# feiyeha/EGM-Unet

Hardware: AMD Instinct MI355X
Metric: train images/sec at 3x512x512 bs=8/GPU (higher is better)
Workload: dtype bf16; 1 GPU; EGM-UNet GRFBUNet(3,2,base_c=32) fwd+5-term-loss+bwd+SGD, 8x3x512x512 per GPU (BASELINE.json configs[1]); global_batch=8, parallelism=dp1, launch=hipGraph replay, world_size=1

## Files before the change

egm_unet_amd/csrc/blocks.hip:

```cpp
#include "common.h"
#include "derived_pack.h"

namespace {

__device__ __forceinline__ float sigm(float v) { return 1.f / (1.f + expf(-v)); }

#define PIX_LOOP(total_expr)                                                                           \
    const int ncv = C >> 3;                                                                            \
    const long long total = (total_expr);                                                              \
    for (long long i = blockIdx.x * 256LL + threadIdx.x; i < total; i += (long long)gridDim.x * 256)
#define PIX_LOOP_XCD(total_expr)                                                                       \
    const int ncv = C >> 3;                                                                            \
    const long long total = (total_expr);                                                              \
    for (long long i = xcd_contiguous_item(blockIdx.x, gridDim.x) * 256LL + threadIdx.x; i < total; i += (long long)gridDim.x * 256)

template <typename T>
__global__ void highpass3_kernel(const T* __restrict__ x, int ldx, T* __restrict__ out, int ldo, int N, int H, int W, int C) {
    PIX_LOOP_XCD((long long)N * H * W * ncv) {
        long long p; int cv; egm_divmod(i, ncv, p, cv);
        int xx, yy; egm_pix_yx(p, H, W, yy, xx);
        float s[8], c[8], v[8];
        zero8(s);
        load8(x + p * ldx + cv * 8, c);
#pragma unroll
        for (int r = -1; r <= 1; ++r)
#pragma unroll
            for (int q = -1; q <= 1; ++q) {
                if (yy + r < 0 || yy + r >= H || xx + q < 0 || xx + q >= W) continue;
                load8(x + (p + (long long)r * W + q) * ldx + cv * 8, v);
#pragma unroll
                for (int j = 0; j < 8; ++j) s[j] += v[j];
            }
#pragma unroll
        for (int j = 0; j < 8; ++j) c[j] -= s[j] * (1.f / 9.f);
        store8(out + p * ldo + cv * 8, c);
    }
}

template <typename T>
__global__ void gate_mul_fwd_kernel(const T* __restrict__ x, int ldx, const T* __restrict__ w, int ldw, T* __restrict__ out, int ldo,
                                    long long npix, int C) {
    PIX_LOOP(npix * ncv) {
        long long p; int cv; egm_divmod(i, ncv, p, cv);
        float a[8], b[8];
        load8(x + p * ldx + cv * 8, a); load8(w + p * ldw + cv * 8, b);
#pragma unroll
        for (int j = 0; j < 8; ++j) a[j] *= (1.f + b[j]);
        store8(out + p * ldo + cv * 8, a);
    }
}
template <typename T>
__global__ void gate_mul_bwd_kernel(const T* __restrict__ g, int ldg, const T* __restrict__ x, int ldx, const T* __restrict__ w, int ldw,
                                    T* __restrict__ dx, int lddx, T* __restrict__ dw, int lddw, long long npix, int C) {
    PIX_LOOP(npix * ncv) {
        long long p; int cv; egm_divmod(i, ncv, p, cv);
        float gg[8], a[8], b[8], o1[8], o2[8];
        load8(g + p * ldg + cv * 8, gg); load8(x + p * ldx + cv * 8, a); load8(w + p * ldw + cv * 8, b);
#pragma unroll
        for (int j = 0; j < 8; ++j) { o1[j] = gg[j] * (1.f + b[j]); o2[j] = gg[j] * a[j]; }
        store8(dx + p * lddx + cv * 8, o1); store8(dw + p * lddw + cv * 8, o2);
    }
}

template <typename T>
__global__ void scale_add_relu_fwd_kernel(const T* __restrict__ a, int lda, float alpha, const T* __restrict__ b, int ldb,
                                          T* __restrict__ out, int ldo, long long npix, int C) {
    PIX_LOOP(npix * ncv) {
        long long p; int cv; egm_divmod(i, ncv, p, cv);
        float u[8], v[8];
        load8(a + p * lda + cv * 8, u); load8(b + p * ldb + cv * 8, v);
#pragma unroll
        for (int j = 0; j < 8; ++j) u[j] = fmaxf(fmaf(alpha, u[j], v[j]), 0.f);
        store8(out + p * ldo + cv * 8, u);
    }
}
template <typename T>
__global__ void scale_add_relu_bwd_kernel(const T* __restrict__ g, int ldg, const T* __restrict__ out, int ldo, float alpha,
                                          T* __restrict__ da, int ldda, T* __restrict__ db, int lddb, long long npix, int C) {
    PIX_LOOP(npix * ncv) {
        long long p; int cv; egm_divmod(i, ncv, p, cv);
        float gg[8], o[8], u[8];
        load8(g + p * ldg + cv * 8, gg); load8(out + p * ldo + cv * 8, o);
#pragma unroll
        for (int j = 0; j < 8; ++j) { gg[j] = o[j] > 0.f ? gg[j] : 0.f; u[j] = alpha * gg[j]; }
        store8(da + p * ldda + cv * 8, u); store8(db + p * lddb + cv * 8, gg);
    }
}

template <int GROUP>
__device__ __forceinline__ float group_sum(float v) {
#pragma unroll
    for (int o = GROUP / 2; o > 0; o >>= 1) v += __shfl_xor(v, o, 64);
    return v;
}

template <typename T>
__global__ void gate3_fwd_kernel(const T* __restrict__ x, int ldx, const T* __restrict__ t, int ldt, T* __restrict__ out, int ldo,
                                 long long npix, int C) {
    PIX_LOOP(npix * ncv) {
        long long p; int cv; egm_divmod(i, ncv, p, cv);
        float a[8], tv[8];
        load8(x + p * ldx + cv * 8, a); load8(t + p * ldt, tv);
        const float m = 1.f + (sigm(tv[0]) + sigm(tv[1]) + sigm(tv[2])) * (1.f / 3.f);
#pragma unroll
        for (int j = 0; j < 8; ++j) a[j] *= m;
        store8(out + p * ldo + cv * 8, a);
    }
}
template <typename T, int GROUP>
__global__ void gate3_bwd_kernel(const T* __restrict__ g, int ldg, const T* __restrict__ x, int ldx, const T* __restrict__ t, int ldt,
                                 T* __restrict__ dx, int lddx, T* __restrict__ dt, int lddt, long long npix, int C) {
    const int ncv = C >> 3;
    const int ppb = 256 / GROUP;
    const int lane_in = threadIdx.x % GROUP, slot = threadIdx.x / GROUP;
    for (long long p0 = (long long)blockIdx.x * ppb; p0 < npix; p0 += (long long)gridDim.x * ppb) {
        const long long p = p0 + slot;
        float dot = 0.f, tv[8];
        zero8(tv);
        if (p < npix) {
            load8(t + p * ldt, tv);
            const float m = 1.f + (sigm(tv[0]) + sigm(tv[1]) + sigm(tv[2])) * (1.f / 3.f);
            for (int cv = lane_in; cv < ncv; cv += GROUP) {
                float gg[8], a[8], o[8];
                load8(g + p * ldg + cv * 8, gg); load8(x + p * ldx + cv * 8, a);
#pragma unroll
                for (int j = 0; j < 8; ++j) { o[j] = gg[j] * m; dot += gg[j] * a[j]; }
                store8(dx + p * lddx + cv * 8, o);
            }
        }
        dot = group_sum<GROUP>(dot);
        if (p < npix && lane_in == 0) {
            float o[8];
#pragma unroll
            for (int k = 0; k < 8; ++k) { const float s = sigm(tv[k]); o[k] = k < 3 ? dot * (1.f / 3.f) * s * (1.f - s) : 0.f; }
            store8(dt + p * lddt, o);
        }
    }
}

template <typename T>
__global__ void bcast_gate_fwd_kernel(const T* __restrict__ a, int lda, const T* __restrict__ gl, int ldgl, T* __restrict__ out, int ldo,
                                      long long npix, int C) {
    PIX_LOOP(npix * ncv) {
        long long p; int cv; egm_divmod(i, ncv, p, cv);
        float u[8];
        load8(a + p * lda + cv * 8, u);
        const float s = sigm(to_f32(gl[p * ldgl]));
#pragma unroll
        for (int j = 0; j < 8; ++j) u[j] *= s;
        store8(out + p * ldo + cv * 8, u);
    }
}
template <typename T, int GROUP>
__global__ void bcast_gate_bwd_kernel(const T* __restrict__ g, int ldg, const T* __restrict__ a, int lda, const T* __restrict__ gl, int ldgl,
                                      T* __restrict__ da, int ldda, T* __restrict__ dgl, int lddgl, long long npix, int C) {
    const int ncv = C >> 3;
    const int ppb = 256 / GROUP;
    const int lane_in = threadIdx.x % GROUP, slot = threadIdx.x / GROUP;
    for (long long p0 = (long long)blockIdx.x * ppb; p0 < npix; p0 += (long long)gridDim.x * ppb) {
        const long long p = p0 + slot;
        float dot = 0.f, s = 0.f;
        if (p < npix) {
            s = sigm(to_f32(gl[p * ldgl]));
            for (int cv = lane_in; cv < ncv; cv += GROUP) {
                float gg[8], u[8], o[8];
                load8(g + p * ldg + cv * 8, gg); load8(a + p * lda + cv * 8, u);
#pragma unroll
                for (int j = 0; j < 8; ++j) { o[j] = gg[j] * s; dot += gg[j] * u[j]; }
                store8(da + p * ldda + cv * 8, o);
            }
        }
        dot = group_sum<GROUP>(dot);
        if (p < npix && lane_in == 0) {
            float o[8]; zero8(o);
            o[0] = dot * s * (1.f - s);
            store8(dgl + p * lddgl, o);
        }
    }
}

template <typename T>
__global__ void gelu_fwd_kernel(const T* __restrict__ x, int ldx, T* __restrict__ out, int ldo, long long npix, int C) {
    PIX_LOOP(npix * ncv) {
        long long p; int cv; egm_divmod(i, ncv, p, cv);
        float v[8];
        load8(x + p * ldx + cv * 8, v);
#pragma unroll
        for (int j = 0; j < 8; ++j) v[j] = 0.5f * v[j] * (1.f + erff(v[j] * 0.70710678118654752f));
        store8(out + p * ldo + cv * 8, v);
    }
}
template <typename T>
__global__ void gelu_bwd_kernel(const T* __restrict__ g, int ldg, const T* __restrict__ x, int ldx, T* __restrict__ dx, int lddx,
                                long long npix, int C) {
    PIX_LOOP(npix * ncv) {
        long long p; int cv; egm_divmod(i, ncv, p, cv);
        float gg[8], v[8];
        load8(g + p * ldg + cv * 8, gg); load8(x + p * ldx + cv * 8, v);
#pragma unroll
        for (int j = 0; j < 8; ++j) {
            const float cdf = 0.5f * (1.f + erff(v[j] * 0.70710678118654752f));
            const float pdf = 0.3989422804014327f * expf(-0.5f * v[j] * v[j]);
            gg[j] *= cdf + v[j] * pdf;
        }
        store8(dx + p * lddx + cv * 8, gg);
    }
}

template <typename T, int GROUP>
__global__ void chan_meanmax_fwd_kernel(const T* __restrict__ x, int ldx, T* __restrict__ out, int ldo, long long npix, int C, int Creal) {
    const int ncv = C >> 3;
    const int ppb = 256 / GROUP;
    const int lane_in = threadIdx.x % GROUP, slot = threadIdx.x / GROUP;
    for (long long p0 = (long long)blockIdx.x * ppb; p0 < npix; p0 += (long long)gridDim.x * ppb) {
        const long long p = p0 + slot;
        float s = 0.f, m = -INFINITY;
        if (p < npix)
            for (int cv = lane_in; cv < ncv; cv += GROUP) {
                float v[8];
                load8(x + p * ldx + cv * 8, v);
#pragma unroll
                for (int j = 0; j < 8; ++j) if (cv * 8 + j < Creal) { s += v[j]; m = fmaxf(m, v[j]); }
            }
        s = group_sum<GROUP>(s);
#pragma unroll
        for (int o = GROUP / 2; o > 0; o >>= 1) m = fmaxf(m, __shfl_xor(m, o, 64));
        if (p < npix && lane_in == 0) {
            float o[8]; zero8(o);
            o[0] = s / (float)Creal; o[1] = m;
            store8(out + p * ldo, o);
        }
    }
}
template <typename T, int GROUP>
__global__ void chan_meanmax_bwd_kernel(const T* __restrict__ g, int ldg, const T* __restrict__ x, int ldx, T* __restrict__ dx, int lddx,
                                        long long npix, int C, int Creal) {
    const int ncv = C >> 3;
    const int ppb = 256 / GROUP;
    const int lane_in = threadIdx.x % GROUP, slot = threadIdx.x / GROUP;
    for (long long p0 = (long long)blockIdx.x * ppb; p0 < npix; p0 += (long long)gridDim.x * ppb) {
        const long long p = p0 + slot;
        float m = -INFINITY; int am = 0x7fffffff;
        if (p < npix)
            for (int cv = lane_in; cv < ncv; cv += GROUP) {
                float v[8];
                load8(x + p * ldx + cv * 8, v);
#pragma unroll
                for (int j = 0; j < 8; ++j) if (cv * 8 + j < Creal && v[j] > m) { m = v[j]; am = cv * 8 + j; }
            }
#pragma unroll
        for (int o = GROUP / 2; o > 0; o >>= 1) {
            const float m2 = __shfl_xor(m, o, 64); const int a2 = __shfl_xor(am, o, 64);
            if (m2 > m || (m2 == m && a2 < am)) { m = m2; am = a2; }
        }
        if (p < npix) {
            const float gm = to_f32(g[p * ldg]) / (float)Creal, gx = to_f32(g[p * ldg + 1]);
            for (int cv = lane_in; cv < ncv; cv += GROUP) {
                float o[8];
#pragma unroll
                for (int j = 0; j < 8; ++j) o[j] = (cv * 8 + j < Creal) ? gm + ((cv * 8 + j == am) ? gx : 0.f) : 0.f;
                store8(dx + p * lddx + cv * 8, o);
            }
        }
    }
}

template <typename T>
__global__ __launch_bounds__(256) void global_pool_partial_kernel(const T* __restrict__ x, int ldx, long long HW, int C,
                                                                  float* __restrict__ part, int* __restrict__ part_idx) {
    __shared__ float rs[256 * 8];
    __shared__ float rm[256 * 8];
    __shared__ int ri[256 * 8];
    const int n = blockIdx.y, ncv = C >> 3, rows = 256 / ncv;
    const int tid = threadIdx.x, cv = tid % ncv, row = tid / ncv;
    float s[8], m[8]; int ix[8];
#pragma unroll
    for (int j = 0; j < 8; ++j) { s[j] = 0.f; m[j] = -INFINITY; ix[j] = 0x7fffffff; }
    if (row < rows)
        for (long long p = (long long)blockIdx.x * rows + row; p < HW; p += (long long)gridDim.x * rows) {
            float v[8];
            load8(x + ((long long)n * HW + p) * ldx + cv * 8, v);
#pragma unroll
            for (int j = 0; j < 8; ++j) { s[j] += v[j]; if (v[j] > m[j]) { m[j] = v[j]; ix[j] = (int)p; } }
        }
#pragma unroll
    for (int j = 0; j < 8; ++j) { rs[tid * 8 + j] = s[j]; rm[tid * 8 + j] = m[j]; ri[tid * 8 + j] = ix[j]; }
    __syncthreads();
    for (int c = tid; c < C; c += 256) {
        float ss = 0.f, mm = -INFINITY; int ii = 0x7fffffff;
        for (int r = 0; r < rows; ++r) {
            const int k = (r * ncv + (c >> 3)) * 8 + (c & 7);
            ss += rs[k];
            if (rm[k] > mm || (rm[k] == mm && ri[k] < ii)) { mm = rm[k]; ii = ri[k]; }
        }
        const long long o = ((long long)n * gridDim.x + blockIdx.x) * 2 * C;
        part[o + c] = ss; part[o + C + c] = mm;
        part_idx[((long long)n * gridDim.x + blockIdx.x) * C + c] = ii;
    }
}
template <typename T>
__global__ __launch_bounds__(64) void global_pool_final_kernel(const float* __restrict__ part, const int* __restrict__ part_idx, int nblk, int N,
                                                               long long HW, int C, T* __restrict__ out, int* __restrict__ argidx) {
    const int n = blockIdx.y, c = blockIdx.x, lane = threadIdx.x;
    double ss = 0.0; float mm = -INFINITY; int ii = 0x7fffffff;
    for (int b = lane; b < nblk; b += 64) {
        const long long o = ((long long)n * nblk + b) * 2 * C;
        ss += (double)part[o + c];
        const float m = part[o + C + c]; const int k = part_idx[((long long)n * nblk + b) * C + c];
        if (m > mm || (m == mm && k < ii)) { mm = m; ii = k; }
    }
#pragma unroll
    for (int o = 32; o > 0; o >>= 1) {
        ss += __shfl_xor(ss, o, 64);
        const float m2 = __shfl_xor(mm, o, 64); const int i2 = __shfl_xor(ii, o, 64);
        if (m2 > mm || (m2 == mm && i2 < ii)) { mm = m2; ii = i2; }
    }
    if (lane == 0) {
        out[(long long)n * C + c] = from_f32<T>((float)(ss / (double)HW));
        out[(long long)(N + n) * C + c] = from_f32<T>(mm);
        argidx[(long long)n * C + c] = ii;
    }
}
template <typename T>
__global__ void global_pool_bwd_kernel(const T* __restrict__ gout, const int* __restrict__ argidx, T* __restrict__ dx, int lddx, int N,
                                       long long HW, int C) {
    PIX_LOOP((long long)N * HW * ncv) {
        long long p; int cv; egm_divmod(i, ncv, p, cv);
        const long long n = p / HW, pp = p - n * HW;
        float ga[8], gm[8], o[8];
        load8(gout + n * C + cv * 8, ga); load8(gout + (N + n) * C + cv * 8, gm);
#pragma unroll
        for (int j = 0; j < 8; ++j) o[j] = ga[j] / (float)HW + ((long long)argidx[n * C + cv * 8 + j] == pp ? gm[j] : 0.f);
        store8(dx + p * lddx + cv * 8, o);
    }
}

template <typename T>
__global__ void fusion_combine_fwd_kernel(const T* __restrict__ f, int ldf, const T* __restrict__ sv, int lds, const T* __restrict__ sa,
                                          int ldsa, const T* __restrict__ ca, T* __restrict__ out, int ldo, int N, long long HW, int C) {
    PIX_LOOP((long long)N * HW * ncv) {
        long long p; int cv; egm_divmod(i, ncv, p, cv);
        const long long n = p / HW;
        float a[8], b[8], c1[8], c2[8];
        load8(f + p * ldf + cv * 8, a); load8(sv + p * lds + cv * 8, b);
        load8(ca + n * C + cv * 8, c1); load8(ca + (N + n) * C + cv * 8, c2);
        const float ss = sigm(to_f32(sa[p * ldsa]));
#pragma unroll
        for (int j = 0; j < 8; ++j) a[j] += b[j] * ss * sigm(c1[j] + c2[j]);
        store8(out + p * ldo + cv * 8, a);
    }
}
template <typename T, int GROUP>
__global__ __launch_bounds__(256) void fusion_combine_bwd_kernel(const T* __restrict__ g, int ldg, const T* __restrict__ sv, int lds,
                                                                 const T* __restrict__ sa, int ldsa, const T* __restrict__ ca,
                                                                 T* __restrict__ ds, int ldds, T* __restrict__ dsa, int lddsa,
                                                                 float* __restrict__ part, int N, long long HW, int C) {
    __shared__ float red[256 * 8];
    const int n = blockIdx.y, ncv = C >> 3;
    const int ppb = 256 / GROUP;
    const int lane_in = threadIdx.x % GROUP, slot = threadIdx.x / GROUP;
    const int cv = lane_in;
    float sca[8], acc[8];
    zero8(acc); zero8(sca);
    if (cv < ncv) {
        float c1[8], c2[8];
        load8(ca + (long long)n * C + cv * 8, c1); load8(ca + (long long)(N + n) * C + cv * 8, c2);
#pragma unroll
        for (int j = 0; j < 8; ++j) sca[j] = sigm(c1[j] + c2[j]);
    }
    for (long long p0 = (long long)blockIdx.x * ppb; p0 < HW; p0 += (long long)gridDim.x * ppb) {
        const long long pl = p0 + slot, p = (long long)n * HW + pl;
        float dot = 0.f, ss = 0.f;
        if (pl < HW && cv < ncv) {
            float gg[8], b[8], o[8];
            ss = sigm(to_f32(sa[p * ldsa]));
            load8(g + p * ldg + cv * 8, gg); load8(sv + p * lds + cv * 8, b);
#pragma unroll
            for (int j = 0; j < 8; ++j) {
                o[j] = gg[j] * ss * sca[j];
                dot += gg[j] * b[j] * sca[j];
                acc[j] += gg[j] * b[j] * ss * sca[j] * (1.f - sca[j]);
            }
            store8(ds + p * ldds + cv * 8, o);
        }
        dot = group_sum<GROUP>(dot);
        if (pl < HW && lane_in == 0) {
            float o[8]; zero8(o);
            o[0] = dot * ss * (1.f - ss);
            store8(dsa + p * lddsa, o);
        }
    }
#pragma unroll
    for (int j = 0; j < 8; ++j) red[threadIdx.x * 8 + j] = acc[j];
    __syncthreads();
    for (int c = threadIdx.x; c < C; c += 256) {
        float v = 0.f;
        for (int sl = 0; sl < ppb; ++sl) v += red[(sl * GROUP + (c >> 3)) * 8 + (c & 7)];
        const long long o = ((long long)n * gridDim.x + blockIdx.x) * 2 * C;
        part[o + c] = v; part[o + C + c] = 0.f;
    }
}

__global__ void fold2_fwd_kernel(const float* __restrict__ w, float* __restrict__ out, int rows, int K) {
    for (int i = blockIdx.x * blockDim.x + threadIdx.x; i < rows * K; i += gridDim.x * blockDim.x) {
        const int r = i / K, k = i - r * K;
        out[i] = w[(long long)r * 2 * K + k] + w[(long long)r * 2 * K + K + k];
    }
}
__global__ void fold2_bwd_kernel(const float* __restrict__ g, float* __restrict__ dw, int rows, int K) {
    for (int i = blockIdx.x * blockDim.x + threadIdx.x; i < rows * K; i += gridDim.x * blockDim.x) {
        const int r = i / K, k = i - r * K;
        dw[(long long)r * 2 * K + k] = g[i]; dw[(long long)r * 2 * K + K + k] = g[i];
    }
}
__global__ void merge357_fwd_kernel(const float* __restrict__ w3, const float* __restrict__ w5, const float* __restrict__ w7,
                                    const float* __restrict__ b3, const float* __restrict__ b5, const float* __restrict__ b7,
                                    float* __restrict__ w, float* __restrict__ b, int Co, int Ci) {
    const int total = Co * Ci * 49;
    for (int i = blockIdx.x * blockDim.x + threadIdx.x; i < total; i += gridDim.x * blockDim.x) {
        const int t = i % 49, oc = i / 49, r = t / 7, s = t % 7;
        float v = w7[i];
        if (r >= 1 && r <= 5 && s >= 1 && s <= 5) v += w5[oc * 25 + (r - 1) * 5 + (s - 1)];
        if (r >= 2 && r <= 4 && s >= 2 && s <= 4) v += w3[oc * 9 + (r - 2) * 3 + (s - 2)];
        w[i] = v;
        if (i < Co) b[i] = b3[i] + b5[i] + b7[i];
    }
}
__global__ void merge357_bwd_kernel(const float* __restrict__ gw, float* __restrict__ d3, float* __restrict__ d5, float* __restrict__ d7,
                                    const float* __restrict__ gb, float* __restrict__ gb3, int Co, int Ci) {
    const int total = Co * Ci * 49;
    if (gb != nullptr)
        for (int i = blockIdx.x * blockDim.x + threadIdx.x; i < 3 * Co; i += gridDim.x * blockDim.x) gb3[i] = gb[i % Co];
    for (int i = blockIdx.x * blockDim.x + threadIdx.x; i < total; i += gridDim.x * blockDim.x) {
        const int t = i % 49, oc = i / 49, r = t / 7, s = t % 7;
        const float v = gw[i];
        d7[i] = v;
        if (r >= 1 && r <= 5 && s >= 1 && s <= 5) d5[oc * 25 + (r - 1) * 5 + (s - 1)] = v;
        if (r >= 2 && r <= 4 && s >= 2 && s <= 4) d3[oc * 9 + (r - 2) * 3 + (s - 2)] = v;
    }
}


template <typename T> __device__ __forceinline__ void load2(const T* p, float& a, float& b);
template <> __device__ __forceinline__ void load2<float>(const float* p, float& a, float& b) { const float2 v = *reinterpret_cast<const float2*>(p); a = v.x; b = v.y; }
template <> __device__ __forceinline__ void load2<bf16_t>(const bf16_t* p, float& a, float& b) {
    const uint32_t v = *reinterpret_cast<const uint32_t*>(p);
    a = __uint_as_float(v << 16); b = __uint_as_float(v & 0xffff0000u);
}
constexpr int SAF_TY = 16, SAF_TX = 64, SAF_PY = SAF_TY + 6, SAF_PX = SAF_TX + 6;
template <typename T>
__global__ __launch_bounds__(256) void sa_conv7_fwd_kernel(const T* __restrict__ x, int ldx, const float* __restrict__ w, T* __restrict__ y, int ldy, int N, int H, int W) {
    __shared__ float2 sx[SAF_PY * SAF_PX];
    __shared__ float sw[98];
    if (threadIdx.x < 98) sw[threadIdx.x] = w[threadIdx.x];
    const int tiles_x = (W + SAF_TX - 1) / SAF_TX, tiles_y = (H + SAF_TY - 1) / SAF_TY, ntiles = N * tiles_x * tiles_y;
    const int tx = threadIdx.x & 63, ty0 = threadIdx.x >> 6;
    for (int t = blockIdx.x; t < ntiles; t += gridDim.x) {
        const int n = t / (tiles_x * tiles_y), tr = t - n * tiles_x * tiles_y;
        const int y0 = (tr / tiles_x) * SAF_TY, x0 = (tr % tiles_x) * SAF_TX;
        const long long img = (long long)n * H * W;
        __syncthreads();
        for (int i = threadIdx.x; i < SAF_PY * SAF_PX; i += 256) {
            const int py = i / SAF_PX, px = i - py * SAF_PX, gy = y0 + py - 3, gx = x0 + px - 3;
            float a = 0.f, b2 = 0.f;
            if (gy >= 0 && gy < H && gx >= 0 && gx < W) load2(x + (img + (long long)gy * W + gx) * ldx, a, b2);
            sx[i] = make_float2(a, b2);
        }
        __syncthreads();
#pragma unroll
        for (int k4 = 0; k4 < SAF_TY / 4; ++k4) {
            const int ly = ty0 + 4 * k4, gy = y0 + ly, gx = x0 + tx;
            float acc = 0.f;
#pragma unroll
            for (int r = 0; r < 7; ++r)
#pragma unroll
                for (int q = 0; q < 7; ++q) {
                    const float2 v = sx[(ly + r) * SAF_PX + tx + q];
                    acc += v.x * sw[r * 7 + q] + v.y * sw[49 + r * 7 + q];
                }
            if (gy < H && gx < W) {
                float o[8]; zero8(o); o[0] = acc;
                store8(y + (img + (long long)gy * W + gx) * ldy, o);
            }
        }
    }
}
template <typename T>
__global__ __launch_bounds__(256) void sa_conv7_bwd_data_kernel(const T* __restrict__ dy, int lddy, const float* __restrict__ w, T* __restrict__ dx, int lddx, int N,
                                                                int H, int W) {
    __shared__ float sg[SAF_PY * SAF_PX];
    __shared__ float sw[98];
    if (threadIdx.x < 98) sw[threadIdx.x] = w[threadIdx.x];
    const int tiles_x = (W + SAF_TX - 1) / SAF_TX, tiles_y = (H + SAF_TY - 1) / SAF_TY, ntiles = N * tiles_x * tiles_y;
    const int tx = threadIdx.x & 63, ty0 = threadIdx.x >> 6;
    for (int t = blockIdx.x; t < ntiles; t += gridDim.x) {
        const int n = t / (tiles_x * tiles_y), tr = t - n * tiles_x * tiles_y;
        const int y0 = (tr / tiles_x) * SAF_TY, x0 = (tr % tiles_x) * SAF_TX;
        const long long img = (long long)n * H * W;
        __syncthreads();
        for (int i = threadIdx.x; i < SAF_PY * SAF_PX; i += 256) {
            const int py = i / SAF_PX, px = i - py * SAF_PX, gy = y0 + py - 3, gx = x0 + px - 3;
            sg[i] = (gy >= 0 && gy < H && gx >= 0 && gx < W) ? to_f32(dy[(img + (long long)gy * W + gx) * lddy]) : 0.f;
        }
        __syncthreads();
#pragma unroll
        for (int k4 = 0; k4 < SAF_TY / 4; ++k4) {
            const int ly = ty0 + 4 * k4, gy = y0 + ly, gx = x0 + tx;
            float a0 = 0.f, a1 = 0.f;
#pragma unroll
            for (int r = 0; r < 7; ++r)
#pragma unroll
                for (int q = 0; q < 7; ++q) {
                    const float g = sg[(ly + 6 - r) * SAF_PX + tx + 6 - q];
                    a0 += g * sw[r * 7 + q]; a1 += g * sw[49 + r * 7 + q];
                }
            if (gy < H && gx < W) {
                float o[8]; zero8(o); o[0] = a0; o[1] = a1;
                store8(dx + (img + (long long)gy * W + gx) * lddx, o);
            }
        }
    }
}
constexpr int SA_TY = 16, SA_TX = 64, SA_PY = SA_TY + 6, SA_PX = SA_TX + 6;
template <typename T>
__global__ __launch_bounds__(256) void sa_conv7_bwd_w_kernel(const T* __restrict__ x, int ldx, const T* __restrict__ dy, int lddy,
                                                             float* __restrict__ part, int N, int H, int W) {
    constexpr int kTileFloats = 2 * SA_PY * SA_PX + SA_TY * SA_TX, kRedFloats = 14 * 257;
    __shared__ __attribute__((aligned(16))) float sbuf[kTileFloats > kRedFloats ? kTileFloats : kRedFloats];
    float2* sx = reinterpret_cast<float2*>(sbuf);
    float* sdy = sbuf + 2 * SA_PY * SA_PX;
    __shared__ float red[4][98];
    float acc[98];
#pragma unroll
    for (int k = 0; k < 98; ++k) acc[k] = 0.f;
    const int tiles_x = (W + SA_TX - 1) / SA_TX, tiles_y = (H + SA_TY - 1) / SA_TY, ntiles = N * tiles_x * tiles_y;
    const int tx = threadIdx.x & 63, ty0 = threadIdx.x >> 6;
    for (int t = blockIdx.x; t < ntiles; t += gridDim.x) {
        const int n = t / (tiles_x * tiles_y), tr = t - n * tiles_x * tiles_y;
        const int y0 = (tr / tiles_x) * SA_TY, x0 = (tr % tiles_x) * SA_TX;
        const long long img = (long long)n * H * W;
        __syncthreads();
        for (int i = threadIdx.x; i < SA_PY * SA_PX; i += 256) {
            const int py = i / SA_PX, px = i - py * SA_PX, gy = y0 + py - 3, gx = x0 + px - 3;
            float a = 0.f, b2 = 0.f;
            if (gy >= 0 && gy < H && gx >= 0 && gx < W) load2(x + (img + (long long)gy * W + gx) * ldx, a, b2);
            sx[i] = make_float2(a, b2);
        }
        for (int i = threadIdx.x; i < SA_TY * SA_TX; i += 256) {
            const int py = i / SA_TX, px = i - py * SA_TX, gy = y0 + py, gx = x0 + px;
            sdy[i] = (gy < H && gx < W) ? to_f32(dy[(img + (long long)gy * W + gx) * lddy]) : 0.f;
        }
        __syncthreads();
#pragma unroll
        for (int k4 = 0; k4 < SA_TY / 4; ++k4) {
            const int ly = ty0 + 4 * k4;
            const float g = sdy[ly * SA_TX + tx];
#pragma unroll
            for (int r = 0; r < 7; ++r)
#pragma unroll
                for (int q = 0; q < 7; ++q) {
                    const float2 v = sx[(ly + r) * SA_PX + tx + q];
                    acc[r * 7 + q] += g * v.x; acc[49 + r * 7 + q] += g * v.y;
                }
        }
    }
    float* lds = sbuf;
#pragma unroll
    for (int k0 = 0; k0 < 98; k0 += 14) {
        __syncthreads();
#pragma unroll
        for (int j = 0; j < 14; ++j) lds[j * 257 + threadIdx.x] = acc[k0 + j];
        __syncthreads();
        if (threadIdx.x < 14 * 8) {
            const int j = threadIdx.x >> 3, part8 = threadIdx.x & 7;
            float v = 0.f;
            for (int i = 0; i < 32; ++i) v += lds[j * 257 + part8 * 32 + i];
            v += __shfl_xor(v, 1, 64); v += __shfl_xor(v, 2, 64); v += __shfl_xor(v, 4, 64);
            if (part8 == 0) red[0][k0 + j] = v;
        }
    }
    __syncthreads();
    if (threadIdx.x < 98) part[(long long)blockIdx.x * 98 + threadIdx.x] = red[0][threadIdx.x];
}
__global__ __launch_bounds__(256) void sa_conv7_bwd_w_final_kernel(const float* __restrict__ part, int nblk, float* __restrict__ dw) {
    __shared__ double red[256];
    const int k = blockIdx.x;
    double s = 0.0;
    for (int b = threadIdx.x; b < nblk; b += 256) s += (double)part[(long long)b * 98 + k];
    red[threadIdx.x] = s;
    __syncthreads();
    for (int o = 128; o > 0; o >>= 1) { if (threadIdx.x < o) red[threadIdx.x] += red[threadIdx.x + o]; __syncthreads(); }
    if (threadIdx.x == 0) dw[k] = (float)red[0];
}

inline int group_for(int ncv) { int g = 1; while (g < ncv) g <<= 1; return g; }

template <typename T>
__global__ __launch_bounds__(256) void ca_mlp_fwd_kernel(const T* __restrict__ pooled, int ldp, const float* __restrict__ w0,
                                                         const float* __restrict__ w2, float* __restrict__ h_out, T* __restrict__ logits,
                                                         int ldo, int R, int C, int Cr) {
    extern __shared__ float ca_smem[];
    float* sp = ca_smem;
    float* sh = ca_smem + R * C;
    float* s0 = sh + R * Cr;
    float* s2 = s0 + Cr * (C + 1);
    for (int i = threadIdx.x; i < R * C; i += 256) { const int r = i / C, c = i - r * C; sp[i] = to_f32(pooled[(long long)r * ldp + c]); }
    for (int i = threadIdx.x; i < Cr * C; i += 256) { const int j = i / C, c = i - j * C; s0[j * (C + 1) + c] = w0[i]; }
    for (int i = threadIdx.x; i < C * Cr; i += 256) { const int c = i / Cr, j = i - c * Cr; s2[c * (Cr + 1) + j] = w2[i]; }
    __syncthreads();
    for (int i = threadIdx.x; i < R * Cr; i += 256) {
        const int r = i / Cr, j = i - r * Cr;
        float a = 0.f;
        for (int c = 0; c < C; ++c) a = fmaf(s0[j * (C + 1) + c], sp[r * C + c], a);
        a = to_f32(from_f32<T>(a));
        a = a > 0.f ? a : 0.f;
        sh[i] = a; h_out[i] = a;
    }
    __syncthreads();
    for (int i = threadIdx.x; i < R * C; i += 256) {
        const int r = i / C, c = i - r * C;
        float a = 0.f;
        for (int j = 0; j < Cr; ++j) a = fmaf(s2[c * (Cr + 1) + j], sh[r * Cr + j], a);
        logits[(long long)r * ldo + c] = from_f32<T>(a);
    }
}
template <typename T>
__global__ __launch_bounds__(256) void ca_mlp_bwd_kernel(const T* __restrict__ dl, int ldd, const T* __restrict__ pooled, int ldp,
                                                         const float* __restrict__ h, const float* __restrict__ w0,
                                                         const float* __restrict__ w2, float* __restrict__ dw0, float* __restrict__ dw2,
                                                         T* __restrict__ dpooled, int lddp, int R, int C, int Cr) {
    extern __shared__ float ca_smem[];
    float* sdl = ca_smem;
    float* sp = sdl + R * C;
    float* sh = sp + R * C;
    float* sdh = sh + R * Cr;
    float* s0 = sdh + R * Cr;
    float* s2 = s0 + Cr * (C + 1);
    for (int i = threadIdx.x; i < R * C; i += 256) {
        const int r = i / C, c = i - r * C;
        sdl[i] = to_f32(dl[(long long)r * ldd + c]); sp[i] = to_f32(pooled[(long long)r * ldp + c]);
    }
    for (int i = threadIdx.x; i < R * Cr; i += 256) sh[i] = h[i];
    for (int i = threadIdx.x; i < Cr * C; i += 256) { const int j = i / C, c = i - j * C; s0[j * (C + 1) + c] = w0[i]; }
    for (int i = threadIdx.x; i < C * Cr; i += 256) { const int c = i / Cr, j = i - c * Cr; s2[c * (Cr + 1) + j] = w2[i]; }
    __syncthreads();
    for (int i = threadIdx.x; i < R * Cr; i += 256) {
        const int r = i / Cr, j = i - r * Cr;
        float a = 0.f;
        for (int c = 0; c < C; ++c) a = fmaf(s2[c * (Cr + 1) + j], sdl[r * C + c], a);
        a = to_f32(from_f32<T>(a));
        sdh[i] = sh[i] > 0.f ? a : 0.f;
    }
    for (int i = threadIdx.x; i < C * Cr; i += 256) {
        const int c = i / Cr, j = i - c * Cr;
        float a = 0.f;
        for (int r = 0; r < R; ++r) a = fmaf(sdl[r * C + c], sh[r * Cr + j], a);
        dw2[i] = a;
    }
    __syncthreads();
    for (int i = threadIdx.x; i < Cr * C; i += 256) {
        const int j = i / C, c = i - j * C;
        float a = 0.f;
        for (int r = 0; r < R; ++r) a = fmaf(sdh[r * Cr + j], sp[r * C + c], a);
        dw0[i] = a;
    }
    for (int i = threadIdx.x; i < R * C; i += 256) {
        const int r = i / C, c = i - r * C;
        float a = 0.f;
        for (int j = 0; j < Cr; ++j) a = fmaf(s0[j * (C + 1) + c], sdh[r * Cr + j], a);
        dpooled[(long long)r * lddp + c] = from_f32<T>(a);
    }
}

template <typename T>
__global__ __launch_bounds__(256) void rows_dup_kernel(const float* __restrict__ red, T* __restrict__ dst, int ldd, int N, int C) {
    for (int i = blockIdx.x * 256 + threadIdx.x; i < N * C; i += gridDim.x * 256) {
        const int n = i / C, c = i - n * C;
        const T v = from_f32<T>(red[((long long)n * 2) * C + c]);
        dst[(long long)n * ldd + c] = v;
        dst[(long long)(N + n) * ldd + c] = v;
    }
}

template <typename T>
__global__ void fold2_pack_kernel(const float* __restrict__ w, float* __restrict__ out, T* __restrict__ wf, T* __restrict__ wd, int rows, int K,
                                  int CoutP, int CinP) {
    for (int i = blockIdx.x * blockDim.x + threadIdx.x; i < CoutP * CinP; i += gridDim.x * blockDim.x)
        fold2_pack_elem<T>(i, w, out, wf, wd, rows, K, CoutP, CinP);
}
template <typename T>
__global__ void merge357_pack_kernel(const float* __restrict__ w3, const float* __restrict__ w5, const float* __restrict__ w7,
                                     const float* __restrict__ b3, const float* __restrict__ b5, const float* __restrict__ b7,
                                     float* __restrict__ w, float* __restrict__ b, T* __restrict__ wf, T* __restrict__ wd, int Co, int Ci,
                                     int CoutP, int CinP) {
    const int total = 49 * CoutP * CinP;
    for (int i = blockIdx.x * blockDim.x + threadIdx.x; i < total; i += gridDim.x * blockDim.x)
        merge357_pack_elem<T>(i, w3, w5, w7, b3, b5, b7, w, b, wf, wd, Co, Ci, CoutP, CinP);
}

}

#define EGM_GROUP_SWITCH(G, ...)                                                                \
    switch (G) { case 1: { constexpr int GROUP = 1; __VA_ARGS__; break; } case 2: { constexpr int GROUP = 2; __VA_ARGS__; break; } \
                 case 4: { constexpr int GROUP = 4; __VA_ARGS__; break; } case 8: { constexpr int GROUP = 8; __VA_ARGS__; break; } \
                 case 16: { constexpr int GROUP = 16; __VA_ARGS__; break; } case 32: { constexpr int GROUP = 32; __VA_ARGS__; break; } \
                 default: { constexpr int GROUP = 64; __VA_ARGS__; break; } }

extern "C" int egm_highpass3(int dtype, const void* x, int ldx, void* out, int ldo, int N, int H, int W, int C, egm_stream_t s) {
    EGM_REQ_VEC("highpass3", x, ldx, C); EGM_REQ_VEC("highpass3", out, ldo, C);
    EGM_REQUIRE(N > 0 && H > 0 && W > 0, "highpass3: bad shape");
    EGM_DISPATCH_DTYPE(dtype, hipLaunchKernelGGL((highpass3_kernel<T>), dim3(egm_stream_grid((long long)N * H * W * (C / 8))), dim3(256), 0,
                                                 (hipStream_t)s, (const T*)x, ldx, (T*)out, ldo, N, H, W, C));
    EGM_CHECK_LAUNCH("highpass3");
    return EGM_OK;
}
extern "C" int egm_gate_mul_fwd(int dtype, const void* x, int ldx, const void* w, int ldw, void* out, int ldo, long long npix, int C,
                                egm_stream_t s) {
    EGM_REQ_VEC("gate_mul_fwd", x, ldx, C); EGM_REQ_VEC("gate_mul_fwd", w, ldw, C); EGM_REQ_VEC("gate_mul_fwd", out, ldo, C);
    EGM_DISPATCH_DTYPE(dtype, hipLaunchKernelGGL((gate_mul_fwd_kernel<T>), dim3(egm_stream_grid(npix * (C / 8))), dim3(256), 0, (hipStream_t)s,
                                                 (const T*)x, ldx, (const T*)w, ldw, (T*)out, ldo, npix, C));
    EGM_CHECK_LAUNCH("gate_mul_fwd");
    return EGM_OK;
}
extern "C" int egm_gate_mul_bwd(int dtype, const void* g, int ldg, const void* x, int ldx, const void* w, int ldw, void* dx, int lddx,
                                void* dw, int lddw, long long npix, int C, egm_stream_t s) {
    EGM_REQ_VEC("gate_mul_bwd", g, ldg, C); EGM_REQ_VEC("gate_mul_bwd", x, ldx, C); EGM_REQ_VEC("gate_mul_bwd", w, ldw, C);
    EGM_REQ_VEC("gate_mul_bwd", dx, lddx, C); EGM_REQ_VEC("gate_mul_bwd", dw, lddw, C);
    EGM_DISPATCH_DTYPE(dtype, hipLaunchKernelGGL((gate_mul_bwd_kernel<T>), dim3(egm_stream_grid(npix * (C / 8))), dim3(256), 0, (hipStream_t)s,
                                                 (const T*)g, ldg, (const T*)x, ldx, (const T*)w, ldw, (T*)dx, lddx, (T*)dw, lddw, npix, C));
    EGM_CHECK_LAUNCH("gate_mul_bwd");
    return EGM_OK;
}
extern "C" int egm_scale_add_relu_fwd(int dtype, const void* a, int lda, float alpha, const void* b, int ldb, void* out, int ldo,
                                      long long npix, int C, egm_stream_t s) {
    EGM_REQ_VEC("scale_add_relu_fwd", a, lda, C); EGM_REQ_VEC("scale_add_relu_fwd", b, ldb, C); EGM_REQ_VEC("scale_add_relu_fwd", out, ldo, C);
    EGM_DISPATCH_DTYPE(dtype, hipLaunchKernelGGL((scale_add_relu_fwd_kernel<T>), dim3(egm_stream_grid(npix * (C / 8))), dim3(256), 0,
                                                 (hipStream_t)s, (const T*)a, lda, alpha, (const T*)b, ldb, (T*)out, ldo, npix, C));
    EGM_CHECK_LAUNCH("scale_add_relu_fwd");
    return EGM_OK;
}
extern "C" int egm_scale_add_relu_bwd(int dtype, const void* g, int ldg, const void* out, int ldo, float alpha, void* da, int ldda,
                                      void* db, int lddb, long long npix, int C, egm_stream_t s) {
    EGM_REQ_VEC("scale_add_relu_bwd", g, ldg, C); EGM_REQ_VEC("scale_add_relu_bwd", out, ldo, C);
    EGM_REQ_VEC("scale_add_relu_bwd", da, ldda, C); EGM_REQ_VEC("scale_add_relu_bwd", db, lddb, C);
    EGM_DISPATCH_DTYPE(dtype, hipLaunchKernelGGL((scale_add_relu_bwd_kernel<T>), dim3(egm_stream_grid(npix * (C / 8))), dim3(256), 0,
                                                 (hipStream_t)s, (const T*)g, ldg, (const T*)out, ldo, alpha, (T*)da, ldda, (T*)db, lddb, npix, C));
    EGM_CHECK_LAUNCH("scale_add_relu_bwd");
    return EGM_OK;
}
extern "C" int egm_gate3_fwd(int dtype, const void* x, int ldx, const void* t, int ldt, void* out, int ldo, long long npix, int C,
                             egm_stream_t s) {
    EGM_REQ_VEC("gate3_fwd", x, ldx, C); EGM_REQ_VEC("gate3_fwd", t, ldt, 8); EGM_REQ_VEC("gate3_fwd", out, ldo, C);
    EGM_DISPATCH_DTYPE(dtype, hipLaunchKernelGGL((gate3_fwd_kernel<T>), dim3(egm_stream_grid(npix * (C / 8))), dim3(256), 0, (hipStream_t)s,
                                                 (const T*)x, ldx, (const T*)t, ldt, (T*)out, ldo, npix, C));
    EGM_CHECK_LAUNCH("gate3_fwd");
    return EGM_OK;
}
extern "C" int egm_gate3_bwd(int dtype, const void* g, int ldg, const void* x, int ldx, const void* t, int ldt, void* dx, int lddx,
                             void* dt, int lddt, long long npix, int C, egm_stream_t s) {
    EGM_REQ_VEC("gate3_bwd", g, ldg, C); EGM_REQ_VEC("gate3_bwd", x, ldx, C); EGM_REQ_VEC("gate3_bwd", t, ldt, 8);
    EGM_REQ_VEC("gate3_bwd", dx, lddx, C); EGM_REQ_VEC("gate3_bwd", dt, lddt, 8);
    const int G = group_for(C / 8 > 64 ? 64 : C / 8);
    const int grid = egm_stream_grid(npix * G);
    EGM_DISPATCH_DTYPE(dtype, EGM_GROUP_SWITCH(G, hipLaunchKernelGGL((gate3_bwd_kernel<T, GROUP>), dim3(grid), dim3(256), 0, (hipStream_t)s,
                                                                     (const T*)g, ldg, (const T*)x, ldx, (const T*)t, ldt, (T*)dx, lddx,
                                                                     (T*)dt, lddt, npix, C)));
    EGM_CHECK_LAUNCH("gate3_bwd");
    return EGM_OK;
}
extern "C" int egm_bcast_gate_fwd(int dtype, const void* a, int lda, const void* gl, int ldgl, void* out, int ldo, long long npix, int C,
                                  egm_stream_t s) {
    EGM_REQ_VEC("bcast_gate_fwd", a, lda, C); EGM_REQ_VEC("bcast_gate_fwd", gl, ldgl, 8); EGM_REQ_VEC("bcast_gate_fwd", out, ldo, C);
    EGM_DISPATCH_DTYPE(dtype, hipLaunchKernelGGL((bcast_gate_fwd_kernel<T>), dim3(egm_stream_grid(npix * (C / 8))), dim3(256), 0, (hipStream_t)s,
                                                 (const T*)a, lda, (const T*)gl, ldgl, (T*)out, ldo, npix, C));
    EGM_CHECK_LAUNCH("bcast_gate_fwd");
    return EGM_OK;
}
extern "C" int egm_bcast_gate_bwd(int dtype, const void* g, int ldg, const void* a, int lda, const void* gl, int ldgl, void* da, int ldda,
                                  void* dgl, int lddgl, long long npix, int C, egm_stream_t s) {
    EGM_REQ_VEC("bcast_gate_bwd", g, ldg, C); EGM_REQ_VEC("bcast_gate_bwd", a, lda, C); EGM_REQ_VEC("bcast_gate_bwd", gl, ldgl, 8);
    EGM_REQ_VEC("bcast_gate_bwd", da, ldda, C); EGM_REQ_VEC("bcast_gate_bwd", dgl, lddgl, 8);
    const int G = group_for(C / 8 > 64 ? 64 : C / 8);
    const int grid = egm_stream_grid(npix * G);
    EGM_DISPATCH_DTYPE(dtype, EGM_GROUP_SWITCH(G, hipLaunchKernelGGL((bcast_gate_bwd_kernel<T, GROUP>), dim3(grid), dim3(256), 0,
                                                                     (hipStream_t)s, (const T*)g, ldg, (const T*)a, lda, (const T*)gl, ldgl,
                                                                     (T*)da, ldda, (T*)dgl, lddgl, npix, C)));
    EGM_CHECK_LAUNCH("bcast_gate_bwd");
    return EGM_OK;
}
extern "C" int egm_gelu_fwd(int dtype, const void* x, int ldx, void* out, int ldo, long long npix, int C, egm_stream_t s) {
    EGM_REQ_VEC("gelu_fwd", x, ldx, C); EGM_REQ_VEC("gelu_fwd", out, ldo, C);
    EGM_DISPATCH_DTYPE(dtype, hipLaunchKernelGGL((gelu_fwd_kernel<T>), dim3(egm_stream_grid(npix * (C / 8))), dim3(256), 0, (hipStream_t)s,
                                                 (const T*)x, ldx, (T*)out, ldo, npix, C));
    EGM_CHECK_LAUNCH("gelu_fwd");
    return EGM_OK;
}
extern "C" int egm_gelu_bwd(int dtype, const void* g, int ldg, const void* x, int ldx, void* dx, int lddx, long long npix, int C,
                            egm_stream_t s) {
    EGM_REQ_VEC("gelu_bwd", g, ldg, C); EGM_REQ_VEC("gelu_bwd", x, ldx, C); EGM_REQ_VEC("gelu_bwd", dx, lddx, C);
    EGM_DISPATCH_DTYPE(dtype, hipLaunchKernelGGL((gelu_bwd_kernel<T>), dim3(egm_stream_grid(npix * (C / 8))), dim3(256), 0, (hipStream_t)s,
                                                 (const T*)g, ldg, (const T*)x, ldx, (T*)dx, lddx, npix, C));
    EGM_CHECK_LAUNCH("gelu_bwd");
    return EGM_OK;
}
extern "C" int egm_chan_meanmax_fwd(int dtype, const void* x, int ldx, void* out, int ldo, long long npix, int C, int C_real,
                                    egm_stream_t s) {
    EGM_REQ_VEC("chan_meanmax_fwd", x, ldx, C); EGM_REQ_VEC("chan_meanmax_fwd", out, ldo, 8);
    EGM_REQUIRE(C_real > 0 && C_real <= C, "chan_meanmax_fwd: bad C_real");
    const int G = group_for(C / 8 > 64 ? 64 : C / 8);
    EGM_DISPATCH_DTYPE(dtype, EGM_GROUP_SWITCH(G, hipLaunchKernelGGL((chan_meanmax_fwd_kernel<T, GROUP>), dim3(egm_stream_grid(npix * G)), dim3(256),
                                                                     0, (hipStream_t)s, (const T*)x, ldx, (T*)out, ldo, npix, C, C_real)));
    EGM_CHECK_LAUNCH("chan_meanmax_fwd");
    return EGM_OK;
}
extern "C" int egm_chan_meanmax_bwd(int dtype, const void* g, int ldg, const void* x, int ldx, void* dx, int lddx, long long npix, int C,
                                    int C_real, egm_stream_t s) {
    EGM_REQ_VEC("chan_meanmax_bwd", g, ldg, 8); EGM_REQ_VEC("chan_meanmax_bwd", x, ldx, C); EGM_REQ_VEC("chan_meanmax_bwd", dx, lddx, C);
    EGM_REQUIRE(C_real > 0 && C_real <= C, "chan_meanmax_bwd: bad C_real");
    const int G = group_for(C / 8 > 64 ? 64 : C / 8);
    EGM_DISPATCH_DTYPE(dtype, EGM_GROUP_SWITCH(G, hipLaunchKernelGGL((chan_meanmax_bwd_kernel<T, GROUP>), dim3(egm_stream_grid(npix * G)), dim3(256),
                                                                     0, (hipStream_t)s, (const T*)g, ldg, (const T*)x, ldx, (T*)dx, lddx, npix,
                                                                     C, C_real)));
    EGM_CHECK_LAUNCH("chan_meanmax_bwd");
    return EGM_OK;
}

static int pool_blocks(long long HW, int C) {
    const int rows = 256 / (C >> 3);
    long long b = (HW + rows - 1) / rows;
    if (b > 128) b = 128;
    return (int)(b < 1 ? 1 : b);
}
extern "C" long long egm_global_pool_workspace(int N, long long HW, int C) {
    if (N <= 0 || HW <= 0 || C <= 0 || C % 8 || C > 2048) return -1;
    return (long long)N * pool_blocks(HW, C) * 3 * C * 4;
}
extern "C" int egm_global_avgmax_fwd(int dtype, const void* x, int ldx, void* out, int* argidx, void* workspace, int N, long long HW,
                                     int C, egm_stream_t s) {
    EGM_REQ_VEC("global_avgmax_fwd", x, ldx, C);
    EGM_REQUIRE(out && argidx && workspace && egm_aligned16(out) && N > 0 && HW > 0 && C <= 2048, "global_avgmax_fwd: bad args");
    const int nb = pool_blocks(HW, C);
    float* part = (float*)workspace;
    int* pidx = (int*)(part + (long long)N * nb * 2 * C);
    EGM_DISPATCH_DTYPE(dtype, {
        hipLaunchKernelGGL((global_pool_partial_kernel<T>), dim3(nb, N), dim3(256), 0, (hipStream_t)s, (const T*)x, ldx, HW, C, part, pidx);
        hipLaunchKernelGGL((global_pool_final_kernel<T>), dim3(C, N), dim3(64), 0, (hipStream_t)s, part, pidx, nb, N, HW, C,
                           (T*)out, argidx);
    });
    EGM_CHECK_LAUNCH("global_avgmax_fwd");
    return EGM_OK;
}
extern "C" int egm_global_avgmax_bwd(int dtype, const void* gout, const int* argidx, void* dx, int lddx, int N, long long HW, int C,
                                     egm_stream_t s) {
    EGM_REQ_VEC("global_avgmax_bwd", dx, lddx, C);
    EGM_REQUIRE(gout && argidx && egm_aligned16(gout) && N > 0 && HW > 0, "global_avgmax_bwd: bad args");
    EGM_DISPATCH_DTYPE(dtype, hipLaunchKernelGGL((global_pool_bwd_kernel<T>), dim3(egm_stream_grid((long long)N * HW * (C / 8))), dim3(256), 0,
                                                 (hipStream_t)s, (const T*)gout, argidx, (T*)dx, lddx, N, HW, C));
    EGM_CHECK_LAUNCH("global_avgmax_bwd");
    return EGM_OK;
}

extern "C" int egm_rows_dup(int dtype, const float* red, void* dst, int ldd, int N, int C, egm_stream_t s) {
    EGM_REQUIRE(red && dst && N > 0 && C > 0 && ldd >= C, "rows_dup: bad args");
    int grid = (N * C + 255) / 256; if (grid > 64) grid = 64;
    EGM_DISPATCH_DTYPE(dtype, hipLaunchKernelGGL((rows_dup_kernel<T>), dim3(grid), dim3(256), 0, (hipStream_t)s, red, (T*)dst, ldd, N, C));
    EGM_CHECK_LAUNCH("rows_dup");
    return EGM_OK;
}
extern "C" int egm_ca_mlp_fwd(int dtype, const void* pooled, int ldp, const float* w0, const float* w2, float* h, void* logits, int ldo, int R,
                              int C, int Cr, egm_stream_t s) {
    EGM_REQUIRE(pooled && w0 && w2 && h && logits, "ca_mlp_fwd: null pointer");
    EGM_REQUIRE(R > 0 && C > 0 && Cr > 0 && ldp >= C && ldo >= C, "ca_mlp_fwd: bad shape R=%d C=%d Cr=%d", R, C, Cr);
    const size_t smem = (size_t)(R * C + R * Cr + Cr * (C + 1) + C * (Cr + 1)) * sizeof(float);
    EGM_REQUIRE(smem <= 64 * 1024, "ca_mlp_fwd: %d rows x %d channels do not fit one workgroup's LDS", R, C);
    EGM_DISPATCH_DTYPE(dtype, hipLaunchKernelGGL((ca_mlp_fwd_kernel<T>), dim3(1), dim3(256), smem, (hipStream_t)s, (const T*)pooled, ldp, w0, w2, h,
                                                 (T*)logits, ldo, R, C, Cr));
    EGM_CHECK_LAUNCH("ca_mlp_fwd");
    return EGM_OK;
}
extern "C" int egm_ca_mlp_bwd(int dtype, const void* dlogits, int ldd, const void* pooled, int ldp, const float* h, const float* w0,
                              const float* w2, float* dw0, float* dw2, void* dpooled, int lddp, int R, int C, int Cr, egm_stream_t s) {
    EGM_REQUIRE(dlogits && pooled && h && w0 && w2 && dw0 && dw2 && dpooled, "ca_mlp_bwd: null pointer");
    EGM_REQUIRE(R > 0 && C > 0 && Cr > 0 && ldd >= C && ldp >= C && lddp >= C, "ca_mlp_bwd: bad shape R=%d C=%d Cr=%d", R, C, Cr);
    const size_t smem = (size_t)(2 * R * C + 2 * R * Cr + Cr * (C + 1) + C * (Cr + 1)) * sizeof(float);
    EGM_REQUIRE(smem <= 64 * 1024, "ca_mlp_bwd: %d rows x %d channels do not fit one workgroup's LDS", R, C);
    EGM_DISPATCH_DTYPE(dtype, hipLaunchKernelGGL((ca_mlp_bwd_kernel<T>), dim3(1), dim3(256), smem, (hipStream_t)s, (const T*)dlogits, ldd,
                                                 (const T*)pooled, ldp, h, w0, w2, dw0, dw2, (T*)dpooled, lddp, R, C, Cr));
    EGM_CHECK_LAUNCH("ca_mlp_bwd");
    return EGM_OK;
}
extern "C" int egm_fusion_combine_fwd(int dtype, const void* f, int ldf, const void* sv, int lds, const void* sa, int ldsa, const void* ca,
                                      void* out, int ldo, int N, long long HW, int C, egm_stream_t s) {
    EGM_REQ_VEC("fusion_combine_fwd", f, ldf, C); EGM_REQ_VEC("fusion_combine_fwd", sv, lds, C); EGM_REQ_VEC("fusion_combine_fwd", sa, ldsa, 8);
    EGM_REQ_VEC("fusion_combine_fwd", out, ldo, C);
    EGM_REQUIRE(ca && egm_aligned16(ca) && N > 0 && HW > 0, "fusion_combine_fwd: bad args");
    EGM_DISPATCH_DTYPE(dtype, hipLaunchKernelGGL((fusion_combine_fwd_kernel<T>), dim3(egm_stream_grid((long long)N * HW * (C / 8))), dim3(256), 0,
                                                 (hipStream_t)s, (const T*)f, ldf, (const T*)sv, lds, (const T*)sa, ldsa, (const T*)ca, (T*)out,
                                                 ldo, N, HW, C));
    EGM_CHECK_LAUNCH("fusion_combine_fwd");
    return EGM_OK;
}
extern "C" int egm_fusion_combine_blocks(long long HW, int C) {
    if (C <= 0 || C % 8 || C > 512) return -1;
    const int G = group_for(C / 8);
    long long b = (HW + 256 / G - 1) / (256 / G);
    if (b > 256) b = 256;
    return (int)(b < 1 ? 1 : b);
}
extern "C" int egm_fusion_combine_bwd(int dtype, const void* g, int ldg, const void* sv, int lds, const void* sa, int ldsa, const void* ca,
                                      void* ds, int ldds, void* dsa, int lddsa, float* partials, int N, long long HW, int C, egm_stream_t s) {
    EGM_REQ_VEC("fusion_combine_bwd", g, ldg, C); EGM_REQ_VEC("fusion_combine_bwd", sv, lds, C); EGM_REQ_VEC("fusion_combine_bwd", sa, ldsa, 8);
    EGM_REQ_VEC("fusion_combine_bwd", ds, ldds, C); EGM_REQ_VEC("fusion_combine_bwd", dsa, lddsa, 8);
    EGM_REQUIRE(ca && partials && N > 0 && HW > 0 && C <= 512, "fusion_combine_bwd: bad args (C <= 512)");
    const int G = group_for(C / 8);
    const int nb = egm_fusion_combine_blocks(HW, C);
    EGM_DISPATCH_DTYPE(dtype, EGM_GROUP_SWITCH(G, hipLaunchKernelGGL((fusion_combine_bwd_kernel<T, GROUP>), dim3(nb, N), dim3(256), 0,
                                                                     (hipStream_t)s, (const T*)g, ldg, (const T*)sv, lds, (const T*)sa, ldsa,
                                                                     (const T*)ca, (T*)ds, ldds, (T*)dsa, lddsa, partials, N, HW, C)));
    EGM_CHECK_LAUNCH("fusion_combine_bwd");
    return EGM_OK;
}

extern "C" int egm_fold2_fwd(const float* w, float* out, int rows, int K, egm_stream_t s) {
    EGM_REQUIRE(w && out && rows > 0 && K > 0, "fold2_fwd: bad args");
    hipLaunchKernelGGL(fold2_fwd_kernel, dim3((rows * K + 255) / 256), dim3(256), 0, (hipStream_t)s, w, out, rows, K);
    EGM_CHECK_LAUNCH("fold2_fwd");
    return EGM_OK;
}
extern "C" int egm_fold2_bwd(const float* g, float* dw, int rows, int K, egm_stream_t s) {
    EGM_REQUIRE(g && dw && rows > 0 && K > 0, "fold2_bwd: bad args");
    hipLaunchKernelGGL(fold2_bwd_kernel, dim3((rows * K + 255) / 256), dim3(256), 0, (hipStream_t)s, g, dw, rows, K);
    EGM_CHECK_LAUNCH("fold2_bwd");
    return EGM_OK;
}
extern "C" int egm_merge357_fwd(const float* w3, const float* w5, const float* w7, const float* b3, const float* b5, const float* b7,
                                float* w, float* b, int Co, int Ci, egm_stream_t s) {
    EGM_REQUIRE(w3 && w5 && w7 && b3 && b5 && b7 && w && b && Co > 0 && Ci > 0, "merge357_fwd: bad args");
    hipLaunchKernelGGL(merge357_fwd_kernel, dim3((Co * Ci * 49 + 255) / 256), dim3(256), 0, (hipStream_t)s, w3, w5, w7, b3, b5, b7, w, b, Co, Ci);
    EGM_CHECK_LAUNCH("merge357_fwd");
    return EGM_OK;
}
extern "C" int egm_fold2_pack(int dtype, const float* w, float* out, void* wf, void* wd, int rows, int K, egm_stream_t s) {
    EGM_REQUIRE(w && out && wf && wd && rows > 0 && K > 0, "fold2_pack: bad args");
    const int CoutP = (rows + 7) / 8 * 8, CinP = (K + 7) / 8 * 8;
    EGM_DISPATCH_DTYPE(dtype, hipLaunchKernelGGL((fold2_pack_kernel<T>), dim3((CoutP * CinP + 255) / 256), dim3(256), 0, (hipStream_t)s, w, out,
                                                 (T*)wf, (T*)wd, rows, K, CoutP, CinP));
    EGM_CHECK_LAUNCH("fold2_pack");
    return EGM_OK;
}
extern "C" int egm_merge357_pack(int dtype, const float* w3, const float* w5, const float* w7, const float* b3, const float* b5, const float* b7,
                                 float* w, float* b, void* wf, void* wd, int Co, int Ci, egm_stream_t s) {
    EGM_REQUIRE(w3 && w5 && w7 && b3 && b5 && b7 && w && b && wf && wd && Co > 0 && Ci > 0, "merge357_pack: bad args");
    const int CoutP = (Co + 7) / 8 * 8, CinP = (Ci + 7) / 8 * 8;
    EGM_DISPATCH_DTYPE(dtype, hipLaunchKernelGGL((merge357_pack_kernel<T>), dim3((49 * CoutP * CinP + 255) / 256), dim3(256), 0, (hipStream_t)s,
                                                 w3, w5, w7, b3, b5, b7, w, b, (T*)wf, (T*)wd, Co, Ci, CoutP, CinP));
    EGM_CHECK_LAUNCH("merge357_pack");
    return EGM_OK;
}
extern "C" int egm_merge357_bwd(const float* gw, float* d3, float* d5, float* d7, const float* gb, float* gb3, int Co, int Ci, egm_stream_t s) {
    EGM_REQUIRE(gw && d3 && d5 && d7 && Co > 0 && Ci > 0 && ((gb == nullptr) == (gb3 == nullptr)), "merge357_bwd: bad args");
    hipLaunchKernelGGL(merge357_bwd_kernel, dim3((Co * Ci * 49 + 255) / 256), dim3(256), 0, (hipStream_t)s, gw, d3, d5, d7, gb, gb3, Co, Ci);
    EGM_CHECK_LAUNCH("merge357_bwd");
    return EGM_OK;
}

static int sa_tile_grid(int N, int H, int W) {
    const long long t = (long long)N * ((H + SAF_TY - 1) / SAF_TY) * ((W + SAF_TX - 1) / SAF_TX);
    return (int)(t > 4096 ? 4096 : (t < 1 ? 1 : t));
}
static int sa_blocks(long long npix) { long long b = (npix + 255) / 256; if (b > 512) b = 512; return (int)(b < 1 ? 1 : b); }
extern "C" int egm_sa_conv7_fwd(int dtype, const void* x, int ldx, const float* w, void* y, int ldy, int N, int H, int W, egm_stream_t s) {
    EGM_REQ_VEC("sa_conv7_fwd", x, ldx, 8); EGM_REQ_VEC("sa_conv7_fwd", y, ldy, 8);
    EGM_REQUIRE(w && N > 0 && H > 0 && W > 0, "sa_conv7_fwd: bad args");
    EGM_DISPATCH_DTYPE(dtype, hipLaunchKernelGGL((sa_conv7_fwd_kernel<T>), dim3(sa_tile_grid(N, H, W)), dim3(256), 0, (hipStream_t)s,
                                                 (const T*)x, ldx, w, (T*)y, ldy, N, H, W));
    EGM_CHECK_LAUNCH("sa_conv7_fwd");
    return EGM_OK;
}
extern "C" long long egm_sa_conv7_bwd_workspace(int N, int H, int W) {
    if (N <= 0 || H <= 0 || W <= 0) return -1;
    return (long long)sa_blocks((long long)N * H * W) * 98 * 4;
}
extern "C" int egm_sa_conv7_bwd(int dtype, const void* x, int ldx, const void* dy, int lddy, const float* w, void* dx, int lddx, float* dw,
                                void* workspace, int N, int H, int W, egm_stream_t s) {
    EGM_REQ_VEC("sa_conv7_bwd", x, ldx, 8); EGM_REQ_VEC("sa_conv7_bwd", dy, lddy, 8); EGM_REQ_VEC("sa_conv7_bwd", dx, lddx, 8);
    EGM_REQUIRE(w && dw && workspace && N > 0 && H > 0 && W > 0, "sa_conv7_bwd: bad args");
    const long long npix = (long long)N * H * W;
    const int nb = sa_blocks(npix);
    EGM_DISPATCH_DTYPE(dtype, {
        hipLaunchKernelGGL((sa_conv7_bwd_data_kernel<T>), dim3(sa_tile_grid(N, H, W)), dim3(256), 0, (hipStream_t)s, (const T*)dy, lddy, w, (T*)dx, lddx,
                           N, H, W);
        hipLaunchKernelGGL((sa_conv7_bwd_w_kernel<T>), dim3(nb), dim3(256), 0, (hipStream_t)s, (const T*)x, ldx, (const T*)dy, lddy,
                           (float*)workspace, N, H, W);
    });
    hipLaunchKernelGGL(sa_conv7_bwd_w_final_kernel, dim3(98), dim3(256), 0, (hipStream_t)s, (const float*)workspace, nb, dw);
    EGM_CHECK_LAUNCH("sa_conv7_bwd");
    return EGM_OK;
}
```

egm_unet_amd/egm_unet.py:

```python
import math
from typing import Dict

import torch
import torch.nn as nn

from . import ops
from ._lib import ACT_NONE, ACT_RELU, ACT_SIGMOID
from .unet import DoubleConv, OutConv, Up, _SegNetBase


class StdPool(nn.Module):
    """Holder only (src/EGM-UNet.py:827-834); the statistics come from egm_mca_reduce."""


class MCAGate(nn.Module):
    def __init__(self, k_size, pool_types=("avg", "std")):
        super().__init__()
        self.pools = nn.ModuleList([nn.AdaptiveAvgPool2d(1) if p == "avg" else StdPool() for p in pool_types])
        self.conv = nn.Conv2d(1, 1, kernel_size=(1, k_size), stride=1, padding=(0, (k_size - 1) // 2), bias=False)
        self.sigmoid = nn.Sigmoid()
        self.weight = nn.Parameter(torch.rand(2))
        self.conv._egm_no_prepack = True


class MCALayer(nn.Module):
    def __init__(self, inp, no_spatial=False):
        super().__init__()
        self.no_spatial = no_spatial
        self.inp = inp
        temp = round(abs((math.log2(inp) - 1) / 1.5))
        kernel = temp if temp % 2 else temp - 1
        self.h_cw = MCAGate(3)
        self.w_hc = MCAGate(3)
        if not no_spatial:
            self.c_hw = MCAGate(kernel)

    def forward(self, x, exclusive=False):
        return ops.mca_layer(x, self, self.training and torch.is_grad_enabled(), exclusive)


class EdgeAwareFeatureEnhancer(nn.Module):
    def __init__(self, in_channels):
        super().__init__()
        self.edge_extractor = nn.AvgPool2d(kernel_size=3, stride=1, padding=1)
        self.weight_generator = nn.Sequential(nn.Conv2d(in_channels, in_channels, kernel_size=1), nn.BatchNorm2d(in_channels),
                                              nn.Sigmoid())

    def forward(self, x, x_alias=None, edge=None):
        if edge is not None:
            e, xb = edge, x_alias
        elif x_alias is not None:
            e, xb = ops.highpass3(x), x_alias
        else:
            e, xb = ops.fork_highpass3(x, 1)
        return ops.conv_bn_ew(e, self.weight_generator[0], self.weight_generator[1], ACT_SIGMOID, xb, ops.EW_GATE)


class BasicConv(nn.Module):

    def __init__(self, in_channels, out_channels, kernel_size, stride=1, padding=0, dilation=1, groups=1, relu=True, bn=True,
                 bias=False):
        super().__init__()
        if stride != 1 or not bn:
            raise NotImplementedError("egm_unet_amd: BasicConv is used with stride 1 and BN only")
        self.out_channels = out_channels
        self.conv = nn.Conv2d(in_channels, out_channels, kernel_size=kernel_size, stride=stride, padding=padding, dilation=dilation,
                              groups=groups, bias=bias)
        self.bn = nn.BatchNorm2d(out_channels, eps=1e-5, momentum=0.01, affine=True)
        self.relu = nn.ReLU(inplace=True) if relu else None
        self._dil, self._groups = dilation, groups

    def forward(self, x, out=None):
        return ops.conv_bn_act(x, self.conv, self.bn, ACT_RELU if self.relu is not None else ACT_NONE, dil=self._dil,
                               groups=self._groups, out=out)


class ChannelAttentionModule(nn.Module):
    def __init__(self, in_channels, reduction=4):
        super().__init__()
        self.avg_pool = nn.AdaptiveAvgPool2d(1)
        self.max_pool = nn.AdaptiveMaxPool2d(1)
        self.fc = nn.Sequential(nn.Conv2d(in_channels, in_channels // reduction, 1, bias=False), nn.ReLU(inplace=True),
                                nn.Conv2d(in_channels // reduction, in_channels, 1, bias=False))
        self.sigmoid = nn.Sigmoid()
        self.fc[0]._egm_no_prepack = self.fc[2]._egm_no_prepack = True

    def logits(self, f):
        return ops.ca_mlp(ops.global_avgmax(f), self.fc[0].weight, self.fc[2].weight)


class SpatialAttentionModule(nn.Module):
    def __init__(self, kernel_size=7):
        super().__init__()
        self.conv1 = nn.Conv2d(2, 1, kernel_size, padding=kernel_size // 2, bias=False)
        self.conv1._egm_no_prepack = kernel_size == 7
        self.sigmoid = nn.Sigmoid()

    def logits(self, s, c_real):
        mm = ops.chan_meanmax(s, c_real)
        if tuple(self.conv1.weight.shape) == (1, 2, 7, 7):
            return ops.sa_conv7(mm, self.conv1.weight)
        return ops.conv2d(mm, self.conv1.weight)


class FusionConv(nn.Module):
    def __init__(self, in_channels, out_channels, factor=4.0):
        super().__init__()
        dim = int(out_channels // factor)
        self.down = nn.Conv2d(2 * in_channels, dim, kernel_size=1, stride=1)
        self.conv_3x3 = nn.Conv2d(dim, dim, kernel_size=3, stride=1, padding=1)
        self.conv_5x5 = nn.Conv2d(dim, dim, kernel_size=5, stride=1, padding=2)
        self.conv_7x7 = nn.Conv2d(dim, dim, kernel_size=7, stride=1, padding=3)
        self.spatial_attention = SpatialAttentionModule()
        self.channel_attention = ChannelAttentionModule(dim)
        self.up = nn.Conv2d(dim, out_channels, kernel_size=1, stride=1)
        self._dim = dim
        for m in (self.down, self.conv_3x3, self.conv_5x5, self.conv_7x7):
            m._egm_no_prepack = True

    def _egm_derived_weights(self):
        return [("fold2", (self.down.weight,)),
                ("merge357", (self.conv_3x3.weight, self.conv_5x5.weight, self.conv_7x7.weight, self.conv_3x3.bias, self.conv_5x5.bias,
                              self.conv_7x7.bias))]

    def forward(self, x1, x2=None):
        if x2 is not None and x2 is not x1:
            k = self.down.weight.shape[1] // 2
            x1 = ops.cat_channels([x1, x2])
            wdown = self.down.weight if k % 8 == 0 else ops.spread_cols(self.down.weight, (k, k))
        else:
            wdown = ops.fold2(self.down.weight, pack_dtype=x1.dtype)
        f = ops.conv2d(x1, wdown, self.down.bias)
        f_res, f_ms, f_ca = ops.fork(f, 3)
        w7, b7 = ops.merge357(self.conv_3x3.weight, self.conv_5x5.weight, self.conv_7x7.weight, self.conv_3x3.bias,
                              self.conv_5x5.bias, self.conv_7x7.bias, pack_dtype=f.dtype)
        s = ops.conv2d(f_ms, w7, b7)
        s_a, s_b = ops.fork(s, 2)
        sa = self.spatial_attention.logits(s_a, self._dim)
        ca = self.channel_attention.logits(f_ca)
        return ops.conv2d(ops.fusion_combine(f_res, s_b, sa, ca), self.up.weight, self.up.bias)


class EdgeEnhancedGRFB(nn.Module):
    def __init__(self, in_channels, out_channels, stride=1, scale=0.1, visual=12, fusion_factor=4.0):
        super().__init__()
        self.scale = scale
        self.out_channels = out_channels
        self.inter_planes = i = max(in_channels // 8, 4)
        self.edge_enhancer = EdgeAwareFeatureEnhancer(in_channels)
        self.branch_dir = nn.Sequential(
            BasicConv(in_channels, 2 * i, 1),
            BasicConv(2 * i, 2 * i, 3, padding=visual, dilation=visual, relu=False),
            BasicConv(2 * i, 2 * i, 1))
        self.branch_edge = nn.Sequential(
            BasicConv(in_channels, i, 1),
            EdgeAwareFeatureEnhancer(i),
            BasicConv(i, 2 * i, (3, 3), stride, padding=1, groups=i),
            BasicConv(2 * i, 2 * i, 3, padding=2 * visual, dilation=2 * visual, relu=False),
            BasicConv(2 * i, 2 * i, 1))
        self.branch_ctx = nn.Sequential(
            BasicConv(in_channels, i, 3, padding=1),
            BasicConv(i, 2 * i, 3, stride=stride, padding=1, groups=2),
            BasicConv(2 * i, 2 * i, 3, padding=3 * visual, dilation=3 * visual, relu=False),
            BasicConv(2 * i, 2 * i, 1))
        self.concat_channels = in_channels + 6 * i
        self.fusion_conv = FusionConv(self.concat_channels, out_channels, factor=fusion_factor)
        self.shortcut = BasicConv(in_channels, out_channels, 1, stride, relu=False)
        self.relu = nn.ReLU(inplace=False)
        self.target_enhancer = nn.Sequential(nn.Conv2d(out_channels, 3, 3, padding=1), nn.Sigmoid())

    @staticmethod
    def _seq(seq, x, out):
        mods = list(seq)
        for m in mods[:-1]:
            x = m(x)
        return mods[-1](x, out=out)

    def cat_buffer(self, N, H, W, dtype, device):
        C, i2 = self.shortcut.conv.in_channels, 2 * self.inter_planes
        if i2 % 8 or C % 8:
            return None
        return ops.cat_slots(N, H, W, [C, i2, i2, i2], dtype, device)

    def forward(self, x, out=None, cat=None, pool=False, x_slot=None):
        edge, x_e2, x_cat, x_sc = ops.fork_highpass3(x, 3, out=x_slot)
        xe = self.edge_enhancer(None, x_e2, edge=edge)
        N, H, W, C = x.shape
        if cat is None:
            cat = self.cat_buffer(N, H, W, x.dtype, x.device) if C == self.shortcut.conv.in_channels else None
        if cat is not None:
            buf, (_, sd, se, sc) = cat
        else:
            buf, sd, se, sc = None, None, None, None
        bd, be, bc = self.branch_dir, self.branch_edge, self.branch_ctx
        xe_d, xe_e, xe_c = ops.fork(xe, 3)
        def item(m, t, o=None):
            return (t, m.conv, m.bn, ACT_RELU if m.relu is not None else ACT_NONE, m._dil, m._groups, o)

        d, e, c = ops.multi_conv_bn_act([item(bd[0], xe_d), item(be[0], xe_e), item(bc[0], xe_c)])
        e = be[1](e)
        e, c = ops.multi_conv_bn_act([item(be[2], e), item(bc[1], c)])
        d, e, c = ops.multi_conv_bn_act([item(bd[1], d), item(be[3], e), item(bc[2], c)])
        d, e, c = ops.multi_conv_bn_act([item(bd[2], d, sd), item(be[4], e, se), item(bc[3], c, sc)])
        cat = ops.cat_channels([x_cat, d, e, c], buf)
        out_f = self.fusion_conv(cat)
        sc = self.shortcut
        out_f = ops.conv_bn_ew(x_sc, sc.conv, sc.bn, ACT_NONE, out_f, ops.EW_SAR, alpha=self.scale)
        o_a, o_b = ops.fork(out_f, 2)
        t = ops.conv2d(o_a, self.target_enhancer[0].weight, self.target_enhancer[0].bias)
        if pool:
            if ops.pool_fusable(o_b):
                return ops.gate3_pool(o_b, t, out)
            return ops.fork_maxpool2(ops.gate3(o_b, t, out))
        return ops.gate3(o_b, t, out)


class Conv(nn.Module):
    default_act = nn.SiLU()

    def __init__(self, c1, c2, k=1, s=1, p=None, g=1, d=1, act=True):
        super().__init__()
        if s != 1 or not isinstance(k, int) or (p is not None and p != d * (k - 1) // 2):
            raise NotImplementedError("egm_unet_amd: Conv is built for square kernels, stride 1, 'same' padding")
        self.conv = nn.Conv2d(c1, c2, k, s, d * (k - 1) // 2, groups=g, dilation=d, bias=False)
        self.bn = nn.BatchNorm2d(c2)
        self.act = self.default_act if act is True else act if isinstance(act, nn.Module) else nn.Identity()
        if not isinstance(self.act, (nn.SiLU, nn.Identity, nn.ReLU, nn.Sigmoid)):
            raise NotImplementedError("egm_unet_amd: Conv activation must be SiLU, ReLU, Sigmoid or identity")
        self._dil, self._groups = d, g

    def forward(self, x):
        from ._lib import ACT_SIGMOID, ACT_SILU
        code = {nn.SiLU: ACT_SILU, nn.Identity: ACT_NONE, nn.ReLU: ACT_RELU, nn.Sigmoid: ACT_SIGMOID}[type(self.act)]
        return ops.conv_bn_act(x, self.conv, self.bn, code, dil=self._dil, groups=self._groups)


class HEGDC(nn.Module):

    def __init__(self, in_channels, out_channels, mid_channels=None, den=0.5):
        super().__init__()
        mid_channels = out_channels if mid_channels is None else mid_channels
        self.in_channels = in_channels
        self.edge_conv = nn.Conv2d(1, 4, kernel_size=3, padding=1, bias=False)
        sx = torch.tensor([[3., 0., -3.], [10., 0., -10.], [3., 0., -3.]]) / 16.0
        sy = torch.tensor([[3., 10., 3.], [0., 0., 0.], [-3., -10., -3.]]) / 16.0
        ox = torch.tensor([[1., 0., -1.], [2., 0., -2.], [1., 0., -1.]]) / 4.0
        oy = torch.tensor([[1., 2., 1.], [0., 0., 0.], [-1., -2., -1.]]) / 4.0
        self.edge_conv.weight.data = torch.stack([sx, sy, ox, oy], dim=0).unsqueeze(1)
        self.edge_conv.weight.requires_grad = False
        self.den = nn.Parameter(torch.tensor([den]))
        self.alpha = nn.Parameter(torch.tensor(1.0))
        self.conv1 = nn.Sequential(nn.Conv2d(in_channels, mid_channels, kernel_size=3, padding=1, bias=False), nn.BatchNorm2d(mid_channels),
                                   nn.ReLU(inplace=True))
        self.conv2 = nn.Sequential(nn.Conv2d(mid_channels, out_channels, kernel_size=3, padding=1, bias=False), nn.BatchNorm2d(out_channels))
        self.edge_fusion = nn.Sequential(nn.Conv2d(5, 8, kernel_size=1), nn.ReLU(inplace=True), nn.Conv2d(8, mid_channels, kernel_size=1),
                                         nn.Sigmoid())
        self.register_buffer("phi_base", torch.ones(1, 1, 3, 3))
        for c in (self.edge_conv, self.conv1[0]):
            c._egm_no_prepack = True

    def forward(self, x):
        feats = ops.hegdc_edge_features(x, self.in_channels)
        ef = self.edge_fusion
        w = ops.act(ops.conv2d(feats, ef[0].weight, ef[0].bias), ACT_RELU)
        w = ops.act(ops.conv2d(w, ef[2].weight, ef[2].bias), ACT_SIGMOID)
        w1 = ops.scale_sigmoid(self.conv1[0].weight, self.den)
        bn1 = self.conv1[1]
        if bn1.training:
            y, stats = ops.conv2d(x, w1, None, want_stats=True)
            h = ops.bn_act(y, bn1, ACT_RELU, stats)
        else:
            h = ops.bn_act(ops.conv2d(x, w1, None), bn1, ACT_RELU)
        h = ops.mul2_scalar(h, w, self.alpha)
        return ops.conv_bn_act(h, self.conv2[0], self.conv2[1], ACT_RELU)


class ELA(nn.Module):

    def __init__(self, channel, kernel_size=7):
        super().__init__()
        self.conv = nn.Conv1d(channel, channel, kernel_size=kernel_size, padding=kernel_size // 2, groups=channel, bias=False)
        self.gn = nn.GroupNorm(16, channel)
        self.sigmoid = nn.Sigmoid()

    def forward(self, x):
        return ops.ela(x, self.conv, self.gn)


class GRFB(nn.Module):

    def __init__(self, in_channels, out_channels, stride=1, scale=0.1, visual=12):
        super().__init__()
        self.scale = scale
        self.out_channels = out_channels
        i = in_channels // 8
        self.branch0 = nn.Sequential(
            BasicConv(in_channels, 2 * i, 1, stride),
            BasicConv(2 * i, 2 * i, 3, 1, padding=visual, dilation=visual, relu=False),
            BasicConv(2 * i, 2 * i, 1, stride))
        self.branch1 = nn.Sequential(
            BasicConv(in_channels, i, 1, 1),
            BasicConv(i, 2 * i, (3, 3), stride, padding=(1, 1), groups=i),
            BasicConv(2 * i, 2 * i, 1, stride),
            BasicConv(2 * i, 2 * i, 3, 1, padding=2 * visual, dilation=2 * visual, relu=False),
            BasicConv(2 * i, 2 * i, 1, 1))
        self.branch2 = nn.Sequential(
            BasicConv(in_channels, i, 1, 1),
            BasicConv(i, 2 * i, 3, 1, padding=1, groups=i),
            BasicConv(2 * i, 2 * i, 1, stride),
            BasicConv(2 * i, 2 * i, 3, stride, padding=1, groups=2 * i),
            BasicConv(2 * i, 2 * i, 1, stride),
            BasicConv(2 * i, 2 * i, 3, 1, padding=3 * visual, dilation=3 * visual, relu=False),
            BasicConv(2 * i, 2 * i, 1, stride))
        self.ConvLinear = BasicConv(14 * i, out_channels, 1, 1, relu=False)
        self.shortcut = BasicConv(in_channels, out_channels, 1, stride, relu=False)
        self.relu = nn.ReLU(inplace=False)

    def forward(self, x):
        x_cat, x0, x1, x2, x_sc = ops.fork(x, 5)
        seq = EdgeEnhancedGRFB._seq
        cat = ops.cat_channels([x_cat, seq(self.branch0, x0, None), seq(self.branch1, x1, None), seq(self.branch2, x2, None)])
        return ops.scale_add_relu(self.ConvLinear(cat), self.scale, self.shortcut(x_sc))


class RecursiveGatedAttention(nn.Module):
    def __init__(self, dim, order=2, reduction=8, kernel_size=3):
        super().__init__()
        if order < 1 or kernel_size != 3:
            raise NotImplementedError("egm_unet_amd: RecursiveGatedAttention is built for a 3x3 depthwise kernel (as EGM-UNet uses it)")
        self.order, self.dim = order, dim
        self.split_sizes = [dim // (2 ** i) for i in range(1, order)]
        self.split_sizes.append(dim // (2 ** (order - 1)))
        self.split_sizes.reverse()
        total = sum(self.split_sizes)
        if total > dim:
            self.split_sizes[-1] = dim - sum(self.split_sizes[:-1])
        if any(s % 8 for s in self.split_sizes):
            raise NotImplementedError("egm_unet_amd: RGA split sizes must be multiples of 8")
        self.proj_in = nn.Conv2d(dim, self.split_sizes[0] + sum(self.split_sizes), 1)
        self.gate_convs = nn.ModuleList()
        for i in range(order):
            in_ch = self.split_sizes[i]
            self.gate_convs.append(nn.Sequential(nn.Conv2d(in_ch, max(in_ch // reduction, 8), 1), nn.GELU(),
                                                 nn.Conv2d(max(in_ch // reduction, 8), 1, 1), nn.Sigmoid()))
        self.transform_convs = nn.ModuleList()
        for i in range(order - 1):
            self.transform_convs.append(nn.Conv2d(self.split_sizes[i], self.split_sizes[i + 1], 1))
        self.dwconv = nn.Conv2d(sum(self.split_sizes), sum(self.split_sizes), kernel_size, padding=kernel_size // 2,
                                groups=sum(self.split_sizes))
        self.proj_out = nn.Conv2d(self.split_sizes[-1], dim, 1)
        self.scale = nn.Parameter(torch.tensor(1.0))
        self.dwconv._egm_no_prepack = True
        print(f"[RGA] order={order}, split_sizes={self.split_sizes}")

    def _gate(self, i, g):
        seq = self.gate_convs[i]
        h = ops.gelu(ops.conv2d(g, seq[0].weight, seq[0].bias))
        return ops.conv2d(h, seq[2].weight, seq[2].bias)

    def forward(self, x):
        s0 = self.split_sizes[0]
        fused = ops.conv2d(x, self.proj_in.weight, self.proj_in.bias)
        base, gates = ops.split_channels(fused, s0)
        gates = ops.dwconv3(gates, self.dwconv.weight, self.dwconv.bias, self.scale)
        pieces, rest = [], gates
        for i in range(self.order - 1):
            piece, rest = ops.split_channels(rest, self.split_sizes[i])
            pieces.append(piece)
        pieces.append(rest)
        out = base
        for i in range(self.order):
            out = ops.bcast_gate(out, self._gate(i, pieces[i]))
            if i < self.order - 1:
                out = ops.conv2d(out, self.transform_convs[i].weight, self.transform_convs[i].bias)
        return ops.conv2d(out, self.proj_out.weight, self.proj_out.bias)


class DoubleConv1(nn.Sequential):

    def __init__(self, in_channels, out_channels, mid_channels=None, use_mca=True):
        if mid_channels is None:
            mid_channels = out_channels
        layers = [nn.Conv2d(in_channels, mid_channels, kernel_size=3, padding=1, bias=False), nn.BatchNorm2d(mid_channels), nn.ReLU(inplace=True)]
        if use_mca:
            layers.append(MCALayer(mid_channels))
        layers += [nn.Conv2d(mid_channels, out_channels, kernel_size=3, padding=1, bias=False), nn.BatchNorm2d(out_channels),
                   nn.ReLU(inplace=True), EdgeEnhancedGRFB(mid_channels, out_channels, stride=1, scale=0.1, visual=12)]
        super().__init__(*layers)
        self._mca = use_mca

    def forward(self, x, out=None, pool=False):
        o = 1 if self._mca else 0
        if self._mca:
            if ops.fuse_mca_bn():
                x = self[3](ops.conv_bn_lazy(x, self[0], self[1], ACT_RELU), exclusive=True)
            else:
                x = self[3](ops.conv_bn_act(x, self[0], self[1], ACT_RELU))
        else:
            x = ops.conv_bn_act(x, self[0], self[1], ACT_RELU)
        grfb = self[6 + o]
        N, H, W = x.shape[0], x.shape[1], x.shape[2]
        cat = grfb.cat_buffer(N, H, W, x.dtype, x.device) if self[3 + o].out_channels == grfb.shortcut.conv.in_channels else None
        slot = None if cat is None else cat[1][0]
        if ops.bn_hp_fusable(x.dtype):
            return grfb(ops.conv_bn_act(x, self[3 + o], self[4 + o], ACT_RELU, lazy="force"), out, cat, pool=pool, x_slot=slot)
        x = ops.conv_bn_act(x, self[3 + o], self[4 + o], ACT_RELU, out=slot)
        return grfb(x, out, cat, pool=pool)


class Down(nn.Sequential):
    def __init__(self, in_channels, out_channels, use_mca=True):
        super().__init__(nn.MaxPool2d(2, stride=2), DoubleConv1(in_channels, out_channels, use_mca=use_mca))

    def forward(self, x, out=None, pooled=None, pool=False):
        return self[1](ops.maxpool2(x) if pooled is None else pooled, out, pool=pool)


class GRFBUNet(_SegNetBase):
    def __init__(self, in_channels: int = 1, num_classes: int = 2, bilinear: bool = True, base_c: int = 64,
                 use_attention: bool = False, use_mca: bool = True):
        super().__init__()
        self.in_channels = in_channels
        self.num_classes = num_classes
        self.bilinear = bilinear
        self.in_conv = DoubleConv(in_channels, base_c)
        self.down1 = Down(base_c, base_c * 2, use_mca)
        self.down2 = Down(base_c * 2, base_c * 4, use_mca)
        self.down3 = Down(base_c * 4, base_c * 8, use_mca)
        factor = 2 if bilinear else 1
        self.down4 = Down(base_c * 8, base_c * 16 // factor, use_mca)
        self.attn1 = RecursiveGatedAttention(base_c * 16 // factor)
        self.up1 = Up(base_c * 16, base_c * 8 // factor, bilinear)
        self.up2 = Up(base_c * 8, base_c * 4 // factor, bilinear)
        self.up3 = Up(base_c * 4, base_c * 2 // factor, bilinear)
        self.up4 = Up(base_c * 2, base_c, bilinear)
        self.out_conv = OutConv(base_c, num_classes)

    def forward(self, x: torch.Tensor) -> Dict[str, torch.Tensor]:
        x = self._enter(x)
# ... 24 lines not shown
```

egm_unet_amd/ops.py:

```python
import ctypes
import os
import struct
import threading
import weakref
from collections import namedtuple

import torch
from torch.autograd import Function, Variable

from ._lib import ACT_NONE, ACT_RELU, ACT_SIGMOID, dtype_code, lib, ptr, stream


def pad8(c: int) -> int:
    return (c + 7) // 8 * 8


def _nhwc(t: torch.Tensor):
    assert t.dim() == 4, t.shape
    N, H, W, C = t.shape
    s = t.stride()
    ok = (s[3] == 1 and s[2] % 8 == 0 and s[2] >= C and s[1] == W * s[2] and s[0] == H * W * s[2]
          and t.data_ptr() % 16 == 0 and C % 8 == 0)
    if not ok:
        if C % 8:
# ... 1772 lines not shown
        lib().call("egm_gate_mul_bwd", dtype_code(x.dtype), ptr(g), ldg, ptr(x), ldx, ptr(w), ldw, ptr(dx), C, ptr(dw), C, _npix(x), C, stream())
        return dx, dw


def gate_mul(x, w):
    return _GateMul.apply(x, w)


class _ScaleAddRelu(Function):
    @staticmethod
    def forward(ctx, a, alpha, b):
        a, lda = _nhwc(a); b, ldb = _nhwc(b)
        C = a.shape[3]
        out = torch.empty(a.shape, dtype=a.dtype, device=a.device)
        lib().call("egm_scale_add_relu_fwd", dtype_code(a.dtype), ptr(a), lda, float(alpha), ptr(b), ldb, ptr(out), C, _npix(a), C, stream())
        ctx.save_for_backward(out)
        ctx.alpha = float(alpha)
        return out

    @staticmethod
    def backward(ctx, g):
        (out,) = ctx.saved_tensors
        out, ldo = _nhwc(out); g, ldg = _nhwc(g)
        C = out.shape[3]
        da = torch.empty(out.shape, dtype=out.dtype, device=out.device)
        db = torch.empty(out.shape, dtype=out.dtype, device=out.device)
        lib().call("egm_scale_add_relu_bwd", dtype_code(out.dtype), ptr(g), ldg, ptr(out), ldo, ctx.alpha, ptr(da), C, ptr(db), C, _npix(out), C,
                   stream())
        return da, None, db


def scale_add_relu(a, alpha, b):
    return _ScaleAddRelu.apply(a, alpha, b)


class _Gate3(Function):
    @staticmethod
    def forward(ctx, x, t, out_slot=None):
        x, ldx = _nhwc(x); t, ldt = _nhwc(t)
        C = x.shape[3]
        out, ldo = _slot_or_new(out_slot, tuple(x.shape), x.dtype, x.device)
        lib().call("egm_gate3_fwd", dtype_code(x.dtype), ptr(x), ldx, ptr(t), ldt, ptr(out), ldo, _npix(x), C, stream())
        ctx.save_for_backward(x, t)
        return out

    @staticmethod
    def backward(ctx, g):
        x, t = ctx.saved_tensors
        x, ldx = _nhwc(x); t, ldt = _nhwc(t); g, ldg = _nhwc(g)
        C = x.shape[3]
        dx = torch.empty(x.shape, dtype=x.dtype, device=x.device)
        dt = torch.empty(t.shape[:3] + (8,), dtype=x.dtype, device=x.device)
        lib().call("egm_gate3_bwd", dtype_code(x.dtype), ptr(g), ldg, ptr(x), ldx, ptr(t), ldt, ptr(dx), C, ptr(dt), 8, _npix(x), C, stream())
        return dx, dt, None


def gate3(x, t, out=None):
    return _Gate3.apply(x, t, None if out is None else [out])


class _Gate3Pool(Function):

    @staticmethod
    def forward(ctx, x, t, out_slot=None):
        x, ldx = _nhwc(x); t, ldt = _nhwc(t)
        N, H, W, C = x.shape
        out, ldo = _slot_or_new(out_slot, tuple(x.shape), x.dtype, x.device)
        pooled = torch.empty((N, H // 2, W // 2, C), dtype=x.dtype, device=x.device)
        lib().call("egm_gate3_fwd_pool", dtype_code(x.dtype), ptr(x), ldx, ptr(t), ldt, ptr(out), ldo, ptr(pooled), C, N, H, W, C, stream())
        ctx.save_for_backward(x, t, out)
        ctx.set_materialize_grads(False)
        return out, pooled

    @staticmethod
    def backward(ctx, gskip, gpool):
        if gskip is None and gpool is None:
            return None, None, None
        x, t, out = ctx.saved_tensors
        x, ldx = _nhwc(x); t, ldt = _nhwc(t)
        N, H, W, C = x.shape
        L, dt_, st = lib(), dtype_code(x.dtype), stream()
        dx = torch.empty(x.shape, dtype=x.dtype, device=x.device)
        dt = torch.empty(t.shape[:3] + (8,), dtype=x.dtype, device=x.device)
        if gskip is not None and gpool is not None:
            gs, lds = _nhwc(gskip); gp, ldp = _nhwc(gpool)
            L.call("egm_gate3_pool_bwd", dt_, ptr(gs), lds, ptr(gp), ldp, ptr(x), ldx, ptr(t), ldt, ptr(dx), C, ptr(dt), 8, N, H, W, C, st)
            return dx, dt, None
        if gskip is None:
            ok, ldo = _nhwc(out); gp, ldp = _nhwc(gpool)
            gskip = torch.empty(x.shape, dtype=x.dtype, device=x.device)
            L.call("egm_maxpool2_bwd", dt_, ptr(ok), ldo, ptr(gp), ldp, ptr(gskip), C, N, H, W, C, st)
        g, ldg = _nhwc(gskip)
        L.call("egm_gate3_bwd", dt_, ptr(g), ldg, ptr(x), ldx, ptr(t), ldt, ptr(dx), C, ptr(dt), 8, _npix(x), C, st)
        return dx, dt, None


def gate3_pool(x, t, out=None):
    return _Gate3Pool.apply(x, t, None if out is None else [out])


class _BcastGate(Function):
    @staticmethod
    def forward(ctx, a, gl):
        a, lda = _nhwc(a); gl, ldg = _nhwc(gl)
        C = a.shape[3]
        out = torch.empty(a.shape, dtype=a.dtype, device=a.device)
        lib().call("egm_bcast_gate_fwd", dtype_code(a.dtype), ptr(a), lda, ptr(gl), ldg, ptr(out), C, _npix(a), C, stream())
        ctx.save_for_backward(a, gl)
        return out

    @staticmethod
    def backward(ctx, g):
        a, gl = ctx.saved_tensors
        a, lda = _nhwc(a); gl, ldgl = _nhwc(gl); g, ldg = _nhwc(g)
        C = a.shape[3]
        da = torch.empty(a.shape, dtype=a.dtype, device=a.device)
        dgl = torch.empty(gl.shape[:3] + (8,), dtype=a.dtype, device=a.device)
        lib().call("egm_bcast_gate_bwd", dtype_code(a.dtype), ptr(g), ldg, ptr(a), lda, ptr(gl), ldgl, ptr(da), C, ptr(dgl), 8, _npix(a), C,
                   stream())
        return da, dgl


def bcast_gate(a, gl):
    return _BcastGate.apply(a, gl)


class _Gelu(Function):
    @staticmethod
    def forward(ctx, x):
        x, ldx = _nhwc(x)
        C = x.shape[3]
        out = torch.empty(x.shape, dtype=x.dtype, device=x.device)
        lib().call("egm_gelu_fwd", dtype_code(x.dtype), ptr(x), ldx, ptr(out), C, _npix(x), C, stream())
        ctx.save_for_backward(x)
        return out

    @staticmethod
    def backward(ctx, g):
        (x,) = ctx.saved_tensors
        x, ldx = _nhwc(x); g, ldg = _nhwc(g)
        C = x.shape[3]
        dx = torch.empty(x.shape, dtype=x.dtype, device=x.device)
        lib().call("egm_gelu_bwd", dtype_code(x.dtype), ptr(g), ldg, ptr(x), ldx, ptr(dx), C, _npix(x), C, stream())
        return dx


def gelu(x):
    return _Gelu.apply(x)


class _Act(Function):

    @staticmethod
    def forward(ctx, x, act):
        x, ldx = _nhwc(x)
        C = x.shape[3]
        coef = torch.zeros((4, C), dtype=torch.float32, device=x.device)
        lib().call("egm_fill_f32", ptr(coef[0]), 1.0, C, stream())
        out = torch.empty(x.shape, dtype=x.dtype, device=x.device)
        lib().call("egm_bn_act_fwd", dtype_code(x.dtype), ptr(x), ldx, ptr(coef[0]), ptr(coef[1]), act, ptr(out), C, _npix(x), C, stream())
        ctx.save_for_backward(x, coef)
        ctx.act = act
        return out

    @staticmethod
    def backward(ctx, g):
        x, coef = ctx.saved_tensors
        x, ldx = _nhwc(x); g, ldg = _nhwc(g)
        C = x.shape[3]
        dx = torch.empty(x.shape, dtype=x.dtype, device=x.device)
        lib().call("egm_bn_act_bwd_apply", dtype_code(x.dtype), ptr(g), ldg, ptr(x), ldx, ptr(coef[0]), ptr(coef[1]), ptr(coef[2]),
                   ptr(coef[3]), ctx.act, 0, ptr(coef[2]), ptr(dx), C, _npix(x), C, stream())
        return dx, None


def act(x, code):
    return _Act.apply(x, code)


class _ChanMeanMax(Function):
    @staticmethod
    def forward(ctx, x, c_real):
        x, ldx = _nhwc(x)
        out = torch.empty(x.shape[:3] + (8,), dtype=x.dtype, device=x.device)
        lib().call("egm_chan_meanmax_fwd", dtype_code(x.dtype), ptr(x), ldx, ptr(out), 8, _npix(x), x.shape[3], c_real, stream())
        ctx.save_for_backward(x)
        ctx.c_real = c_real
        return out

    @staticmethod
    def backward(ctx, g):
        (x,) = ctx.saved_tensors
        x, ldx = _nhwc(x); g, ldg = _nhwc(g)
        dx = torch.empty(x.shape, dtype=x.dtype, device=x.device)
        lib().call("egm_chan_meanmax_bwd", dtype_code(x.dtype), ptr(g), ldg, ptr(x), ldx, ptr(dx), x.shape[3], _npix(x), x.shape[3], ctx.c_real,
                   stream())
        return dx, None


def chan_meanmax(x, c_real):
    return _ChanMeanMax.apply(x, c_real)


class _GlobalAvgMax(Function):

    @staticmethod
    def forward(ctx, x):
        x, ldx = _nhwc(x)
        N, H, W, C = x.shape
        L = lib()
        out = torch.empty((2 * N, 1, 1, C), dtype=x.dtype, device=x.device)
        argidx = torch.empty((N, C), dtype=torch.int32, device=x.device)
        ws = torch.empty(L.query("egm_global_pool_workspace", N, H * W, C) // 4 + 4, dtype=torch.float32, device=x.device)
        L.call("egm_global_avgmax_fwd", dtype_code(x.dtype), ptr(x), ldx, ptr(out), ptr(argidx), ptr(ws), N, H * W, C, stream())
        ctx.save_for_backward(argidx)
        ctx.shape = (N, H, W, C)
        return out

    @staticmethod
    def backward(ctx, g):
        (argidx,) = ctx.saved_tensors
        N, H, W, C = ctx.shape
        g = g.contiguous()
        dx = torch.empty((N, H, W, C), dtype=g.dtype, device=g.device)
        lib().call("egm_global_avgmax_bwd", dtype_code(g.dtype), ptr(g), ptr(argidx), ptr(dx), C, N, H * W, C, stream())
        return dx


def global_avgmax(x):
    return _GlobalAvgMax.apply(x)


class _CaMlp(Function):

    @staticmethod
    def forward(ctx, pooled, w0, w2):
        R, Cp = pooled.shape[0], pooled.shape[3]
        Cr, C = w0.shape[0], w0.shape[1]
        pooled = pooled.contiguous()
        w0c, w2c = w0.detach().contiguous(), w2.detach().contiguous()
        h = torch.empty((R, Cr), dtype=torch.float32, device=pooled.device)
        out = (torch.empty if Cp == C else torch.zeros)((R, 1, 1, Cp), dtype=pooled.dtype, device=pooled.device)
        lib().call("egm_ca_mlp_fwd", dtype_code(pooled.dtype), ptr(pooled), Cp, ptr(w0c), ptr(w2c), ptr(h), ptr(out), Cp, R, C, Cr, stream())
        ctx.save_for_backward(pooled, h, w0c, w2c)
        return out

    @staticmethod
    def backward(ctx, g):
        pooled, h, w0, w2 = ctx.saved_tensors
        R, Cp = pooled.shape[0], pooled.shape[3]
        Cr, C = w0.shape[0], w0.shape[1]
        g = g.contiguous()
        dw0, dw2 = torch.empty_like(w0), torch.empty_like(w2)
        dp = (torch.empty if Cp == C else torch.zeros)(pooled.shape, dtype=pooled.dtype, device=pooled.device)
        lib().call("egm_ca_mlp_bwd", dtype_code(pooled.dtype), ptr(g), Cp, ptr(pooled), Cp, ptr(h), ptr(w0), ptr(w2), ptr(dw0), ptr(dw2),
                   ptr(dp), Cp, R, C, Cr, stream())
        return dp, dw0, dw2


def ca_mlp(pooled, w0, w2):
    return _CaMlp.apply(pooled, w0, w2)


class _FusionCombine(Function):

    @staticmethod
    def forward(ctx, f, s, sa, ca):
        f, ldf = _nhwc(f); s, lds = _nhwc(s); sa, ldsa = _nhwc(sa)
        ca = ca.contiguous()
        N, H, W, C = f.shape
        out = torch.empty(f.shape, dtype=f.dtype, device=f.device)
        lib().call("egm_fusion_combine_fwd", dtype_code(f.dtype), ptr(f), ldf, ptr(s), lds, ptr(sa), ldsa, ptr(ca), ptr(out), C, N, H * W, C,
                   stream())
        ctx.save_for_backward(s, sa, ca)
        return out

    @staticmethod
    def backward(ctx, g):
        s, sa, ca = ctx.saved_tensors
        s, lds = _nhwc(s); sa, ldsa = _nhwc(sa); g, ldg = _nhwc(g)
        N, H, W, C = s.shape
        L, dev = lib(), s.device
        ds = torch.empty(s.shape, dtype=s.dtype, device=dev)
        dsa = torch.empty((N, H, W, 8), dtype=s.dtype, device=dev)
        nb = L.query("egm_fusion_combine_blocks", H * W, C)
        part = _f32((N, nb, 2, C), dev)
        L.call("egm_fusion_combine_bwd", dtype_code(s.dtype), ptr(g), ldg, ptr(s), lds, ptr(sa), ldsa, ptr(ca), ptr(ds), C, ptr(dsa), 8,
               ptr(part), N, H * W, C, stream())
        red = _f32((N, 2, C), dev)
        L.call("egm_reduce_tiles_batched", ptr(part), N, nb, C, ptr(red), stream())
        dca = torch.empty((2 * N, 1, 1, C), dtype=s.dtype, device=dev)
        _f32_rows_to_act(red, dca, N, C)
        return g, ds, dsa, dca


def _f32_rows_to_act(red, dca, N, C):
    lib().call("egm_rows_dup", dtype_code(dca.dtype), ptr(red), ptr(dca), C, N, C, stream())


def fusion_combine(f, s, sa, ca):
    return _FusionCombine.apply(f, s, sa, ca)


def _register_pack(weight, dtype, wf, wd):
    key = (weight.data_ptr(), weight._version, _weight_generation[0], dtype, 1, tuple(weight.shape))
    _pack_cache[id(weight)] = (key, wf, wd, weakref.ref(weight))


class _Fold2(Function):
    @staticmethod
    def forward(ctx, w, pack_dtype, pre=None):
        rows, K2 = w.shape[0], w.shape[1]
        K = K2 // 2
        ctx.real = w
        if pre is not None:
            _Fold2.packs = (pre[2], pre[3])
            return pre[0].detach()
        out = torch.empty((rows, K, 1, 1), dtype=torch.float32, device=w.device)
        if pack_dtype is None:
            lib().call("egm_fold2_fwd", ptr(w.detach().contiguous()), ptr(out), rows, K, stream())
            _Fold2.packs = None
        else:
            wf = torch.empty((1, pad8(rows), pad8(K)), dtype=pack_dtype, device=w.device)
            wd = torch.empty((1, pad8(K), pad8(rows)), dtype=pack_dtype, device=w.device)
            lib().call("egm_fold2_pack", dtype_code(pack_dtype), ptr(w.detach().contiguous()), ptr(out), ptr(wf), ptr(wd), rows, K, stream())
            _Fold2.packs = (wf, wd)
        return out

    @staticmethod
    def backward(ctx, g):
        rows, K = g.shape[0], g.shape[1]
        pend = _take_derived(g)
        if pend is not None:
            dw = _unfilled((rows, 2 * K, 1, 1), g.device)
            _attach_derived(pend, (ctx.real,), (dw,))
            return dw, None, None
        _no_open_standin((ctx.real,))
        dw = torch.empty((rows, 2 * K, 1, 1), dtype=torch.float32, device=g.device)
        lib().call("egm_fold2_bwd", ptr(g.contiguous()), ptr(dw), rows, K, stream())
        return dw, None, None


def fold2(w, pack_dtype=None):
    out = _Fold2.apply(w, pack_dtype, _prepacked((w,), pack_dtype) if pack_dtype is not None else None)
    if pack_dtype is not None and _Fold2.packs is not None:
        _register_pack(out, pack_dtype, *_Fold2.packs)
        _Fold2.packs = None
    _register_derived(out, "fold2", (w,))
    return out


class _SpreadCols(Function):

    @staticmethod
    def forward(ctx, w, real):
        rows, st = w.shape[0], stream()
        tot_r, tot_p = sum(real), sum(pad8(c) for c in real)
        out = torch.zeros((rows, tot_p, 1, 1), dtype=torch.float32, device=w.device)
        wc = w.detach().contiguous()
        o_r = o_p = 0
        for c in real:
            lib().call("egm_copy_cols_f32", ptr(wc), tot_r, o_r, ptr(out), tot_p, o_p, rows, c, st)
            o_r, o_p = o_r + c, o_p + pad8(c)
        ctx.real = tuple(real)
        return out

    @staticmethod
    def backward(ctx, g):
        real = ctx.real
        rows, st = g.shape[0], stream()
        tot_r, tot_p = sum(real), sum(pad8(c) for c in real)
        gc = g.contiguous()
        dw = torch.empty((rows, tot_r, 1, 1), dtype=torch.float32, device=g.device)
        o_r = o_p = 0
        for c in real:
            lib().call("egm_copy_cols_f32", ptr(gc), tot_p, o_p, ptr(dw), tot_r, o_r, rows, c, st)
            o_r, o_p = o_r + c, o_p + pad8(c)
        return dw, None


def spread_cols(w, real):
    return _SpreadCols.apply(w, real)


class _Merge357(Function):
    @staticmethod
    def forward(ctx, w3, w5, w7, b3, b5, b7, pack_dtype, pre=None):
        Co, Ci = w7.shape[0], w7.shape[1]
        ctx.shape = (Co, Ci)
        ctx.real = (w3, w5, w7, b3, b5, b7)
        if pre is not None:
            _Merge357.packs = (pre[2], pre[3])
            return pre[0].detach(), pre[1].detach()
        w = torch.empty((Co, Ci, 7, 7), dtype=torch.float32, device=w7.device)
        b = torch.empty((Co,), dtype=torch.float32, device=w7.device)
        args = (ptr(w3.detach().contiguous()), ptr(w5.detach().contiguous()), ptr(w7.detach().contiguous()), ptr(b3.detach()),
                ptr(b5.detach()), ptr(b7.detach()), ptr(w), ptr(b))
        if pack_dtype is None:
            lib().call("egm_merge357_fwd", *args, Co, Ci, stream())
            _Merge357.packs = None
        else:
            wf = torch.empty((49, pad8(Co), pad8(Ci)), dtype=pack_dtype, device=w7.device)
            wd = torch.empty((49, pad8(Ci), pad8(Co)), dtype=pack_dtype, device=w7.device)
            lib().call("egm_merge357_pack", dtype_code(pack_dtype), *args, ptr(wf), ptr(wd), Co, Ci, stream())
            _Merge357.packs = (wf, wd)
        return w, b

    @staticmethod
    def backward(ctx, gw, gb):
        Co, Ci = ctx.shape
        dev = gw.device
        w3, w5, w7, b3, b5, b7 = ctx.real
        pw = _take_derived(gw)
        if pw is not None:
            d3, d5, d7 = _unfilled((Co, Ci, 3, 3), dev), _unfilled((Co, Ci, 5, 5), dev), _unfilled((Co, Ci, 7, 7), dev)
            _attach_derived(pw, (w7, w5, w3), (d7, d5, d3))
            if gb is None or not any(ctx.needs_input_grad[3:6]):
                return d3, d5, d7, None, None, None, None, None
            pb = _take_derived(gb)
            if pb is None:
                raise RuntimeError("egm_unet_amd: merge357 received a deferred weight gradient with a bias gradient that is not")
            gb3 = _unfilled((3, Co), dev)
            rows = (gb3[0], gb3[1], gb3[2])
            _attach_derived(pb, (b3, b5, b7), rows)
            return d3, d5, d7, rows[0], rows[1], rows[2], None, None
        _no_open_standin(ctx.real)
        d3 = torch.empty((Co, Ci, 3, 3), dtype=torch.float32, device=dev)
        d5 = torch.empty((Co, Ci, 5, 5), dtype=torch.float32, device=dev)
        d7 = torch.empty((Co, Ci, 7, 7), dtype=torch.float32, device=dev)
        gb3 = None
        if gb is not None:
            gb3 = torch.empty((3, Co), dtype=torch.float32, device=dev)
        lib().call("egm_merge357_bwd", ptr(gw.contiguous()), ptr(d3), ptr(d5), ptr(d7), ptr(gb), ptr(gb3), Co, Ci, stream())
        if gb3 is None:
            return d3, d5, d7, None, None, None, None, None
        return d3, d5, d7, gb3[0], gb3[1], gb3[2], None, None


def merge357(w3, w5, w7, b3, b5, b7, pack_dtype=None):
    reals = (w3, w5, w7, b3, b5, b7)
    w, b = _Merge357.apply(*reals, pack_dtype, _prepacked(reals, pack_dtype) if pack_dtype is not None else None)
    if pack_dtype is not None and _Merge357.packs is not None:
        _register_pack(w, pack_dtype, *_Merge357.packs)
        _Merge357.packs = None
    _register_derived(w, "merge357", (w7, w5, w3))
    _register_derived(b, "bias3", (b3, b5, b7))
    return w, b


class _DwConv3(Function):

    @staticmethod
    def forward(ctx, x, w, b, scale):
        x, ldx = _nhwc(x)
        N, H, W, C = x.shape
        y = torch.empty((N, H, W, C), dtype=x.dtype, device=x.device)
        wd, bd, sd = w.detach().contiguous(), b.detach().contiguous(), scale.detach().reshape(1).contiguous()
        lib().call("egm_dwconv3_fwd", dtype_code(x.dtype), ptr(x), ldx, ptr(wd), ptr(bd), ptr(sd), ptr(y), C, N, H, W, C, stream())
        ctx.save_for_backward(x, wd, bd, sd)
        return y

    @staticmethod
    def backward(ctx, g):
        x, w, b, sc = ctx.saved_tensors
        x, ldx = _nhwc(x); g, ldg = _nhwc(g)
        N, H, W, C = x.shape
        L, dev = lib(), x.device
        dx = torch.empty(x.shape, dtype=x.dtype, device=dev)
        dw = torch.empty((C, 1, 3, 3), dtype=torch.float32, device=dev)
        db = torch.empty((C,), dtype=torch.float32, device=dev)
        ds = torch.empty((1,), dtype=torch.float32, device=dev)
        ws = torch.empty(L.query("egm_dwconv3_bwd_workspace", N, H, W, C) // 4 + 4, dtype=torch.float32, device=dev)
        L.call("egm_dwconv3_bwd", dtype_code(x.dtype), ptr(x), ldx, ptr(g), ldg, ptr(w), ptr(b), ptr(sc), ptr(dx), C, ptr(dw), ptr(db), ptr(ds),
               ptr(ws), N, H, W, C, stream())
        return dx, dw, db, ds.reshape(())


def dwconv3(x, w, b, scale):
    return _DwConv3.apply(x, w, b, scale)


class _ConvTPack(Function):

    @staticmethod
    def forward(ctx, w):
        Cin, Cout = w.shape[0], w.shape[1]
        CoutP = pad8(Cout)
        w4 = torch.empty((4 * CoutP, Cin, 1, 1), dtype=torch.float32, device=w.device)
        lib().call("egm_convT2x2_pack", ptr(w.detach().contiguous()), ptr(w4), Cin, Cout, CoutP, 1, stream())
        ctx.shape = tuple(w.shape)
        return w4

    @staticmethod
    def backward(ctx, g):
        Cin, Cout = ctx.shape[0], ctx.shape[1]
        dw = torch.empty(ctx.shape, dtype=torch.float32, device=g.device)
        lib().call("egm_convT2x2_pack", ptr(dw), ptr(g.contiguous()), Cin, Cout, pad8(Cout), 0, stream())
        return dw


class _Shuffle2x2(Function):
    @staticmethod
    def forward(ctx, y4, bias, C, Ho, Wo):
        y4, ld4 = _nhwc(y4)
        N, H, W, _ = y4.shape
        CP = pad8(C)
        oy, ox = (Ho - 2 * H) // 2, (Wo - 2 * W) // 2
        out = torch.empty((N, Ho, Wo, CP), dtype=y4.dtype, device=y4.device)
        lib().call("egm_shuffle2x2_fwd", dtype_code(y4.dtype), ptr(y4), ld4, ptr(bias.detach() if bias is not None else None), C, ptr(out), CP,
                   N, H, W, CP, Ho, Wo, oy, ox, stream())
        ctx.meta = (N, H, W, CP, Ho, Wo, oy, ox, C, bias is not None)
        return out

    @staticmethod
    def backward(ctx, g):
        N, H, W, CP, Ho, Wo, oy, ox, C, has_bias = ctx.meta
        g, ldg = _nhwc(g)
        d4 = torch.empty((N, H, W, 4 * CP), dtype=g.dtype, device=g.device)
        lib().call("egm_shuffle2x2_bwd", dtype_code(g.dtype), ptr(g), ldg, ptr(d4), 4 * CP, N, H, W, CP, Ho, Wo, oy, ox, stream())
        db = None
        if has_bias and ctx.needs_input_grad[1]:
            db4 = _channel_sum(d4)[0]
            db = _fold4(db4, CP)[:C]
        return d4, db, None, None, None


def _fold4(v, CP):
    t = v.reshape(1, 1, 4, CP)
    a = _axpby(t[:, :, 0:1], 1.0, t[:, :, 1:2], 1.0)
    b = _axpby(t[:, :, 2:3], 1.0, t[:, :, 3:4], 1.0)
    return _axpby(a, 1.0, b, 1.0).reshape(CP)


def conv_transpose2x2(x, convT, out_hw):
    w4 = _ConvTPack.apply(convT.weight)
    y4 = conv2d(x, w4)
    return _Shuffle2x2.apply(y4, convT.bias, convT.weight.shape[1], out_hw[0], out_hw[1])


@torch.no_grad()
def hegdc_edge_features(x, c_real):
    x, ldx = _nhwc(x)
    N, H, W, _ = x.shape
    L = lib()
    ws = torch.empty(L.query("egm_hegdc_edge_workspace", N, H, W) // 4 + 4, dtype=torch.float32, device=x.device)
    feats = torch.empty((N, H, W, 8), dtype=x.dtype, device=x.device)
    L.call("egm_hegdc_edge_features", dtype_code(x.dtype), ptr(x), ldx, c_real, ptr(feats), ptr(ws), N, H, W, stream())
    return feats


class _ScaleSigmoid(Function):

    @staticmethod
    def forward(ctx, w, den):
        wc = w.detach().contiguous()
        out = torch.empty_like(wc)
        lib().call("egm_scale_sigmoid_fwd", ptr(wc), ptr(den.detach()), ptr(out), wc.numel(), stream())
        ctx.save_for_backward(wc, den)
        return out

    @staticmethod
    def backward(ctx, g):
        w, den = ctx.saved_tensors
        g = g.contiguous()
        dw, dden = torch.empty_like(w), torch.empty_like(den, dtype=torch.float32)
        part = _f32(256, w.device)
        lib().call("egm_scale_sigmoid_bwd", ptr(g), ptr(w), ptr(den.detach()), ptr(dw), ptr(dden), ptr(part), w.numel(), stream())
        return dw, dden.reshape(den.shape)


def scale_sigmoid(w, den):
    return _ScaleSigmoid.apply(w, den)


class _Mul2Scalar(Function):

    @staticmethod
    def forward(ctx, a, b, alpha):
        a, lda = _nhwc(a); b, ldb = _nhwc(b)
        out = torch.empty(a.shape, dtype=a.dtype, device=a.device)
        al = alpha.detach().reshape(1).float()
        lib().call("egm_mul2_scalar_fwd", dtype_code(a.dtype), ptr(a), lda, ptr(b), ldb, ptr(al), ptr(out), a.shape[3], _npix(a), a.shape[3], stream())
        ctx.save_for_backward(a, b, al)
        ctx.ashape = alpha.shape
        return out

    @staticmethod
    def backward(ctx, g):
        a, b, al = ctx.saved_tensors
        a, lda = _nhwc(a); b, ldb = _nhwc(b); g, ldg = _nhwc(g)
        C = a.shape[3]
        da = torch.empty(a.shape, dtype=a.dtype, device=a.device)
        db = torch.empty(b.shape, dtype=b.dtype, device=b.device) if ctx.needs_input_grad[1] else None
        dalpha, part = _f32(1, a.device), _f32(1024, a.device)
        lib().call("egm_mul2_scalar_bwd", dtype_code(a.dtype), ptr(g), ldg, ptr(a), lda, ptr(b), ldb, ptr(al), ptr(da), C, ptr(db), C, ptr(dalpha),
                   ptr(part), _npix(a), C, stream())
        return da, db, dalpha.reshape(ctx.ashape)


def mul2_scalar(a, b, alpha):
    return _Mul2Scalar.apply(a, b, alpha)


class _ELA(Function):
    @staticmethod
    def forward(ctx, x, conv_w, gamma, beta, groups, eps):
# ... 144 lines not shown
```

include/egm_hip.h:

```cpp
#ifndef EGM_HIP_H
#define EGM_HIP_H

#ifdef __cplusplus
extern "C" {
#endif

typedef void* egm_stream_t;

enum egm_status { EGM_OK = 0, EGM_ERR_ARG = -1, EGM_ERR_LAUNCH = -2, EGM_ERR_UNSUPPORTED = -3 };
enum egm_dtype { EGM_F32 = 0, EGM_BF16 = 1 };
enum egm_act { EGM_ACT_NONE = 0, EGM_ACT_RELU = 1, EGM_ACT_SIGMOID = 2, EGM_ACT_SILU = 3  };

int egm_version(void);
const char* egm_last_error(void);
int egm_device_ok(void);

int egm_nchw_to_nhwc(int dtype, const void* src_f32, void* dst, int ld, int N, int C, int H, int W, egm_stream_t s);
int egm_nhwc_to_nchw(int dtype, const void* src, int ld, void* dst_f32, int N, int C, int H, int W, egm_stream_t s);

int egm_conv_pack(int dtype, const void* w_oihw_f32, void* wf, void* wd, int Cout, int Cin, int KH, int KW, int groups,
                  egm_stream_t s);
int egm_conv_pack_chunk(void);
int egm_conv_pack_multi(int dtype, const void* table_dev, int n, long long total_chunks, egm_stream_t s);
int egm_group_begin(void);
int egm_group_end(egm_stream_t s);
int egm_group_abort(void);
int egm_conv_tile_mode(int mode);
int egm_conv_tile_debug(int dbg);
int egm_conv_c7_mode(int mode);
int egm_conv_split_ok(int dtype, int N, int H, int W, int Cin, int Cout, int KH, int KW, int dil, int csplit);
int egm_conv_fwd_split(int dtype, const void* x, int ldx, const void* wf, void* y, int ldy, void* y2, int ldy2, int csplit, int N,
                       int H, int W, int Cin, int Cout, int KH, int KW, int dil, egm_stream_t s);
int egm_conv_kernel_name(int dtype, int N, int H, int W, int Cin, int Cout, int KH, int KW, int dil, char* buf, int buflen);
int egm_conv_fwd(int dtype, const void* x, int ldx, const void* wf, const void* bias_f32, int bias_n, void* y, int ldy,
                 float* stats, int N, int H, int W, int Cin, int Cout, int KH, int KW, int dil, egm_stream_t s);
int egm_conv_stats_tiles(int dtype, int N, int H, int W, int Cin, int Cout, int KH, int KW, int dil);
int egm_conv_fwd_act(int dtype, const void* x, int ldx, const void* wf, const void* bias_f32, int bias_n, void* y, int ldy, int N, int H,
                     int W, int Cin, int Cout, int KH, int KW, int dil, int act, egm_stream_t s);
int egm_conv_fold_chunk(void);
int egm_conv_fold_pack_multi(int dtype, const void* table_dev, int n, long long total_chunks, egm_stream_t s);
int egm_argmax_u8(const float* logits, const unsigned char* lut, unsigned char* out, int N, int C, int H, int W, egm_stream_t s);
long long egm_conv_wgrad_workspace(int N, int H, int W, int Cin, int Cout, int KH, int KW);
int egm_conv_wgrad(int dtype, const void* x, int ldx, const void* dy, int lddy, float* dw_oihw_f32, void* workspace,
                   int N, int H, int W, int Cin, int Cout, int CinR, int CoutR, int KH, int KW, int dil, int groups,
                   int accumulate, egm_stream_t s);
int egm_conv_wgrad_kernel_name(int dtype, int N, int H, int W, int Cin, int Cout, int KH, int KW, int dil, char* buf, int buflen);
#define EGM_WGRAD_MULTI_MAX 4
typedef struct egm_conv_wgrad_desc {
    const void* x; const void* dy; void* slabs;
    int ldx, lddy, N, H, W, Cin, Cout, Cin_real, Cout_real, KH, KW, dil, groups, pad_;
} egm_conv_wgrad_desc;
int egm_conv_wgrad_multi(int dtype, const egm_conv_wgrad_desc* descs, int n, egm_stream_t stream);
int egm_conv_wgrad_slabs(int dtype, int N, int H, int W, int Cin, int Cout, int KH, int KW, int dil);
int egm_wgrad_reduce(const float* slabs, float* dw_oihw_f32, int nslab, int taps, int CoutP, int CinP, int CoutR, int CinR, int groups,
                     int accumulate, egm_stream_t s);
int egm_wgrad_reduce_chunk(void);
int egm_wgrad_reduce_chunk_wide(void);
int egm_wgrad_reduce_is_wide(int nslab, int taps, int CoutP, int CinP);
int egm_wgrad_reduce_multi(const void* table_dev, int n, long long total_chunks, egm_stream_t s);
int egm_dwconv3_fwd(int dtype, const void* x, int ldx, const float* w, const float* b, const float* scale, void* y, int ldy,
                    int N, int H, int W, int C, egm_stream_t s);
long long egm_dwconv3_bwd_workspace(int N, int H, int W, int C);
int egm_dwconv3_bwd(int dtype, const void* x, int ldx, const void* dy, int lddy, const float* w, const float* b,
                    const float* scale, void* dx, int lddx, float* dw, float* db, float* dscale, void* workspace,
                    int N, int H, int W, int C, egm_stream_t s);

int egm_channel_partials_blocks(long long npix, int C);
int egm_channel_sums(int dtype, const void* x, int ld, long long npix, int C, float* partials, egm_stream_t s);
int egm_reduce_tiles(const float* tiles, int ntiles, int C, float* out_2xC, egm_stream_t s);
int egm_reduce_tiles_batched(const float* tiles, int batch, int ntiles, int C, float* out, egm_stream_t s);
typedef struct { const void* x; float* part; float* out; long long npix; int ld, C, Cout, nblk, chunk0, pad; } egm_bsum_entry;
int egm_bias_grad_multi(int dtype, const void* table_dev, int n, long long blocks1, long long blocks2, egm_stream_t s);

int egm_bn_finalize(const float* stats, int ntiles, long long count, const float* gamma, const float* beta, float eps,
                    float momentum, float* running_mean, float* running_var, float* scale, float* shift,
                    float* save_mean, float* save_rstd, int C, int C_real, egm_stream_t s);
int egm_bn_eval_coeffs(const float* gamma, const float* beta, const float* running_mean, const float* running_var,
                       float eps, float* scale, float* shift, float* save_mean, float* save_rstd, int C, int C_real,
                       egm_stream_t s);
int egm_bn_act_fwd(int dtype, const void* y, int ldy, const float* scale, const float* shift, int act, void* z, int ldz,
                   long long npix, int C, egm_stream_t s);
int egm_bn_act_bwd_reduce(int dtype, const void* dz, int lddz, const void* y, int ldy, const float* scale,
                          const float* shift, const float* save_mean, const float* save_rstd, int act, float* partials,
                          long long npix, int C, egm_stream_t s);
int egm_bn_act_bwd_apply(int dtype, const void* dz, int lddz, const void* y, int ldy, const float* scale,
                         const float* shift, const float* save_mean, const float* save_rstd, int act, int train,
                         const float* sums, void* dy, int lddy, long long npix, int C, egm_stream_t s);
int egm_bn_act_cls_fwd(int dtype, const void* y, int ldy, const float* scale, const float* shift, int act, void* z, int ldz,
                       const float* w_cls, int nc, int ldw, const float* bias, float* logits_nchw, int N, int H, int W, int C,
                       egm_stream_t s);
int egm_bn_cls_bwd_reduce(int dtype, const void* dlogits, int lddl, const float* w_cls, int nc, int ldw, const void* y, int ldy,
                          const float* scale, const float* shift, const float* save_mean, const float* save_rstd, int act,
                          float* partials, long long npix, int C, egm_stream_t s);
int egm_bn_cls_bwd_apply(int dtype, const void* dlogits, int lddl, const float* w_cls, int nc, int ldw, const void* y, int ldy,
                         const float* scale, const float* shift, const float* save_mean, const float* save_rstd, int act, int train,
                         const float* sums, void* dy, int lddy, long long npix, int C, egm_stream_t s);
int egm_bn_mca_bwd_reduce(int dtype, const void* dxo, int ldd, const float* gates, const float* coef, int no_spatial, const void* y,
                          int ldy, const float* scale, const float* shift, const float* save_mean, const float* save_rstd, int act,
                          float* partials, int N, int H, int W, int C, egm_stream_t s);
int egm_bn_mca_bwd_apply(int dtype, const void* dxo, int ldd, const float* gates, const float* coef, int no_spatial, const void* y,
                         int ldy, const float* scale, const float* shift, const float* save_mean, const float* save_rstd, int act,
                         int train, const float* sums, void* dy, int lddy, int N, int H, int W, int C, egm_stream_t s);
int egm_bn_bwd_coefs(const float* partials, int ntiles, long long count, const float* scale, const float* shift,
                     const float* save_mean, const float* save_rstd, int train, float* sums_2xC, float* cf_4xC, int C,
                     egm_stream_t s);

#define EGM_BN_MULTI_MAX 4
enum egm_bn_multi_pass { EGM_BN_MULTI_FINALIZE = 0, EGM_BN_MULTI_FWD = 1, EGM_BN_MULTI_BWD_REDUCE = 2, EGM_BN_MULTI_BWD_COEFS = 3,
                         EGM_BN_MULTI_BWD_APPLY = 4 };
typedef struct egm_bn_desc {
    const void* y;  void* z;  const void* dz;  void* dy;
    float* coef;
    const float* stats;
    const float* gamma;  const float* beta;  float* running_mean;  float* running_var;
    float* partials;  float* sums;  float* cf4;
    long long npix;
    int ldy, ldz, lddz, lddy, ntiles, nblocks, C, C_real, act, train;
    float eps, momentum;
} egm_bn_desc;
int egm_bn_multi(int dtype, int pass, const egm_bn_desc* descs, int n, egm_stream_t s);

enum egm_ew_mode { EGM_EW_GATE = 0, EGM_EW_SAR = 1 };
int egm_bn_ew_fwd(int dtype, int mode, const void* y, int ldy, const float* scale, const float* shift, int act, const void* p,
                  int ldp, float alpha, void* out, int ldo, long long npix, int C, egm_stream_t s);
int egm_bn_ew_bwd_reduce(int dtype, int mode, const void* g, int ldg, const void* q, int ldq, const void* y, int ldy,
                         const float* scale, const float* shift, const float* save_mean, const float* save_rstd, int act,
                         float alpha, float* partials, long long npix, int C, egm_stream_t s);
int egm_bn_ew_bwd_apply(int dtype, int mode, const void* g, int ldg, const void* q, int ldq, const void* y, int ldy,
                        const float* cf_4xC, int act, float alpha, void* dy, int lddy, void* dp, int lddp, long long npix, int C,
                        egm_stream_t s);

typedef struct egm_conv1x1_bwd_desc {
    const void* x;  const void* dy;  const void* wd;  void* dx;  float* slabs;
    long long npix;
    int ldx, lddy, lddx, Cin, Cout, pad_;
} egm_conv1x1_bwd_desc;
int egm_conv1x1_bwd_supported(int dtype, int Cin, int Cout);
int egm_conv1x1_bwd_slabs(long long npix);
int egm_conv1x1_bwd(int dtype, const egm_conv1x1_bwd_desc* descs, int n, egm_stream_t s);

int egm_maxpool2_fwd(int dtype, const void* x, int ldx, void* y, int ldy, int N, int H, int W, int C, egm_stream_t s);
int egm_maxpool2_bwd(int dtype, const void* x, int ldx, const void* dy, int lddy, void* dx, int lddx, int N, int H, int W,
                     int C, egm_stream_t s);
int egm_maxpool2_bwd_add(int dtype, const void* x, int ldx, const void* dy, int lddy, const void* add, int ldadd, void* dx, int lddx,
                         int N, int H, int W, int C, egm_stream_t s);
int egm_bn_act_fwd_pool(int dtype, const void* y, int ldy, const float* scale, const float* shift, int act, void* z, int ldz,
                        void* pooled, int ldp, int N, int H, int W, int C, egm_stream_t s);
int egm_bn_pool_bwd_blocks(int N, int H, int W, int C);
int egm_bn_pool_bwd_reduce(int dtype, const void* gskip, int ldgs, const void* gpool, int ldgp, const void* y, int ldy,
                           const float* scale, const float* shift, const float* save_mean, const float* save_rstd, int act,
                           float* partials, int N, int H, int W, int C, egm_stream_t s);
int egm_bn_pool_bwd_apply(int dtype, const void* gskip, int ldgs, const void* gpool, int ldgp, const void* y, int ldy,
                          const float* scale, const float* shift, const float* save_mean, const float* save_rstd, int act, int train,
                          const float* sums, void* dy, int lddy, int N, int H, int W, int C, egm_stream_t s);
int egm_gate3_fwd_pool(int dtype, const void* x, int ldx, const void* t, int ldt, void* out, int ldo, void* pooled, int ldp, int N,
                       int H, int W, int C, egm_stream_t s);
int egm_gate3_pool_bwd(int dtype, const void* gskip, int ldgs, const void* gpool, int ldgp, const void* x, int ldx, const void* t,
                       int ldt, void* dx, int lddx, void* dt, int lddt, int N, int H, int W, int C, egm_stream_t s);
int egm_upcat_fwd(int dtype, const void* skip, int lds, const void* low, int ldl, void* out, int ldo, int N, int Hs, int Ws,
                  int Cs, int Hl, int Wl, int Cl, egm_stream_t s);
int egm_bn_act_hp_fwd(int dtype, const void* y, int ldy, const float* scale, const float* shift, int act, void* z, int ldz,
                      void* edge, int lde, int N, int H, int W, int C, egm_stream_t s);
int egm_bn_act_upcat_fwd(int dtype, const void* skip, int lds, const void* low, int ldl, const float* scale, const float* shift,
                         int act, void* out, int ldo, int N, int Hs, int Ws, int Cs, int Hl, int Wl, int Cl, egm_stream_t s);
int egm_upcat_bwd_low(int dtype, const void* dout, int ldo, void* dlow, int ldl, int N, int Hs, int Ws, int Cs, int Hl,
                      int Wl, int Cl, egm_stream_t s);

int egm_axpby(int dtype, const void* a, int lda, float alpha, const void* b, int ldb, float beta, void* out, int ldo,
              long long npix, int C, egm_stream_t s);
int egm_sum4(int dtype, const void* a, int lda, const void* b, int ldb, const void* c, int ldc, const void* d, int ldd, void* out,
             int ldo, long long npix, int C, egm_stream_t s);
int egm_sum4_hp(int dtype, const void* a, int lda, const void* b, int ldb, const void* c, int ldc, const void* d, int ldd, void* out,
                int ldo, int N, int H, int W, int C, egm_stream_t s);
int egm_vec_add_f32(float* y, const float* x, long long n, egm_stream_t s);
int egm_fill_f32(float* y, float v, long long n, egm_stream_t s);
int egm_copy_cols_f32(const float* src, int ld_src, int col0_src, float* dst, int ld_dst, int col0_dst, int rows, int ncols,
                      egm_stream_t s);

int egm_highpass3(int dtype, const void* x, int ldx, void* out, int ldo, int N, int H, int W, int C, egm_stream_t s);
int egm_gate_mul_fwd(int dtype, const void* x, int ldx, const void* w, int ldw, void* out, int ldo, long long npix, int C,
                     egm_stream_t s);
int egm_gate_mul_bwd(int dtype, const void* g, int ldg, const void* x, int ldx, const void* w, int ldw, void* dx, int lddx,
                     void* dw, int lddw, long long npix, int C, egm_stream_t s);

int egm_scale_add_relu_fwd(int dtype, const void* a, int lda, float alpha, const void* b, int ldb, void* out, int ldo,
                           long long npix, int C, egm_stream_t s);
int egm_scale_add_relu_bwd(int dtype, const void* g, int ldg, const void* out, int ldo, float alpha, void* da, int ldda,
                           void* db, int lddb, long long npix, int C, egm_stream_t s);
int egm_gate3_fwd(int dtype, const void* x, int ldx, const void* t, int ldt, void* out, int ldo, long long npix, int C,
                  egm_stream_t s);
int egm_gate3_bwd(int dtype, const void* g, int ldg, const void* x, int ldx, const void* t, int ldt, void* dx, int lddx,
                  void* dt, int lddt, long long npix, int C, egm_stream_t s);

int egm_bcast_gate_fwd(int dtype, const void* a, int lda, const void* gl, int ldgl, void* out, int ldo, long long npix, int C,
                       egm_stream_t s);
int egm_bcast_gate_bwd(int dtype, const void* g, int ldg, const void* a, int lda, const void* gl, int ldgl, void* da, int ldda,
                       void* dgl, int lddgl, long long npix, int C, egm_stream_t s);
int egm_gelu_fwd(int dtype, const void* x, int ldx, void* out, int ldo, long long npix, int C, egm_stream_t s);
int egm_gelu_bwd(int dtype, const void* g, int ldg, const void* x, int ldx, void* dx, int lddx, long long npix, int C,
                 egm_stream_t s);

int egm_chan_meanmax_fwd(int dtype, const void* x, int ldx, void* out, int ldo, long long npix, int C, int C_real,
                         egm_stream_t s);
int egm_chan_meanmax_bwd(int dtype, const void* g, int ldg, const void* x, int ldx, void* dx, int lddx, long long npix, int C,
                         int C_real, egm_stream_t s);
int egm_sa_conv7_fwd(int dtype, const void* x, int ldx, const float* w, void* y, int ldy, int N, int H, int W, egm_stream_t s);
long long egm_sa_conv7_bwd_workspace(int N, int H, int W);
int egm_sa_conv7_bwd(int dtype, const void* x, int ldx, const void* dy, int lddy, const float* w, void* dx, int lddx, float* dw,
                     void* workspace, int N, int H, int W, egm_stream_t s);
long long egm_global_pool_workspace(int N, long long HW, int C);
int egm_global_avgmax_fwd(int dtype, const void* x, int ldx, void* out, int* argidx, void* workspace, int N, long long HW,
                          int C, egm_stream_t s);
int egm_global_avgmax_bwd(int dtype, const void* gout, const int* argidx, void* dx, int lddx, int N, long long HW, int C,
                          egm_stream_t s);
int egm_rows_dup(int dtype, const float* red, void* dst, int ldd, int N, int C, egm_stream_t s);
int egm_ca_mlp_fwd(int dtype, const void* pooled, int ldp, const float* w0, const float* w2, float* h, void* logits, int ldo, int R,
                   int C, int Cr, egm_stream_t s);
int egm_ca_mlp_bwd(int dtype, const void* dlogits, int ldd, const void* pooled, int ldp, const float* h, const float* w0,
                   const float* w2, float* dw0, float* dw2, void* dpooled, int lddp, int R, int C, int Cr, egm_stream_t s);
int egm_fusion_combine_fwd(int dtype, const void* f, int ldf, const void* sv, int lds, const void* sa, int ldsa, const void* ca,
                           void* out, int ldo, int N, long long HW, int C, egm_stream_t s);
int egm_fusion_combine_blocks(long long HW, int C);
int egm_fusion_combine_bwd(int dtype, const void* g, int ldg, const void* sv, int lds, const void* sa, int ldsa, const void* ca,
                           void* ds, int ldds, void* dsa, int lddsa, float* partials, int N, long long HW, int C, egm_stream_t s);
int egm_fold2_fwd(const float* w, float* out, int rows, int K, egm_stream_t s);
int egm_fold2_bwd(const float* g, float* dw, int rows, int K, egm_stream_t s);
int egm_merge357_fwd(const float* w3, const float* w5, const float* w7, const float* b3, const float* b5, const float* b7,
                     float* w, float* b, int Co, int Ci, egm_stream_t s);
int egm_merge357_bwd(const float* gw, float* d3, float* d5, float* d7, const float* gb, float* gb3, int Co, int Ci, egm_stream_t s);
int egm_fold2_pack(int dtype, const float* w, float* out, void* wf, void* wd, int rows, int K, egm_stream_t s);
int egm_merge357_pack(int dtype, const float* w3, const float* w5, const float* w7, const float* b3, const float* b5, const float* b7,
                      float* w, float* b, void* wf, void* wd, int Co, int Ci, egm_stream_t s);

long long egm_mca_reduce_workspace(int N, int H, int W, int C);
int egm_mca_reduce(int dtype, int mode, const void* a, int lda, const void* b, int ldb, float* sums, void* workspace, int N,
                   int H, int W, int C, egm_stream_t s);
int egm_mca_reduce_bn(int dtype, const void* y, int ldy, const float* scale, const float* shift, int act, void* z, int ldz,
                      float* sums, void* workspace, int N, int H, int W, int C, egm_stream_t s);
int egm_mca_gates_fwd(const float* sums, const float* w_h, const float* k_h, int ks_h, const float* w_w, const float* k_w,
                      int ks_w, const float* w_c, const float* k_c, int ks_c, float* stats, float* o, float* gates, int N, int H,
                      int W, int C, egm_stream_t s);
int egm_mca_gates_bwd(const float* dG, const float* stats, const float* o, const float* gates, const float* w_h, const float* k_h,
                      int ks_h, const float* w_w, const float* k_w, int ks_w, const float* w_c, const float* k_c, int ks_c,
                      float* dz_scratch, float* coef, float* dwts, float* dks, int N, int H, int W, int C, egm_stream_t s);
int egm_mca_xout(int dtype, const void* x, int ldx, const float* gates, void* xo, int ldo, int N, int H, int W, int C,
                 int no_spatial, egm_stream_t s);
int egm_mca_stencil1(int dtype, const void* xo, int ld, void* r1, int ldr, void* u2, int ldu, unsigned char* codes, int N, int H,
                     int W, int C, egm_stream_t s);
int egm_add_avg3(int dtype, const void* a, int lda, const void* b, int ldb, float scale, void* out, int ldo, int N, int H, int W,
                 int C, egm_stream_t s);
int egm_mca_fused_fwd(int dtype, const void* x, int ldx, const float* gates, void* xo, int ldxo, void* out, int ldo, unsigned char* codes,
                      int N, int H, int W, int C, int no_spatial, egm_stream_t s);
int egm_mca_bwd_du(int dtype, const void* xo, int ld, const void* g, int ldg, void* du, int ldd, int N, int H, int W, int C,
                   egm_stream_t s);
int egm_mca_bwd_dxo(int dtype, const unsigned char* codes, const void* g, int ldg, const void* du, int ldd, void* dxo, int ldo,
                    int N, int H, int W, int C, egm_stream_t s);
int egm_mca_bwd_dudxo(int dtype, const unsigned char* codes, const void* xo, int ldxo, const void* g, int ldg, void* dxo, int ldo,
                      int N, int H, int W, int C, egm_stream_t s);
int egm_mca_bwd_dx(int dtype, const void* dxo, int ldd, const void* x, int ldx, const float* gates, const float* coef, void* dx,
                   int ldo, int N, int H, int W, int C, int no_spatial, egm_stream_t s);

int egm_gemm(int dtype, const void* A, int lda, const void* B, int ldb, int transB, void* C, int ldc, int c_is_f32,
             const float* bias, int act, const void* R, int ldr, float alpha, int M, int N, int K, int nb1, int nb2,
             long long sA1, long long sA2, long long sB1, long long sB2, long long sC1, long long sC2, long long sR1,
             long long sR2, egm_stream_t s);
int egm_gemm_kernel_name(int dtype, int transB, int c_is_f32, int M, int N, int K, int lda, int ldb, int ldc, int ldr, int batch,
                         char* buf, int buflen);
int egm_gemm_dma_mode(int mode);
int egm_attention_fused(int dtype, const void* qkv, int ld, int B, int L, int H, int head_dim, int mode, void* out, int ldo,
                        egm_stream_t s);
int egm_softmax_rows(int dtype, const float* S, int lds, void* P, int ldp, long long rows, int L, int causal, int accumulate,
                     egm_stream_t s);
int egm_layernorm(int dtype, const void* x, int ldx, const float* gamma, const float* beta, float eps, void* y, int ldy,
                  long long rows, int D, egm_stream_t s);
int egm_patchify(int dtype, const float* img_nchw, void* out, int B, int C, int H, int W, int P, egm_stream_t s);
int egm_vit_assemble(int dtype, const void* tok, const float* cls, const float* pos, void* x, int B, int Ltok, int D, egm_stream_t s);
int egm_text_embed(int dtype, const int* tokens, const float* emb, const float* pos, const float* pos_res, int split, void* x,
                   int n, int L, int D, egm_stream_t s);
int egm_film(int dtype, void* a, const void* mul, const void* add, int B, int L, int D, egm_stream_t s);
int egm_gather_rows(int dtype, const void* x, const int* idx, void* out, int n, int L, int D, egm_stream_t s);
int egm_pixel_shuffle(int dtype, const void* y, int ldy, int tok_off, int Ltot, const float* bias, float* out, int B, int g,
                      int P, egm_stream_t s);
int egm_cast_f32(int dtype, const float* src, void* dst, long long n, egm_stream_t s);

long long egm_loss_workspace(int N, int C);
int egm_loss_fwd(const float* logits, const long long* target, const float* class_weight, int N, int C, int H, int W,
                 long long ignore_index, int dice, float* loss6, float* workspace, unsigned char* signs, egm_stream_t s);
int egm_loss_bwd(const float* logits, const long long* target, const float* class_weight, int N, int C, int H, int W,
                 long long ignore_index, int dice, const float* workspace, const unsigned char* signs, const float* grad_out,
                 float* dlogits, egm_stream_t s);
int egm_argmax_hist(const float* logits, const long long* target, int N, int C, int H, int W, long long dice_ignore_index,
                    unsigned long long* hist, unsigned long long* counts, long long* pred, egm_stream_t s);
int egm_metrics_finalize(const unsigned long long* hist, const unsigned long long* counts, int N, int C, float* out,
                         egm_stream_t s);
int egm_ensemble_fuse(const float* clip_logits, const float* unet_logits, float alpha, int N, int C, int hc, int wc, int H, int W,
                      long long* pred, float* fused, egm_stream_t s);
int egm_ensemble_alpha_hist(const float* clip_logits, const float* unet_logits, const long long* target, const float* alphas, int na,
                            int N, int C, int hc, int wc, int H, int W, unsigned long long* hist, egm_stream_t s);
int egm_ensemble_miou(const unsigned long long* hist, int na, int C, float* miou, egm_stream_t s);
int egm_sgd_chunk(void);
int egm_sgd_multi(const void* table_dev, int ntensors, long long total_chunks, const float* lr_dev, float lr, float momentum,
                  float weight_decay, float grad_scale, int first_step, egm_stream_t s);
int egm_copy_multi(const void* table_dev, int ntensors, egm_stream_t s);

int egm_convT2x2_pack(float* w_iohw, float* w4, int Cin, int Cout, int CoutP, int to_packed, egm_stream_t s);
int egm_shuffle2x2_fwd(int dtype, const void* y4, int ld4, const float* bias, int bias_n, void* out, int ldo, int N, int H, int W, int C,
                       int Ho, int Wo, int oy, int ox, egm_stream_t s);
int egm_shuffle2x2_bwd(int dtype, const void* g, int ldg, void* d4, int ld4, int N, int H, int W, int C, int Ho, int Wo, int oy, int ox,
                       egm_stream_t s);

int egm_ela_strip_means(int dtype, const void* x, int ldx, float* mh, float* mw, int N, int H, int W, int C, egm_stream_t s);
int egm_ela_gates_fwd(const float* mh, const float* mw, const float* conv_w, int ks, const float* gamma, const float* beta, float eps,
                      float* yh, float* yw, float* gh, float* gw, float* stats, int N, int H, int W, int C, int groups, egm_stream_t s);
int egm_ela_apply(int dtype, const void* x, int ldx, const float* gh, const float* gw, void* out, int ldo, int N, int H, int W, int C,
                  egm_stream_t s);
long long egm_ela_bwd_workspace(int N, int H, int W, int C, int ks);
int egm_ela_bwd(int dtype, const void* g, int ldg, const void* x, int ldx, const float* mh, const float* mw, const float* yh, const float* yw,
                const float* gh, const float* gw, const float* stats, const float* conv_w, int ks, const float* gamma, void* dx, int lddx,
                float* dconv_w, float* dgamma, float* dbeta, float* workspace, int N, int H, int W, int C, int groups, egm_stream_t s);

long long egm_hegdc_edge_workspace(int N, int H, int W);
int egm_hegdc_edge_features(int dtype, const void* x, int ldx, int C_real, void* feats, float* workspace, int N, int H, int W,
                            egm_stream_t s);
int egm_scale_sigmoid_fwd(const float* w, const float* den, float* out, long long n, egm_stream_t s);
int egm_scale_sigmoid_bwd(const float* g, const float* w, const float* den, float* dw, float* dden, float* partials, long long n,
                          egm_stream_t s);
int egm_mul2_scalar_fwd(int dtype, const void* a, int lda, const void* b, int ldb, const float* alpha, void* out, int ldo, long long npix,
                        int C, egm_stream_t s);
int egm_mul2_scalar_bwd(int dtype, const void* g, int ldg, const void* a, int lda, const void* b, int ldb, const float* alpha, void* da,
                        int ldda, void* db, int lddb, float* dalpha, float* partials, long long npix, int C, egm_stream_t s);

int egm_resample_u8(const void* src, int H, int W, int C, void* dst, int axis, int out_size, const int* bounds, const int* coefs,
                    int ksize, egm_stream_t s);
int egm_gather_u8(const void* src, int H, int W, int C, void* dst, int Ho, int Wo, const int* yidx, const int* xidx, egm_stream_t s);
int egm_augment_u8(const void* img_hwc3, const void* mask_hw, int H, int W, int hflip, int vflip, int top, int left, int crop_h,
                   int crop_w, const float* mean3_host, const float* std3_host, float* out_img_chw, long long* out_target,
                   int out_h, int out_w, egm_stream_t s);

int egm_clip_preprocess_u8(const void* img_hwc3, int H, int W, float* out_chw, int Sh, int Sw, const int* xbounds, const float* xweights,
                           int xksize, const int* ybounds, const float* yweights, int yksize, const float* mean3_host,
                           const float* std3_host, float* tmp_chw, egm_stream_t s);
int egm_ensemble_mask_u8(const float* clip_logits, const float* unet_logits, const float* alpha_dev, int N, int C, int hc, int wc, int H,
                         int W, const int* yidx, const int* xidx, const unsigned char* lut, unsigned char* out, int H0, int W0,
                         egm_stream_t s);

int egm_unet_preprocess_batch_u8(const void* imgs_bhwc3, int B, int H, int W, float* out_bchw, int oh, int ow, const int* xbounds,
                                 const int* xcoefs, int xksize, const int* ybounds, const int* ycoefs, int yksize,
                                 const float* mean3_host, const float* std3_host, void* tmp_bhwc3, egm_stream_t s);
int egm_clip_preprocess_batch_u8(const void* imgs_bhwc3, int B, int H, int W, float* out_bchw, int Sh, int Sw, const int* xbounds,
                                 const float* xweights, int xksize, const int* ybounds, const float* yweights, int yksize,
                                 const float* mean3_host, const float* std3_host, float* tmp_cbhw, egm_stream_t s);

int egm_mask_confusion_u8(const unsigned char* pred, const unsigned char* label, long long npix, const unsigned char* pred_cls,
                          const unsigned char* label_cls, int C, unsigned long long* hist, egm_stream_t s);
int egm_ensemble_alpha_hist_u8(const float* clip_logits, const float* unet_logits, const unsigned char* labels,
                               const unsigned char* label_cls, const float* alphas, int na, int N, int C, int hc, int wc, int H, int W,
                               int Hl, int Wl, const int* ybeg, const int* xbeg, unsigned long long* hist, egm_stream_t s);

long long egm_sweep_chunk(void);
int egm_sweep_hist(const float* scores, int N, int C, int c_pos, int c_neg, long long HW, const void* target, int target_f32,
                   const unsigned char* target_cls, const float* cuts_host, const float* cuts_dev, int T, unsigned long long* hist,
                   egm_stream_t s);
int egm_score_mask_u8(const float* scores, int N, int C, int c_pos, int c_neg, long long HW, float cut, int v_bg, int v_fg,
                      unsigned char* out, egm_stream_t s);

long long egm_ccl_workspace(int N, int H, int W);
int egm_ccl_label_u8(const unsigned char* cls, int N, int H, int W, int connectivity, int* labels, int* areas, void* workspace,
                     egm_stream_t s);
int egm_mask_clean_u8(const unsigned char* cls, int N, int H, int W, int connectivity, const int* params_dev, void* workspace,
                      unsigned char* out_cls, const int* yidx, const int* xidx, const unsigned char* lut, unsigned char* out, int H0,
                      int W0, egm_stream_t s);

long long egm_boundary_workspace(int N, int H, int W);
int egm_mask_boundary_u8(const unsigned char* pred, const unsigned char* label, int N, int H, int W, int radius,
                         const unsigned char* pred_cls, const unsigned char* label_cls, int C, void* workspace,
                         unsigned long long* counts, unsigned char* band_pred, unsigned char* band_label, egm_stream_t s);

long long egm_contour_workspace(int N, int H, int W, int C);
int egm_mask_boundary_euclid_u8(const unsigned char* pred, const unsigned char* label, int N, int H, int W, int radius,
                                const unsigned char* pred_cls, const unsigned char* label_cls, int C, void* workspace,
                                unsigned long long* counts, unsigned char* band_pred, unsigned char* band_label, egm_stream_t s);
int egm_mask_contour_f_u8(const unsigned char* pred, const unsigned char* label, int N, int H, int W, int radius,
                          const unsigned char* pred_cls, const unsigned char* label_cls, int C, void* workspace,
                          unsigned long long* counts, unsigned char* contour_pred, unsigned char* contour_label, egm_stream_t s);

long long egm_surface_workspace(int N, int H, int W, int C);
int egm_mask_surface_dist_u8(const unsigned char* pred, const unsigned char* label, int N, int H, int W,
                             const unsigned char* pred_cls, const unsigned char* label_cls, int C, void* workspace,
                             unsigned long long* counts, int* d2_pred, int* d2_label, egm_stream_t s);

int egm_tile_gather_f32(const float* src, int N, int C, int H, int W, const int* ys_dev, int ny, const int* xs_dev, int nx, int h, int w,
                        int t0, int count, float* dst, egm_stream_t s);
int egm_tile_blend_f32(const float* tiles, int N, int C, int H, int W, const int* ys_dev, int ny, const int* xs_dev, int nx, int h, int w,
                       const float* wy_dev, const float* wx_dev, const unsigned char* lut, float* logits_out, unsigned char* mask_out,
                       egm_stream_t s);

typedef struct egm_tta_view {
    const float* logits;
    const int* yi;
    const float* yl;
    const int* xi;
    const float* xl;
    int h, w, flip, pad;
} egm_tta_view;
int egm_tta_views_f32(const float* src, int N, int C, int H, int W, int h, int w, const int* yi_dev, const float* yl_dev,
                      const int* xi_dev, const float* xl_dev, const int* flips_dev, int F, float* dst, egm_stream_t s);
int egm_tta_merge_f32(const egm_tta_view* views_dev, int V, int N, int C, int H, int W, int mode, const unsigned char* lut,
                      float* logits_out, unsigned char* mask_out, egm_stream_t s);

typedef struct egm_train_desc {
    const void* img;
    const void* mask;
    int H, W, oh, ow;
    int hflip, vflip, top, left;
    int crop_h, crop_w, r0, nr;
    int c0, nc, y0, ny;
    int xksize, yksize;
    long long ws_off;
    int xb_off, xc_off, yb_off, yc_off, xnn_off, ynn_off;
} egm_train_desc;
int egm_train_batch_u8(const egm_train_desc* table_dev, int B, int slot_h, int slot_w, int max_crop_h, int max_crop_w,
                       float* out_img_bchw, long long* out_target_bhw, const float* mean3_host, const float* std3_host,
                       void* workspace, long long workspace_bytes, long long max_hpass_pixels, egm_stream_t s);

int egm_transpose(int dtype, const void* src, int rows, int cols, int ld_src, long long batch_stride_src, void* dst, int ld_dst,
                  long long batch_stride_dst, int batch, egm_stream_t s);
int egm_relu_bwd(int dtype, const void* g, const void* out, void* dst, long long n, egm_stream_t s);
int egm_softmax_bwd_rows(int dtype, const void* P, int ldp, const float* dP, int lddp, void* dS, int ldds, long long rows, int L,
                         float alpha, egm_stream_t s);
int egm_layernorm_bwd_blocks(long long rows);
int egm_layernorm_bwd(int dtype, const void* x, int ldx, const void* g, int ldg, const float* gamma, float eps, void* dx, int lddx,
                      float* partials, long long rows, int D, egm_stream_t s);
int egm_film_fwd(int dtype, const void* a, const void* mul, const void* add, void* out, int B, int L, int D, egm_stream_t s);
int egm_film_bwd(int dtype, const void* g, const void* a, const void* mul, void* da, void* dmul, void* dadd, int B, int L, int D,
                 egm_stream_t s);
int egm_pixel_unshuffle(int dtype, const float* dout, void* dy, int B, int g, int P, int tok_off, int Ltot, egm_stream_t s);
int egm_sum_f32(const float* x, long long n, float scale, float* partials, float* out, egm_stream_t s);
int egm_bce_logits_fwd(const float* x, const float* t, long long n, float* partials, float* loss, egm_stream_t s);
int egm_bce_logits_bwd(const float* x, const float* t, const float* grad_out, long long n, float* dx, egm_stream_t s);
int egm_adamw_chunk(void);
int egm_adamw_multi(const void* table_dev, int ntensors, long long total_chunks, float lr, float beta1, float beta2, float eps,
                    float weight_decay, int step, egm_stream_t s);

int egm_dropout(int dtype, const void* x, const void* residual, void* out, long long n, float p, unsigned long long seed,
                egm_stream_t s);
int egm_attn_mask_cls(int dtype, void* probs, int ldp, long long head_stride, const float* mask, int nmask, int nbh, int ntok,
                      egm_stream_t s);

long long egm_refine_packed_elems(int rd, int patch);
long long egm_refine_bwd_workspace(int B, int g, int rd, int patch);
int egm_refine_pack(int dtype, const float* w0, const float* w1, const float* w2, void* packed, int rd, int patch, egm_stream_t s);
int egm_refine_fwd(int dtype, const void* a, int tok_off, int Ltot, const void* packed, const float* b0, const float* b1,
                   const float* b2, void* h, float* out, int B, int g, int rd, int patch, egm_stream_t s);
int egm_refine_bwd(int dtype, const float* dout, const void* a, int tok_off, int Ltot, const void* h, const void* packed,
                   const float* b1, void* da, float* dw0, float* db0, float* dw1, float* db1, float* dw2, float* db2,
                   void* workspace, int B, int g, int rd, int patch, egm_stream_t s);

int egm_baseline_supported(int rd, int rd2, int patch);
long long egm_baseline_packed_elems(int rd, int rd2, int patch);
long long egm_baseline_bwd_workspace(int B, int g, int rd, int rd2, int patch);
int egm_baseline_pack(int dtype, const float* w_red, const float* w1, const float* w2, const float* wt, void* packed, int rd, int rd2,
                      int patch, egm_stream_t s);
int egm_baseline_fwd(int dtype, const void* x, int tok_off, int Ltot, const void* mul, const void* add, const void* packed,
                     const float* b_red, const float* b1, const float* b2, const float* bt, void* u, void* h, float* out, int B, int g,
                     int rd, int rd2, int patch, egm_stream_t s);
int egm_baseline_bwd(int dtype, const float* dout, const void* u, const void* h, const void* mul, const void* add, const void* packed,
                     const float* b2, void* du, int tok_off, int Ltot, float* dwt, float* dbt, float* dw2, float* db2, float* dw1,
                     float* db1, void* dmul, void* dadd, void* workspace, int B, int g, int rd, int rd2, int patch, egm_stream_t s);
int egm_baseline_fwd_multi(int dtype, const void* x, int tok_off, int Ltot, const void* mul, const void* add, const void* packed,
                           const float* b_red, const float* b1, const float* b2, const float* bt, float* out, int B, int K, int g, int rd,
                           int rd2, int patch, int prompts_per_group, egm_stream_t s);

int egm_film_fanout(int dtype, const void* r, const void* mul, const void* add, void* out, int B, int K, int L, int D, egm_stream_t s);
int egm_bcast_add(int dtype, void* a, const void* r, int B, int K, int L, int D, egm_stream_t s);
int egm_sigmoid_affine(float* x, const float* scale, float offset, int N, int C, long long HW, egm_stream_t s);
int egm_bcast_add_out(int dtype, const void* a, const void* r, void* out, int B, int K, int L, int D, egm_stream_t s);
int egm_group_sum(int dtype, const void* g, void* out, int B, int K, int L, int D, egm_stream_t s);
long long egm_film_fanout_bwd_workspace(int dtype, int B, int K, int L, int D);
int egm_film_fanout_bwd(int dtype, const void* g, const void* r, const void* mul, void* dr, void* dmul, void* dadd, void* ws, int B, int K,
                        int L, int D, egm_stream_t s);

int egm_vprompt_mask_f32(const void* masks_khw, int K, int H, int W, float* m_kss, int S, const int* xbounds, const float* xweights,
                         int xksize, const int* ybounds, const float* yweights, int yksize, const unsigned int* lut8_host, float* tmp_khs,
                         int* box_k4, egm_stream_t s);
int egm_vprompt_blend_f32(const float* x_k3ss, const float* m_kss, float* out_k3ss, int* box_k4, int K, int S, int mode,
                          const float* taps15_host, int blur, float bg_fac, float sub, egm_stream_t s);
int egm_vprompt_crop_f32(const float* src_k3ss, const int* box_k4, float* out_k3ss, int K, int S, int cnum, egm_stream_t s);
int egm_cond_mix_f32(float* out_gd, const float* vis_kd, const int* group_off, const float* text_gd, float w, int G, int K, int D,
                     egm_stream_t s);

long long egm_guided_workspace(int N, int C, int h, int w);
int egm_guided_coefs_f32(const float* guide, const float* scores, const unsigned char* cls, int N, int C, int h, int w, int r, float eps0,
                         float eps1, float eps2, float* A_out, void* workspace, egm_stream_t s);
int egm_guided_apply_u8(const unsigned char* imgs, int N, int H0, int W0, const float* A, int C, int h, int w, const int* yi_dev,
                        const float* yl_dev, const int* xi_dev, const float* xl_dev, float scale0, float scale1, float scale2,
                        float offset0, float offset1, float offset2, const unsigned char* lut, unsigned char* mask_out, float* q_out,
                        egm_stream_t s);
int egm_ensemble_fuse_dev_f32(const float* clip_logits, const float* unet_logits, const float* alpha_dev, int N, int C, int hc, int wc,
                              int H, int W, float* fused, egm_stream_t s);

long long egm_sdf_workspace(int N, int H, int W, int K);
int egm_target_sdf_i64(const long long* target, int N, int H, int W, const int* classes, int K, long long ignore_index, void* workspace,
                       int* s_out, egm_stream_t s);
int egm_sdf_phi_f32(const int* sdf, long long n, float* phi, egm_stream_t s);
long long egm_bloss_workspace(int N, int C, int H, int W);
int egm_bloss_fwd(const float* logits, const int* sdf, const long long* target, const int* classes, int K, int N, int C, int H, int W,
                  long long ignore_index, const float* w_dev, void* workspace, float* out2, egm_stream_t s);
int egm_bloss_bwd(const float* logits, const int* sdf, const int* classes, int K, int N, int C, int H, int W, const void* workspace,
                  const float* grad_out, const float* w_dev, float* dlogits, egm_stream_t s);

long long egm_sort_pairs_workspace(int S, long long L);
int egm_sort_pairs_u32(const unsigned int* keys, const unsigned int* vals, int S, long long L, int begin_bit, int end_bit, void* workspace,
                       unsigned int* keys_out, unsigned int* vals_out, egm_stream_t s);

long long egm_lovasz_workspace(int N, int C, int H, int W, int K, int per_image);
int egm_lovasz_errors(const float* logits, const long long* target, const int* classes, int K, int N, int C, int H, int W,
                      long long ignore_index, int per_image, unsigned int* keys, unsigned int* vals, float* e_out, egm_stream_t s);
int egm_lovasz_coefs(const float* logits, const long long* target, const int* classes, int K, int N, int C, int H, int W,
                     long long ignore_index, int per_image, void* workspace, float* e_out, float* coef, egm_stream_t s);
int egm_lovasz_fwd(const float* logits, const long long* target, const int* classes, int K, int N, int C, int H, int W,
                   long long ignore_index, int per_image, int present, const float* w_dev, void* workspace, float* coef, float* out2,
                   egm_stream_t s);
int egm_lovasz_bwd(const float* logits, const float* coef, const int* classes, int K, int N, int C, int H, int W, int per_image,
                   const void* workspace, const float* grad_out, const float* w_dev, float* dlogits, egm_stream_t s);

long long egm_lovasz_hinge_workspace(int N, int H, int W, int per_image);
int egm_lovasz_hinge_errors(const float* logits, const void* target, int target_f32, int N, int C, int c_pos, int c_neg, int H, int W,
// ... 22 lines not shown
```

Before: 704.6 images/s.

## Fuse FusionConv spatial and channel attention into one autograd node with shared launches

Refactors the attention kernels into device-body functions and adds combined kernels that split a single grid by block ranges (AttnCut), so independent spatial-attention and channel-attention work runs in one launch. The forward/backward pair goes from 16 launches to 8 in the bf16 7x7 case. It also folds an add into chan_meanmax backward. The aim is to cut launch count and tail idle time on small kernels, in exchange for more complex code and heterogeneous blocks inside one launch that may load-balance worse.

After: 711.3 images/s (median of 6 runs). No clear change (+1.0%).

```diff
diff --git a/egm_unet_amd/csrc/blocks.hip b/egm_unet_amd/csrc/blocks.hip
--- a/egm_unet_amd/csrc/blocks.hip
+++ b/egm_unet_amd/csrc/blocks.hip
@@ -1,5 +1,6 @@
 #include "common.h"
 #include "derived_pack.h"
+#include "group.h"
 
 namespace {
 
@@ -208,11 +209,12 @@
 }
 
 template <typename T, int GROUP>
-__global__ void chan_meanmax_fwd_kernel(const T* __restrict__ x, int ldx, T* __restrict__ out, int ldo, long long npix, int C, int Creal) {
+__device__ __forceinline__ void chan_meanmax_fwd_body(const T* __restrict__ x, int ldx, T* __restrict__ out, int ldo, long long npix, int C,
+                                                      int Creal, int bid, int nb) {
     const int ncv = C >> 3;
     const int ppb = 256 / GROUP;
     const int lane_in = threadIdx.x % GROUP, slot = threadIdx.x / GROUP;
-    for (long long p0 = (long long)blockIdx.x * ppb; p0 < npix; p0 += (long long)gridDim.x * ppb) {
+    for (long long p0 = (long long)bid * ppb; p0 < npix; p0 += (long long)nb * ppb) {
         const long long p = p0 + slot;
         float s = 0.f, m = -INFINITY;
         if (p < npix)
@@ -233,12 +235,17 @@
     }
 }
 template <typename T, int GROUP>
-__global__ void chan_meanmax_bwd_kernel(const T* __restrict__ g, int ldg, const T* __restrict__ x, int ldx, T* __restrict__ dx, int lddx,
-                                        long long npix, int C, int Creal) {
+__global__ void chan_meanmax_fwd_kernel(const T* __restrict__ x, int ldx, T* __restrict__ out, int ldo, long long npix, int C, int Creal) {
+    chan_meanmax_fwd_body<T, GROUP>(x, ldx, out, ldo, npix, C, Creal, blockIdx.x, gridDim.x);
+}
+template <typename T, int GROUP, bool ADD>
+__device__ __forceinline__ void chan_meanmax_bwd_body(const T* __restrict__ g, int ldg, const T* __restrict__ x, int ldx, T* __restrict__ dx,
+                                                      int lddx, const T* __restrict__ add, int ldadd, long long npix, int C, int Creal,
+                                                      int bid, int nb) {
     const int ncv = C >> 3;
     const int ppb = 256 / GROUP;
     const int lane_in = threadIdx.x % GROUP, slot = threadIdx.x / GROUP;
-    for (long long p0 = (long long)blockIdx.x * ppb; p0 < npix; p0 += (long long)gridDim.x * ppb) {
+    for (long long p0 = (long long)bid * ppb; p0 < npix; p0 += (long long)nb * ppb) {
         const long long p = p0 + slot;
         float m = -INFINITY; int am = 0x7fffffff;
         if (p < npix)
@@ -259,25 +266,36 @@
                 float o[8];
 #pragma unroll
                 for (int j = 0; j < 8; ++j) o[j] = (cv * 8 + j < Creal) ? gm + ((cv * 8 + j == am) ? gx : 0.f) : 0.f;
+                if constexpr (ADD) {
+                    float u[8];
+                    load8(add + p * ldadd + cv * 8, u);
+#pragma unroll
+                    for (int j = 0; j < 8; ++j) o[j] = to_f32(from_f32<T>(o[j])) + u[j];
+                }
                 store8(dx + p * lddx + cv * 8, o);
             }
         }
     }
 }
-
-template <typename T>
-__global__ __launch_bounds__(256) void global_pool_partial_kernel(const T* __restrict__ x, int ldx, long long HW, int C,
-                                                                  float* __restrict__ part, int* __restrict__ part_idx) {
+template <typename T, int GROUP>
+__global__ void chan_meanmax_bwd_kernel(const T* __restrict__ g, int ldg, const T* __restrict__ x, int ldx, T* __restrict__ dx, int lddx,
+                                        long long npix, int C, int Creal) {
+    chan_meanmax_bwd_body<T, GROUP, false>(g, ldg, x, ldx, dx, lddx, nullptr, 0, npix, C, Creal, blockIdx.x, gridDim.x);
+}
+
+template <typename T>
+__device__ __forceinline__ void global_pool_partial_body(const T* __restrict__ x, int ldx, long long HW, int C, float* __restrict__ part,
+                                                         int* __restrict__ part_idx, int bid, int nb, int n) {
     __shared__ float rs[256 * 8];
     __shared__ float rm[256 * 8];
     __shared__ int ri[256 * 8];
-    const int n = blockIdx.y, ncv = C >> 3, rows = 256 / ncv;
+    const int ncv = C >> 3, rows = 256 / ncv;
     const int tid = threadIdx.x, cv = tid % ncv, row = tid / ncv;
     float s[8], m[8]; int ix[8];
 #pragma unroll
     for (int j = 0; j < 8; ++j) { s[j] = 0.f; m[j] = -INFINITY; ix[j] = 0x7fffffff; }
     if (row < rows)
-        for (long long p = (long long)blockIdx.x * rows + row; p < HW; p += (long long)gridDim.x * rows) {
+        for (long long p = (long long)bid * rows + row; p < HW; p += (long long)nb * rows) {
             float v[8];
             load8(x + ((long long)n * HW + p) * ldx + cv * 8, v);
 #pragma unroll
@@ -293,15 +311,20 @@
             ss += rs[k];
             if (rm[k] > mm || (rm[k] == mm && ri[k] < ii)) { mm = rm[k]; ii = ri[k]; }
         }
-        const long long o = ((long long)n * gridDim.x + blockIdx.x) * 2 * C;
+        const long long o = ((long long)n * nb + bid) * 2 * C;
         part[o + c] = ss; part[o + C + c] = mm;
-        part_idx[((long long)n * gridDim.x + blockIdx.x) * C + c] = ii;
-    }
-}
-template <typename T>
-__global__ __launch_bounds__(64) void global_pool_final_kernel(const float* __restrict__ part, const int* __restrict__ part_idx, int nblk, int N,
-                                                               long long HW, int C, T* __restrict__ out, int* __restrict__ argidx) {
-    const int n = blockIdx.y, c = blockIdx.x, lane = threadIdx.x;
+        part_idx[((long long)n * nb + bid) * C + c] = ii;
+    }
+}
+template <typename T>
+__global__ __launch_bounds__(256) void global_pool_partial_kernel(const T* __restrict__ x, int ldx, long long HW, int C,
+                                                                  float* __restrict__ part, int* __restrict__ part_idx) {
+    global_pool_partial_body<T>(x, ldx, HW, C, part, part_idx, blockIdx.x, gridDim.x, blockIdx.y);
+}
+template <typename T>
+__device__ __forceinline__ void global_pool_final_body(const float* __restrict__ part, const int* __restrict__ part_idx, int nblk, int N,
+                                                       long long HW, int C, T* __restrict__ out, int* __restrict__ argidx, int c, int n,
+                                                       int lane) {
     double ss = 0.0; float mm = -INFINITY; int ii = 0x7fffffff;
     for (int b = lane; b < nblk; b += 64) {
         const long long o = ((long long)n * nblk + b) * 2 * C;
@@ -320,6 +343,11 @@
         out[(long long)(N + n) * C + c] = from_f32<T>(mm);
         argidx[(long long)n * C + c] = ii;
     }
+}
+template <typename T>
+__global__ __launch_bounds__(64) void global_pool_final_kernel(const float* __restrict__ part, const int* __restrict__ part_idx, int nblk, int N,
+                                                               long long HW, int C, T* __restrict__ out, int* __restrict__ argidx) {
+    global_pool_final_body<T>(part, part_idx, nblk, N, HW, C, out, argidx, blockIdx.x, blockIdx.y, threadIdx.x);
 }
 template <typename T>
 __global__ void global_pool_bwd_kernel(const T* __restrict__ gout, const int* __restrict__ argidx, T* __restrict__ dx, int lddx, int N,
@@ -449,13 +477,14 @@
 }
 constexpr int SAF_TY = 16, SAF_TX = 64, SAF_PY = SAF_TY + 6, SAF_PX = SAF_TX + 6;
 template <typename T>
-__global__ __launch_bounds__(256) void sa_conv7_fwd_kernel(const T* __restrict__ x, int ldx, const float* __restrict__ w, T* __restrict__ y, int ldy, int N, int H, int W) {
+__device__ __forceinline__ void sa_conv7_fwd_body(const T* __restrict__ x, int ldx, const float* __restrict__ w, T* __restrict__ y, int ldy, int N,
+                                                  int H, int W, int bid, int nb) {
     __shared__ float2 sx[SAF_PY * SAF_PX];
     __shared__ float sw[98];
     if (threadIdx.x < 98) sw[threadIdx.x] = w[threadIdx.x];
     const int tiles_x = (W + SAF_TX - 1) / SAF_TX, tiles_y = (H + SAF_TY - 1) / SAF_TY, ntiles = N * tiles_x * tiles_y;
     const int tx = threadIdx.x & 63, ty0 = threadIdx.x >> 6;
-    for (int t = blockIdx.x; t < ntiles; t += gridDim.x) {
+    for (int t = bid; t < ntiles; t += nb) {
         const int n = t / (tiles_x * tiles_y), tr = t - n * tiles_x * tiles_y;
         const int y0 = (tr / tiles_x) * SAF_TY, x0 = (tr % tiles_x) * SAF_TX;
         const long long img = (long long)n * H * W;
@@ -486,14 +515,18 @@
     }
 }
 template <typename T>
-__global__ __launch_bounds__(256) void sa_conv7_bwd_data_kernel(const T* __restrict__ dy, int lddy, const float* __restrict__ w, T* __restrict__ dx, int lddx, int N,
-                                                                int H, int W) {
+__global__ __launch_bounds__(256) void sa_conv7_fwd_kernel(const T* __restrict__ x, int ldx, const float* __restrict__ w, T* __restrict__ y, int ldy, int N, int H, int W) {
+    sa_conv7_fwd_body<T>(x, ldx, w, y, ldy, N, H, W, blockIdx.x, gridDim.x);
+}
+template <typename T>
+__device__ __forceinline__ void sa_conv7_bwd_data_body(const T* __restrict__ dy, int lddy, const float* __restrict__ w, T* __restrict__ dx, int lddx,
+                                                       int N, int H, int W, int bid, int nb) {
     __shared__ float sg[SAF_PY * SAF_PX];
     __shared__ float sw[98];
     if (threadIdx.x < 98) sw[threadIdx.x] = w[threadIdx.x];
     const int tiles_x = (W + SAF_TX - 1) / SAF_TX, tiles_y = (H + SAF_TY - 1) / SAF_TY, ntiles = N * tiles_x * tiles_y;
     const int tx = threadIdx.x & 63, ty0 = threadIdx.x >> 6;
-    for (int t = blockIdx.x; t < ntiles; t += gridDim.x) {
+    for (int t = bid; t < ntiles; t += nb) {
         const int n = t / (tiles_x * tiles_y), tr = t - n * tiles_x * tiles_y;
         const int y0 = (tr / tiles_x) * SAF_TY, x0 = (tr % tiles_x) * SAF_TX;
         const long long img = (long long)n * H * W;
@@ -521,10 +554,15 @@
         }
     }
 }
+template <typename T>
+__global__ __launch_bounds__(256) void sa_conv7_bwd_data_kernel(const T* __restrict__ dy, int lddy, const float* __restrict__ w, T* __restrict__ dx, int lddx, int N,
+                                                                int H, int W) {
+    sa_conv7_bwd_data_body<T>(dy, lddy, w, dx, lddx, N, H, W, blockIdx.x, gridDim.x);
+}
 constexpr int SA_TY = 16, SA_TX = 64, SA_PY = SA_TY + 6, SA_PX = SA_TX + 6;
 template <typename T>
-__global__ __launch_bounds__(256) void sa_conv7_bwd_w_kernel(const T* __restrict__ x, int ldx, const T* __restrict__ dy, int lddy,
-                                                             float* __restrict__ part, int N, int H, int W) {
+__device__ __forceinline__ void sa_conv7_bwd_w_body(const T* __restrict__ x, int ldx, const T* __restrict__ dy, int lddy, float* __restrict__ part,
+                                                    int N, int H, int W, int bid, int nb) {
     constexpr int kTileFloats = 2 * SA_PY * SA_PX + SA_TY * SA_TX, kRedFloats = 14 * 257;
     __shared__ __attribute__((aligned(16))) float sbuf[kTileFloats > kRedFloats ? kTileFloats : kRedFloats];
     float2* sx = reinterpret_cast<float2*>(sbuf);
@@ -535,7 +573,7 @@
     for (int k = 0; k < 98; ++k) acc[k] = 0.f;
     const int tiles_x = (W + SA_TX - 1) / SA_TX, tiles_y = (H + SA_TY - 1) / SA_TY, ntiles = N * tiles_x * tiles_y;
     const int tx = threadIdx.x & 63, ty0 = threadIdx.x >> 6;
-    for (int t = blockIdx.x; t < ntiles; t += gridDim.x) {
+    for (int t = bid; t < ntiles; t += nb) {
         const int n = t / (tiles_x * tiles_y), tr = t - n * tiles_x * tiles_y;
         const int y0 = (tr / tiles_x) * SA_TY, x0 = (tr % tiles_x) * SA_TX;
         const long long img = (long long)n * H * W;
@@ -580,17 +618,24 @@
         }
     }
     __syncthreads();
-    if (threadIdx.x < 98) part[(long long)blockIdx.x * 98 + threadIdx.x] = red[0][threadIdx.x];
-}
-__global__ __launch_bounds__(256) void sa_conv7_bwd_w_final_kernel(const float* __restrict__ part, int nblk, float* __restrict__ dw) {
+    if (threadIdx.x < 98) part[(long long)bid * 98 + threadIdx.x] = red[0][threadIdx.x];
+}
+template <typename T>
+__global__ __launch_bounds__(256) void sa_conv7_bwd_w_kernel(const T* __restrict__ x, int ldx, const T* __restrict__ dy, int lddy,
+                                                             float* __restrict__ part, int N, int H, int W) {
+    sa_conv7_bwd_w_body<T>(x, ldx, dy, lddy, part, N, H, W, blockIdx.x, gridDim.x);
+}
+__device__ __forceinline__ void sa_conv7_bwd_w_final_body(const float* __restrict__ part, int nblk, float* __restrict__ dw, int k) {
     __shared__ double red[256];
-    const int k = blockIdx.x;
     double s = 0.0;
     for (int b = threadIdx.x; b < nblk; b += 256) s += (double)part[(long long)b * 98 + k];
     red[threadIdx.x] = s;
     __syncthreads();
     for (int o = 128; o > 0; o >>= 1) { if (threadIdx.x < o) red[threadIdx.x] += red[threadIdx.x + o]; __syncthreads(); }
     if (threadIdx.x == 0) dw[k] = (float)red[0];
+}
+__global__ __launch_bounds__(256) void sa_conv7_bwd_w_final_kernel(const float* __restrict__ part, int nblk, float* __restrict__ dw) {
+    sa_conv7_bwd_w_final_body(part, nblk, dw, blockIdx.x);
 }
 
 inline int group_for(int ncv) { int g = 1; while (g < ncv) g <<= 1; return g; }
@@ -625,11 +670,10 @@
     }
 }
 template <typename T>
-__global__ __launch_bounds__(256) void ca_mlp_bwd_kernel(const T* __restrict__ dl, int ldd, const T* __restrict__ pooled, int ldp,
-                                                         const float* __restrict__ h, const float* __restrict__ w0,
-                                                         const float* __restrict__ w2, float* __restrict__ dw0, float* __restrict__ dw2,
-                                                         T* __restrict__ dpooled, int lddp, int R, int C, int Cr) {
-    extern __shared__ float ca_smem[];
+__device__ __forceinline__ void ca_mlp_bwd_body(const T* __restrict__ dl, int ldd, const T* __restrict__ pooled, int ldp,
+                                                const float* __restrict__ h, const float* __restrict__ w0, const float* __restrict__ w2,
+                                                float* __restrict__ dw0, float* __restrict__ dw2, T* __restrict__ dpooled, int lddp, int R,
+                                                int C, int Cr, float* ca_smem) {
     float* sdl = ca_smem;
     float* sp = sdl + R * C;
     float* sh = sp + R * C;
@@ -671,15 +715,108 @@
         dpooled[(long long)r * lddp + c] = from_f32<T>(a);
     }
 }
-
-template <typename T>
-__global__ __launch_bounds__(256) void rows_dup_kernel(const float* __restrict__ red, T* __restrict__ dst, int ldd, int N, int C) {
-    for (int i = blockIdx.x * 256 + threadIdx.x; i < N * C; i += gridDim.x * 256) {
+template <typename T>
+__global__ __launch_bounds__(256) void ca_mlp_bwd_kernel(const T* __restrict__ dl, int ldd, const T* __restrict__ pooled, int ldp,
+                                                         const float* __restrict__ h, const float* __restrict__ w0,
+                                                         const float* __restrict__ w2, float* __restrict__ dw0, float* __restrict__ dw2,
+                                                         T* __restrict__ dpooled, int lddp, int R, int C, int Cr) {
+    extern __shared__ float ca_smem[];
+    ca_mlp_bwd_body<T>(dl, ldd, pooled, ldp, h, w0, w2, dw0, dw2, dpooled, lddp, R, C, Cr, ca_smem);
+}
+
+template <typename T>
+__device__ __forceinline__ void rows_dup_body(const float* __restrict__ red, T* __restrict__ dst, int ldd, int N, int C, int bid, int nb) {
+    for (int i = bid * 256 + threadIdx.x; i < N * C; i += nb * 256) {
         const int n = i / C, c = i - n * C;
         const T v = from_f32<T>(red[((long long)n * 2) * C + c]);
         dst[(long long)n * ldd + c] = v;
         dst[(long long)(N + n) * ldd + c] = v;
     }
+}
+template <typename T>
+__global__ __launch_bounds__(256) void rows_dup_kernel(const float* __restrict__ red, T* __restrict__ dst, int ldd, int N, int C) {
+    rows_dup_body<T>(red, dst, ldd, N, C, blockIdx.x, gridDim.x);
+}
+
+struct AttnCut { int blk0[4]; int n; };
+
+__device__ __forceinline__ void tiles_reduce_256(const float* __restrict__ st, int ntiles, int C, int c0, float* __restrict__ out) {
+    __shared__ double red[2048];
+    for (int v = 0; v < 4; ++v) {
+        const int tid = threadIdx.x + 256 * v, j = tid & 7, tl = tid >> 3;
+        const int c = c0 + j;
+        double s = 0.0, q = 0.0;
+        if (c < C) {
+            for (int t = tl; t < ntiles; t += 128) {
+                s += (double)st[((long long)t * 2 + 0) * C + c];
+                q += (double)st[((long long)t * 2 + 1) * C + c];
+            }
+        }
+        red[tid] = s; red[1024 + tid] = q;
+    }
+    __syncthreads();
+    for (int stride = 64; stride > 0; stride >>= 1) {
+        for (int v = 0; v < 4; ++v) {
+            const int tid = threadIdx.x + 256 * v, tl = tid >> 3;
+            if (tl < stride) { red[tid] += red[tid + stride * 8]; red[1024 + tid] += red[1024 + tid + stride * 8]; }
+        }
+        __syncthreads();
+    }
+    const int c = c0 + (threadIdx.x & 7);
+    if (threadIdx.x < 8 && c < C) { out[c] = (float)red[threadIdx.x]; out[C + c] = (float)red[1024 + threadIdx.x]; }
+}
+
+template <typename T, int GROUP>
+__global__ __launch_bounds__(256) void fusion_attn_fwd_stats_kernel(AttnCut cut, const T* __restrict__ s, int lds, T* __restrict__ mm, long long npix,
+                                                                    int C, int Creal, const T* __restrict__ f, int ldf, long long HW,
+                                                                    float* __restrict__ part, int* __restrict__ part_idx, int nbp) {
+    EGM_GROUP_MEMBER(cut, i);
+    const int bid = (int)blockIdx.x - cut.blk0[i], nb = cut.blk0[i + 1] - cut.blk0[i];
+    if (i == 0) chan_meanmax_fwd_body<T, GROUP>(s, lds, mm, 8, npix, C, Creal, bid, nb);
+    else global_pool_partial_body<T>(f, ldf, HW, C, part, part_idx, bid % nbp, nbp, bid / nbp);
+}
+template <typename T>
+__global__ __launch_bounds__(256) void fusion_attn_fwd_gates_kernel(AttnCut cut, const T* __restrict__ mm, const float* __restrict__ w, T* __restrict__ sa,
+                                                                    int N, int H, int W, const float* __restrict__ part,
+                                                                    const int* __restrict__ part_idx, int nbp, int C, T* __restrict__ pooled,
+                                                                    int* __restrict__ argidx) {
+    EGM_GROUP_MEMBER(cut, i);
+    const int bid = (int)blockIdx.x - cut.blk0[i], nb = cut.blk0[i + 1] - cut.blk0[i];
+    if (i == 0) sa_conv7_fwd_body<T>(mm, 8, w, sa, 8, N, H, W, bid, nb);
+    else {
+        const int item = bid * 4 + (int)(threadIdx.x >> 6);
+        if (item < N * C) global_pool_final_body<T>(part, part_idx, nbp, N, (long long)H * W, C, pooled, argidx, item % C, item / C, threadIdx.x & 63);
+    }
+}
+template <typename T>
+__global__ __launch_bounds__(256) void fusion_attn_bwd_mid_kernel(AttnCut cut, const float* __restrict__ tiles, int ntiles, int C, float* __restrict__ red,
+                                                                  const T* __restrict__ dsa, const float* __restrict__ w, T* __restrict__ dmm,
+                                                                  const T* __restrict__ mm, float* __restrict__ wpart, int N, int H, int W) {
+    EGM_GROUP_MEMBER(cut, i);
+    const int bid = (int)blockIdx.x - cut.blk0[i], nb = cut.blk0[i + 1] - cut.blk0[i];
+    if (i == 0) {
+        const int cb = (C + 7) / 8, bx = bid % cb, by = bid / cb;
+        tiles_reduce_256(tiles + (long long)by * ntiles * 2 * C, ntiles, C, bx * 8, red + (long long)by * 2 * C);
+    } else if (i == 1) sa_conv7_bwd_data_body<T>(dsa, 8, w, dmm, 8, N, H, W, bid, nb);
+    else sa_conv7_bwd_w_body<T>(mm, 8, dsa, 8, wpart, N, H, W, bid, nb);
+}
+template <typename T, int GROUP>
+__global__ __launch_bounds__(256) void fusion_attn_bwd_tail_kernel(AttnCut cut, const float* __restrict__ red, T* __restrict__ dca, const T* __restrict__ pooled,
+                                                                   const float* __restrict__ h, const float* __restrict__ w0,
+                                                                   const float* __restrict__ w2, float* __restrict__ dw0, float* __restrict__ dw2,
+                                                                   T* __restrict__ dpooled, int N, int C, int Creal, int Cr,
+                                                                   const float* __restrict__ wpart, int nbw, float* __restrict__ dw_sa,
+                                                                   const T* __restrict__ dmm, const T* __restrict__ s, int lds,
+                                                                   const T* __restrict__ ds_b, int ldb, T* __restrict__ ds, long long npix) {
+    extern __shared__ float ca_smem[];
+    EGM_GROUP_MEMBER(cut, i);
+    const int bid = (int)blockIdx.x - cut.blk0[i], nb = cut.blk0[i + 1] - cut.blk0[i];
+    if (i == 0) {
+        rows_dup_body<T>(red, dca, C, N, C, 0, 1);
+        __syncthreads();
+        ca_mlp_bwd_body<T>(dca, C, pooled, C, h, w0, w2, dw0, dw2, dpooled, C, 2 * N, Creal, Cr, ca_smem);
+    } else if (i == 1) sa_conv7_bwd_w_final_body(wpart, nbw, dw_sa, bid);
+    else chan_meanmax_bwd_body<T, GROUP, true>(dmm, 8, s, lds, ds, C, ds_b, ldb, npix, C, Creal, bid, nb);
 }
 
 template <typename T>
@@ -997,3 +1134,85 @@
     EGM_CHECK_LAUNCH("sa_conv7_bwd");
     return EGM_OK;
 }
+
+static AttnCut attn_cut(int a, int b, int c) {
+    AttnCut cut;
+    cut.blk0[0] = 0; cut.blk0[1] = a; cut.blk0[2] = a + b; cut.blk0[3] = a + b + c; cut.n = c > 0 ? 3 : 2;
+    return cut;
+}
+extern "C" int egm_fusion_attn_fwd_stats(int dtype, const void* sv, int lds, void* mm, const void* f, int ldf, void* pool_ws, int N, long long HW,
+                                         int C, int C_real, egm_stream_t st) {
+    EGM_REQ_VEC("fusion_attn_fwd_stats", sv, lds, C); EGM_REQ_VEC("fusion_attn_fwd_stats", f, ldf, C); EGM_REQ_VEC("fusion_attn_fwd_stats", mm, 8, 8);
+    EGM_REQUIRE(pool_ws && N > 0 && HW > 0 && C <= 2048 && C_real > 0 && C_real <= C, "fusion_attn_fwd_stats: bad args");
+    const long long npix = (long long)N * HW;
+    const int G = group_for(C / 8 > 64 ? 64 : C / 8);
+    const int nbp = pool_blocks(HW, C);
+    const AttnCut cut = attn_cut(egm_stream_grid(npix * G), nbp * N, 0);
+    float* part = (float*)pool_ws;
+    int* pidx = (int*)(part + (long long)N * nbp * 2 * C);
+    EGM_DISPATCH_DTYPE(dtype, EGM_GROUP_SWITCH(G, hipLaunchKernelGGL((fusion_attn_fwd_stats_kernel<T, GROUP>), dim3(cut.blk0[2]), dim3(256), 0,
+                                                                     (hipStream_t)st, cut, (const T*)sv, lds, (T*)mm, npix, C, C_real,
+                                                                     (const T*)f, ldf, HW, part, pidx, nbp)));
+    EGM_CHECK_LAUNCH("fusion_attn_fwd_stats");
+    return EGM_OK;
+}
+extern "C" int egm_fusion_attn_fwd_gates(int dtype, const void* mm, const float* w_sa, void* sa, const void* pool_ws, void* pooled, int* argidx,
+                                         const float* w0, const float* w2, float* h, void* ca, int N, int H, int W, int C, int C_real, int Cr,
+                                         egm_stream_t st) {
+    EGM_REQ_VEC("fusion_attn_fwd_gates", mm, 8, 8); EGM_REQ_VEC("fusion_attn_fwd_gates", sa, 8, 8);
+    EGM_REQUIRE(w_sa && pool_ws && pooled && argidx && w0 && w2 && h && ca && egm_aligned16(pooled), "fusion_attn_fwd_gates: null pointer");
+    EGM_REQUIRE(N > 0 && H > 0 && W > 0 && C > 0 && C % 8 == 0 && C <= 2048 && C_real > 0 && C_real <= C && Cr > 0,
+                "fusion_attn_fwd_gates: bad shape");
+    const int R = 2 * N;
+    const size_t smem = (size_t)(R * C_real + R * Cr + Cr * (C_real + 1) + C_real * (Cr + 1)) * sizeof(float);
+    EGM_REQUIRE(smem <= 64 * 1024, "fusion_attn_fwd_gates: %d rows x %d channels do not fit one workgroup's LDS", R, C_real);
+    const long long HW = (long long)H * W;
+    const int nbp = pool_blocks(HW, C);
+    const AttnCut cut = attn_cut(sa_tile_grid(N, H, W), (N * C + 3) / 4, 0);
+    const float* part = (const float*)pool_ws;
+    const int* pidx = (const int*)(part + (long long)N * nbp * 2 * C);
+    EGM_DISPATCH_DTYPE(dtype, {
+        hipLaunchKernelGGL((fusion_attn_fwd_gates_kernel<T>), dim3(cut.blk0[2]), dim3(256), 0, (hipStream_t)st, cut, (const T*)mm, w_sa, (T*)sa, N,
+                           H, W, part, pidx, nbp, C, (T*)pooled, argidx);
+        hipLaunchKernelGGL((ca_mlp_fwd_kernel<T>), dim3(1), dim3(256), smem, (hipStream_t)st, (const T*)pooled, C, w0, w2, h, (T*)ca, C, R, C_real,
+                           Cr);
+    });
+    EGM_CHECK_LAUNCH("fusion_attn_fwd_gates");
+    return EGM_OK;
+}
+extern "C" int egm_fusion_attn_bwd_mid(int dtype, const float* partials, int nblk, float* red, const void* dsa, const float* w_sa, void* dmm,
+                                       const void* mm, void* sa_ws, int N, int H, int W, int C, egm_stream_t st) {
+    EGM_REQ_VEC("fusion_attn_bwd_mid", dsa, 8, 8); EGM_REQ_VEC("fusion_attn_bwd_mid", dmm, 8, 8); EGM_REQ_VEC("fusion_attn_bwd_mid", mm, 8, 8);
+    EGM_REQUIRE(partials && red && w_sa && sa_ws && nblk > 0 && N > 0 && H > 0 && W > 0 && C > 0, "fusion_attn_bwd_mid: bad args");
+    const AttnCut cut = attn_cut((C + 7) / 8 * N, sa_tile_grid(N, H, W), sa_blocks((long long)N * H * W));
+    EGM_DISPATCH_DTYPE(dtype, hipLaunchKernelGGL((fusion_attn_bwd_mid_kernel<T>), dim3(cut.blk0[3]), dim3(256), 0, (hipStream_t)st, cut, partials,
+                                                 nblk, C, red, (const T*)dsa, w_sa, (T*)dmm, (const T*)mm, (float*)sa_ws, N, H, W));
+    EGM_CHECK_LAUNCH("fusion_attn_bwd_mid");
+    return EGM_OK;
+}
+extern "C" int egm_fusion_attn_bwd_tail(int dtype, const float* red, void* dca, const void* pooled, const float* h, const float* w0,
+                                        const float* w2, float* dw0, float* dw2, void* dpooled, const int* argidx, void* df, const void* dmm,
+                                        const void* sv, int lds, const void* ds_b, int ldb, void* ds, const void* sa_ws, float* dw_sa, int N,
+                                        int H, int W, int C, int C_real, int Cr, egm_stream_t st) {
+    EGM_REQ_VEC("fusion_attn_bwd_tail", dmm, 8, 8); EGM_REQ_VEC("fusion_attn_bwd_tail", sv, lds, C); EGM_REQ_VEC("fusion_attn_bwd_tail", ds_b, ldb, C);
+    EGM_REQ_VEC("fusion_attn_bwd_tail", ds, C, C); EGM_REQ_VEC("fusion_attn_bwd_tail", df, C, C);
+    EGM_REQUIRE(red && dca && pooled && h && w0 && w2 && dw0 && dw2 && dpooled && argidx && sa_ws && dw_sa && egm_aligned16(dpooled),
+                "fusion_attn_bwd_tail: null pointer");
+    EGM_REQUIRE(N > 0 && H > 0 && W > 0 && C_real > 0 && C_real <= C && Cr > 0, "fusion_attn_bwd_tail: bad shape");
+    const int R = 2 * N;
+    const size_t smem = (size_t)(2 * R * C_real + 2 * R * Cr + Cr * (C_real + 1) + C_real * (Cr + 1)) * sizeof(float);
+    EGM_REQUIRE(smem <= 64 * 1024, "fusion_attn_bwd_tail: %d rows x %d channels do not fit one workgroup's LDS", R, C_real);
+    const long long HW = (long long)H * W, npix = (long long)N * HW;
+    const int G = group_for(C / 8 > 64 ? 64 : C / 8);
+    const AttnCut cut = attn_cut(1, 98, egm_stream_grid(npix * G));
+    EGM_DISPATCH_DTYPE(dtype, {
+        EGM_GROUP_SWITCH(G, hipLaunchKernelGGL((fusion_attn_bwd_tail_kernel<T, GROUP>), dim3(cut.blk0[3]), dim3(256), smem, (hipStream_t)st, cut, red,
+                                               (T*)dca, (const T*)pooled, h, w0, w2, dw0, dw2, (T*)dpooled, N, C, C_real, Cr,
+                                               (const float*)sa_ws, sa_blocks(npix), dw_sa, (const T*)dmm, (const T*)sv, lds, (const T*)ds_b, ldb,
+                                               (T*)ds, npix));
+        hipLaunchKernelGGL((global_pool_bwd_kernel<T>), dim3(egm_stream_grid(npix * (C / 8))), dim3(256), 0, (hipStream_t)st, (const T*)dpooled,
+                           argidx, (T*)df, C, N, HW, C);
+    });
+    EGM_CHECK_LAUNCH("fusion_attn_bwd_tail");
+    return EGM_OK;
+}
diff --git a/egm_unet_amd/egm_unet.py b/egm_unet_amd/egm_unet.py
--- a/egm_unet_amd/egm_unet.py
+++ b/egm_unet_amd/egm_unet.py
@@ -135,6 +135,10 @@
         w7, b7 = ops.merge357(self.conv_3x3.weight, self.conv_5x5.weight, self.conv_7x7.weight, self.conv_3x3.bias,
                               self.conv_5x5.bias, self.conv_7x7.bias, pack_dtype=f.dtype)
         s = ops.conv2d(f_ms, w7, b7)
+        if ops.fusion_attention_ok(s.dtype, self.spatial_attention.conv1.weight):
+            fc = self.channel_attention.fc
+            comb = ops.fusion_attention(f_res, f_ca, s, self.spatial_attention.conv1.weight, fc[0].weight, fc[2].weight, self._dim)
+            return ops.conv2d(comb, self.up.weight, self.up.bias)
         s_a, s_b = ops.fork(s, 2)
         sa = self.spatial_attention.logits(s_a, self._dim)
         ca = self.channel_attention.logits(f_ca)
diff --git a/egm_unet_amd/ops.py b/egm_unet_amd/ops.py
--- a/egm_unet_amd/ops.py
+++ b/egm_unet_amd/ops.py
@@ -2098,6 +2098,75 @@
     return _FusionCombine.apply(f, s, sa, ca)
 
 
+fuse_attention = _Switch("EGM_FUSE_ATTENTION", "1",
+                         """Get / set whether FusionConv runs its spatial and channel attention as ONE autograd node whose independent kernels
+                         share launches (bf16, 7x7 spatial attention; egm_fusion_attn_*): 8 launches per forward/backward pair instead of
+                         16, the same bits (tests compare both ways).""")
+
+
+def fusion_attention_ok(dtype, w_sa):
+    return fuse_attention.on and dtype == torch.bfloat16 and tuple(w_sa.shape) == (1, 2, 7, 7) and _fold_packs() is None
+
+
+class _FusionAttention(Function):
+
+    @staticmethod
+    def forward(ctx, f_res, f_ca, s, w_sa, w_fc0, w_fc2, c_real):
+        f_res, ldr = _nhwc(f_res); f_ca, ldf = _nhwc(f_ca); s, lds = _nhwc(s)
+        N, H, W, C = s.shape
+        Cr = w_fc0.shape[0]
+        L, dev, dt = lib(), s.device, s.dtype
+        code = dtype_code(dt)
+        wsa, w0, w2 = w_sa.detach().contiguous(), w_fc0.detach().contiguous(), w_fc2.detach().contiguous()
+        mm = torch.empty((N, H, W, 8), dtype=dt, device=dev)
+        ws = torch.empty(L.query("egm_global_pool_workspace", N, H * W, C) // 4 + 4, dtype=torch.float32, device=dev)
+        L.call("egm_fusion_attn_fwd_stats", code, ptr(s), lds, ptr(mm), ptr(f_ca), ldf, ptr(ws), N, H * W, C, c_real, stream())
+        sa = torch.empty((N, H, W, 8), dtype=dt, device=dev)
+        pooled = torch.empty((2 * N, 1, 1, C), dtype=dt, device=dev)
+        argidx = torch.empty((N, C), dtype=torch.int32, device=dev)
+        h = torch.empty((2 * N, Cr), dtype=torch.float32, device=dev)
+        ca = (torch.empty if C == c_real else torch.zeros)((2 * N, 1, 1, C), dtype=dt, device=dev)
+        L.call("egm_fusion_attn_fwd_gates", code, ptr(mm), ptr(wsa), ptr(sa), ptr(ws), ptr(pooled), ptr(argidx), ptr(w0), ptr(w2), ptr(h),
+               ptr(ca), N, H, W, C, c_real, Cr, stream())
+        out = torch.empty((N, H, W, C), dtype=dt, device=dev)
+        L.call("egm_fusion_combine_fwd", code, ptr(f_res), ldr, ptr(s), lds, ptr(sa), 8, ptr(ca), ptr(out), C, N, H * W, C, stream())
+        ctx.save_for_backward(s, mm, sa, ca, pooled, h, argidx, wsa, w0, w2)
+        ctx.c_real = c_real
+        return out
+
+    @staticmethod
+    def backward(ctx, g):
+        s, mm, sa, ca, pooled, h, argidx, wsa, w0, w2 = ctx.saved_tensors
+        s, lds = _nhwc(s); g, ldg = _nhwc(g)
+        N, H, W, C = s.shape
+        Cr, c_real = w0.shape[0], ctx.c_real
+        L, dev, dt = lib(), s.device, s.dtype
+        code = dtype_code(dt)
+        ds_b = torch.empty(s.shape, dtype=dt, device=dev)
+        dsa = torch.empty((N, H, W, 8), dtype=dt, device=dev)
+        nb = L.query("egm_fusion_combine_blocks", H * W, C)
+        part = _f32((N, nb, 2, C), dev)
+        L.call("egm_fusion_combine_bwd", code, ptr(g), ldg, ptr(s), lds, ptr(sa), 8, ptr(ca), ptr(ds_b), C, ptr(dsa), 8, ptr(part), N, H * W, C,
+               stream())
+        red = _f32((N, 2, C), dev)
+        dmm = torch.empty((N, H, W, 8), dtype=dt, device=dev)
+        sa_ws = torch.empty(L.query("egm_sa_conv7_bwd_workspace", N, H, W) // 4 + 4, dtype=torch.float32, device=dev)
+        L.call("egm_fusion_attn_bwd_mid", code, ptr(part), nb, ptr(red), ptr(dsa), ptr(wsa), ptr(dmm), ptr(mm), ptr(sa_ws), N, H, W, C, stream())
+        dca = torch.empty((2 * N, 1, 1, C), dtype=dt, device=dev)
+        dw0, dw2 = torch.empty_like(w0), torch.empty_like(w2)
+        dp = (torch.empty if C == c_real else torch.zeros)((2 * N, 1, 1, C), dtype=dt, device=dev)
+        df = torch.empty((N, H, W, C), dtype=dt, device=dev)
+        ds = torch.empty((N, H, W, C), dtype=dt, device=dev)
+        dw_sa = torch.empty((1, 2, 7, 7), dtype=torch.float32, device=dev)
+        L.call("egm_fusion_attn_bwd_tail", code, ptr(red), ptr(dca), ptr(pooled), ptr(h), ptr(w0), ptr(w2), ptr(dw0), ptr(dw2), ptr(dp),
+               ptr(argidx), ptr(df), ptr(dmm), ptr(s), lds, ptr(ds_b), C, ptr(ds), ptr(sa_ws), ptr(dw_sa), N, H, W, C, c_real, Cr, stream())
+        return g, df, ds, dw_sa, dw0, dw2, None
+
+
+def fusion_attention(f_res, f_ca, s, w_sa, w_fc0, w_fc2, c_real):
+    return _FusionAttention.apply(f_res, f_ca, s, w_sa, w_fc0, w_fc2, c_real)
+
+
 def _register_pack(weight, dtype, wf, wd):
     key = (weight.data_ptr(), weight._version, _weight_generation[0], dtype, 1, tuple(weight.shape))
     _pack_cache[id(weight)] = (key, wf, wd, weakref.ref(weight))
diff --git a/include/egm_hip.h b/include/egm_hip.h
--- a/include/egm_hip.h
+++ b/include/egm_hip.h
@@ -223,6 +223,17 @@
 int egm_fusion_combine_blocks(long long HW, int C);
 int egm_fusion_combine_bwd(int dtype, const void* g, int ldg, const void* sv, int lds, const void* sa, int ldsa, const void* ca,
                            void* ds, int ldds, void* dsa, int lddsa, float* partials, int N, long long HW, int C, egm_stream_t s);
+int egm_fusion_attn_fwd_stats(int dtype, const void* sv, int lds, void* mm, const void* f, int ldf, void* pool_ws, int N, long long HW,
+                              int C, int C_real, egm_stream_t st);
+int egm_fusion_attn_fwd_gates(int dtype, const void* mm, const float* w_sa, void* sa, const void* pool_ws, void* pooled, int* argidx,
+                              const float* w0, const float* w2, float* h, void* ca, int N, int H, int W, int C, int C_real, int Cr,
+                              egm_stream_t st);
+int egm_fusion_attn_bwd_mid(int dtype, const float* partials, int nblk, float* red, const void* dsa, const float* w_sa, void* dmm,
+                            const void* mm, void* sa_ws, int N, int H, int W, int C, egm_stream_t st);
+int egm_fusion_attn_bwd_tail(int dtype, const float* red, void* dca, const void* pooled, const float* h, const float* w0,
+                             const float* w2, float* dw0, float* dw2, void* dpooled, const int* argidx, void* df, const void* dmm,
+                             const void* sv, int lds, const void* ds_b, int ldb, void* ds, const void* sa_ws, float* dw_sa, int N,
+                             int H, int W, int C, int C_real, int Cr, egm_stream_t st);
 int egm_fold2_fwd(const float* w, float* out, int rows, int K, egm_stream_t s);
 int egm_fold2_bwd(const float* g, float* dw, int rows, int K, egm_stream_t s);
 int egm_merge357_fwd(const float* w3, const float* w5, const float* w7, const float* b3, const float* b5, const float* b7,
```
